# Ego-J/I2VSGG

Hardware: AMD Instinct MI355X
Metric: frames/sec (600x1000, 32 ROI/frame) (higher is better)
Workload: dtype f32; 1 GPU; BASELINE.json configs[1]: cfgs/res101.yml, SGG_emb fwd+bwd+SGD, 2 frames/GPU 600x1000, 32 boxes + 32 pairs/frame, ResNet-101 C4; frames_per_gpu=2, global_frames=2, hip_graph=True, parallelism=dp1 (frames sharded, RCCL all-reduce of vrd grads)

## Files before the change

i2vsgg_amd/_lib.py:

```python
import ctypes as C
import os

import torch

_HERE = os.path.dirname(os.path.abspath(__file__))
LIB_PATH = os.path.join(_HERE, "libi2vsgg_hip.so")

LAYOUT_NHWC, LAYOUT_NCHW = 0, 1
EPI_RELU, EPI_RESIDUAL, EPI_SCALE, EPI_BIAS, EPI_ZEROED = 1, 2, 4, 8, 16

_p, _i, _f, _z, _l = C.c_void_p, C.c_int32, C.c_float, C.c_size_t, C.c_int64

SIGNATURES = {
    "i2v_version": (_i, []),
    "i2v_last_error": (C.c_char_p, []),
    "i2v_build_flags": (_i, []),
    "i2v_stream_create": (_i, [_i, _i, C.POINTER(C.c_void_p)]),
    "i2v_stream_destroy": (_i, [_p]),
    "i2v_roi_align_fwd": (_i, [_p, _i, _i, _i, _i, _i, _p, _i, _i, _i, _f, _i, _p, _i, _p]),
    "i2v_roi_align_bwd": (_i, [_p, _i, _p, _i, _i, _i, _f, _i, _p, _i, _i, _i, _i, _i, _p]),
    "i2v_roi_align_bwd_gather_workspace_bytes": (_z, [_i, _i, _i, _i, _i]),
    "i2v_roi_align_bwd_gather": (_i, [_p, _p, _i, _i, _i, _f, _i, _p, _i, _i, _i, _i, _p, _z, _p]),
    "i2v_roi_align_sampled_fwd": (_i, [_p, _i, _i, _i, _i, _i, _p, _i, _i, _i, _f, _i, _p, _i, _p]),
    "i2v_roi_align_sampled_bwd": (_i, [_p, _i, _p, _i, _i, _i, _f, _i, _p, _i, _i, _i, _i, _i, _p]),
    "i2v_roi_pool_fwd": (_i, [_p, _i, _i, _i, _i, _i, _p, _i, _i, _i, _f, _p, _p, _i, _p]),
    "i2v_roi_pool_fwd_geom": (_i, [_p, _i, _i, _p, _l, _p, _i, _i, _i, _f, _p, _p, _i, _p]),
    "i2v_roi_pool_bwd": (_i, [_p, _p, _i, _p, _i, _i, _i, _p, _i, _i, _i, _i, _i, _p]),
    "i2v_nms_workspace_bytes": (_z, [_i, _i]),
    "i2v_nms_sorted": (_i, [_p, _i, _i, _f, _i, _p, _p, _p, _z, _p]),
    "i2v_rpn_proposal_workspace_bytes": (_z, [_i, _i, _i, _i, _i]),
    "i2v_rpn_proposal": (_i, [_p, _i, _p, _p, _p, _i, _i, _i, _i, _i, _i, _i, _f, _p, _p, _p, _p, _z, _p]),
    "i2v_rpn_decode": (_i, [_p, _i, _p, _p, _p, _i, _i, _i, _i, _i, _p, _p, _p]),
    "i2v_sort_desc_workspace_bytes": (_z, [_i, _i]),
    "i2v_sort_desc": (_i, [_p, _i, _i, _p, _p, _z, _p]),
    "i2v_bbox_overlaps": (_i, [_p, _i, _i, _i, _p, _i, _i, _i, _p, _p, _p, _p]),
    "i2v_conv_fwd": (_i, [_p, _p, _p, _p, _p, _p, _i, _i, _i, _i, _i, _i, _i, _i, _i, _i, _p, _z, _p]),
    "i2v_conv_fwd_splits": (_i, [_i, _i, _i, _i, _i, _i, _i, _i, _i, _z]),
    "i2v_conv_split_workspace_bytes": (_z, [_i, _i, _i, _i, _i, _i, _i, _i, _i]),
    "i2v_conv_fwd_plan": (_i, [_i, _i, _i, _i, _i, _i, _i, _i, _i, _i, _i, _z, _p, _i]),
    "i2v_conv_wgrad_plan": (_i, [_i, _i, _i, _i, _i, _i, _i, _i, _i, _i, _i, _i, _i, _i, _z, _p, _i]),
    "i2v_set_tuning": (_i, [_i, _i]),
    "i2v_get_tuning": (_i, [_i]),
    "i2v_gemm_nt_batched": (_i, [_p, _p, _p, _i, _i, _i, _i, _l, _l, _l, _p, _z, _p]),
    "i2v_winograd_filter": (_i, [_p, _p, _i, _i, _p]),
    "i2v_conv3x3_winograd_workspace_bytes": (_z, [_i, _i, _i, _i, _i]),
    "i2v_conv3x3_winograd_fwd": (_i, [_p, _p, _p, _p, _p, _i, _i, _i, _i, _i, _i, _p, _z, _p]),
    "i2v_winograd4_filter": (_i, [_p, _p, _i, _i, _p]),
    "i2v_winograd4_filter_dgrad": (_i, [_p, _p, _i, _i, _p]),
    "i2v_conv3x3_winograd4_workspace_bytes": (_z, [_i, _i, _i, _i, _i]),
    "i2v_conv3x3_winograd4_fwd": (_i, [_p, _p, _p, _p, _p, _i, _i, _i, _i, _i, _i, _p, _z, _p]),
    "i2v_conv_set_tile": (_i, [_i]),
    "i2v_conv_debug_clock": (_i, [_p]),
    "i2v_debug_clock_stamp": (_i, [_p, _p]),
    "i2v_conv_dgrad_workspace_bytes": (_z, [_i, _i, _i, _i]),
    "i2v_conv_dgrad": (_i, [_p, _p, _p, _i, _i, _i, _i, _i, _i, _i, _i, _i, _p, _z, _p, _z, _p]),
    "i2v_conv_wgrad_workspace_bytes": (_z, [_i, _i, _i, _i, _i, _i, _i, _i, _i]),
    "i2v_conv_wgrad": (_i, [_p, _p, _p, _i, _i, _i, _i, _i, _i, _i, _i, _i, _f, _p, _z, _p]),
    "i2v_conv_dgrad_fused": (_i, [_p, _p, _p, _p, _p, _p, _p, _i, _i, _i, _i, _i, _i, _i, _i, _i, _p, _z, _p, _z, _p]),
    "i2v_conv_wgrad_scaled": (_i, [_p, _p, _p, _p, _i, _i, _i, _i, _i, _i, _i, _i, _i, _f, _p, _z, _p]),
    "i2v_ordered_fallbacks": (_i, [_i]),
    "i2v_conv3x3_winograd4_dgrad": (_i, [_p, _p, _p, _p, _p, _i, _i, _i, _i, _i, _p, _z, _p]),
    "i2v_conv3x3_winograd4_wgrad_workspace_bytes": (_z, [_i, _i, _i, _i, _i]),
    "i2v_conv3x3_winograd4_wgrad": (_i, [_p, _p, _p, _p, _i, _i, _i, _i, _i, _f, _p, _z, _p]),
    "i2v_gemm_tn_batched": (_i, [_p, _p, _p, _i, _i, _i, _i, _l, _l, _l, _p]),
    "i2v_gemm_tn_batched_acc": (_i, [_p, _p, _p, _i, _i, _i, _i, _l, _l, _l, _p]),
    "i2v_conv3x3_winograd4_v_bytes": (_z, [_i, _i, _i, _i]),
    "i2v_conv3x3_winograd4_fwd_keep": (_i, [_p, _p, _p, _p, _p, _p, _i, _i, _i, _i, _i, _i, _p, _z, _p]),
    "i2v_conv3x3_winograd4_wgrad_v": (_i, [_p, _p, _p, _p, _i, _i, _i, _i, _i, _f, _p, _z, _p]),
    "i2v_conv_wgrad_sgd": (_i, [_p, _p, _p, _p, _i, _i, _i, _i, _i, _i, _i, _i, _i, _f, _f, _f, _p]),
    "i2v_epilogue_bwd": (_i, [_p, _p, _p, _p, _p, _p, _l, _i, _i, _p, _p, _z, _p]),
    "i2v_maxpool3x3s2_fwd": (_i, [_p, _p, _p, _i, _i, _i, _i, _p]),
    "i2v_sgd_momentum": (_i, [_p, _p, _p, _l, _f, _f, _f, _p]),
    "i2v_sgd_momentum_multi": (_i, [_p, _p, _p, _p, _p, _p, _i, _f, _p]),
    "i2v_adam_step": (_i, [_p, _p]),
    "i2v_adam_multi": (_i, [_p, _p, _p, _p, _p, _p, _p, _i, C.c_double, C.c_double, C.c_double, _p, _p]),
    "i2v_dstyle_pool_fwd": (_i, [_p, _p, _p, _l, _i, _i, _i, _p]),
    "i2v_dstyle_pool_bwd": (_i, [_p, _p, _p, _p, _p, _l, _i, _i, _i, _p]),
    "i2v_dstyle_fused_workspace_bytes": (_z, [_l, _i, _i, _i]),
    "i2v_dstyle_fused_fwd": (_i, [_p, _p, _p, _p, _p, _p, _p, _p, _l, _i, _i, _i, _i, _p, _z, _p]),
    "i2v_relation_topk_workspace_bytes": (_z, [_i, _i]),
    "i2v_relation_topk": (_i, [_p, _p, _p, _p, _i, _i, _i, _p, _p, _p, _p, _z, _p]),
    "i2v_video_associate_workspace_bytes": (_z, [_i, _i, _i]),
    "i2v_video_associate": (_i, [_p, _p, _p, _p, _p, _p, _i, _i, _i, _i, _p, _p, _p, _p, _p, _p, _z, _p]),
    "i2v_video_viou_match_workspace_bytes": (_z, [_i, _i]),
    "i2v_video_viou_match": (_i, [_p, _p, _p, _p, _p, _p, _i, _i, _i, _l, _i, _i, C.c_double, _p, _p, _p, _p, _z, _p]),
    "i2v_seqnms_workspace_bytes": (_z, [_i, _i, _i]),
    "i2v_seqnms": (_i, [_p, _p, _p, _p, _p, _i, _i, _i, C.c_double, C.c_double, _i, _p, _p, _p, _p, _z, _p]),
    "i2v_relation_targets_workspace_bytes": (_z, [_i]),
    "i2v_relation_targets": (_i, [_p] * 11 + [_i] * 5 + [_p] * 10 + [_z, _p]),
    "i2v_recognition_rows_workspace_bytes": (_z, [_i]),
    "i2v_recognition_rows": (_i, [_p, _p, _p, _p, _p, _i, _i, _i, _i, _p, _p, _p, _p, _p, _z, _p]),
    "i2v_recognition_align_workspace_bytes": (_z, [_i, _i]),
    "i2v_recognition_align": (_i, [_p, _p, _p, _p, _i, _i, _i, _i, _i, _i, _p, _p, _p, _p, _p, _p, _p, _z, _p]),
    "i2v_image_relation_match_workspace_bytes": (_z, [_i]),
    "i2v_image_relation_match": (_i, [_p, _p, _p, _p, _p, _p, _i, _i, _i, _i, C.c_double, _p, _p, _p, _p, _z, _p]),
    "i2v_image_relation_count": (_i, [_p, _p, _p, _p, _i, _i, _i, _p, _p, _p, _p, _z, _p]),
    "i2v_det_eval_match_workspace_bytes": (_z, [_i]),
    "i2v_det_eval_match": (_i, [_p, _p, _p, _p, _p, _p, _p, _i, _i, _i, _i, _i, C.c_double, _p, _p, _p, _p, _z, _p]),
    "i2v_det_eval_curve_workspace_bytes": (_z, [_i]),
    "i2v_det_eval_curve": (_i, [_p, _p, _p, _p, _i, _i, _p, _p, _p, _p, _p, _p, _p, _p, _z, _p]),
    "i2v_image_prep_size": (_i, [_i, _i, _i, _p, _p, _p]),
    "i2v_image_prep": (_i, [_p, _i, _i, _i, _i, _p, _i, _p, _i, _i, _p]),
    "i2v_det_postprocess_workspace_bytes": (_z, [_i, _i]),
    "i2v_det_postprocess": (_i, [_p, _p, _p, _i, _p, _p, _f, _f, _f, _i, _i, _f, _f, _i, _p, _p, _p, _z, _p]),
    "i2v_det_postprocess_info": (_i, [_p, _p, _p, _i, _p, _p, _p, _i, _i, _f, _f, _i, _p, _p, _p, _z, _p]),
    "i2v_l2norm_rows_fwd": (_i, [_p, _p, _p, _i, _i, _f, _p]),
    "i2v_l2norm_rows_bwd": (_i, [_p, _p, _p, _p, _i, _i, _f, _p]),
    "i2v_bce_rows_fwd": (_i, [_p, _p, _p, _p, _i, _i, _p]),
    "i2v_bce_rows_bwd": (_i, [_p, _p, _p, _p, _p, _i, _i, _p]),
    "i2v_half_mse_fwd": (_i, [_p, _l, _f, _p, _p]),
    "i2v_half_mse_bwd": (_i, [_p, _l, _f, _p, _p, _p]),
    "i2v_smooth_l1_fwd": (_i, [_p, _p, _p, _p, _l, _i, _i, _f, _p, _p]),
    "i2v_smooth_l1_bwd": (_i, [_p, _p, _p, _p, _l, _i, _i, _f, _p, _p, _p]),
    "i2v_bbox_transform": (_i, [_p, _i, _p, _i, _p, _i, _i, _p, _p, _p]),
    "i2v_signed_sqrt_fwd": (_i, [_p, _p, _l, _p]),
    "i2v_signed_sqrt_bwd": (_i, [_p, _p, _p, _l, _p]),
    "i2v_pair_gather_fwd": (_i, [_p, _p, _p, _p, _i, _i, _i, _p]),
    "i2v_pair_gather_bwd": (_i, [_p, _p, _p, _p, _i, _i, _i, _p]),
    "i2v_dpixel_fwd": (_i, [_p, _p, _p, _p, _p, _p, _p, _p, _i, _i, _p]),
    "i2v_dpixel_bwd_workspace_bytes": (_z, []),
    "i2v_dpixel_bwd": (_i, [_p, _p, _p, _p, _p, _p, _p, _p, _p, _p, _p, _p, _i, _i, _f, _p, _z, _p]),
}


class I2VError(RuntimeError):
    pass


def _load():
    if not os.path.exists(LIB_PATH):
        raise ImportError(
            "i2vsgg_amd: %s not found. Build it with `python -c 'import __graft_entry__ as g; g.build()'` "
            "(hipcc --offload-arch=gfx950). There is no CPU fallback." % LIB_PATH)
    lib = C.CDLL(LIB_PATH)
    for name, (res, args) in SIGNATURES.items():
        try:
            fn = getattr(lib, name)
        except AttributeError:
            raise ImportError("i2vsgg_amd: %s does not export %s (stale build?)" % (LIB_PATH, name))
        fn.restype, fn.argtypes = res, args
    return lib


lib = _load()

TUNE = {"I2V_CONV_SPEC": 0, "I2V_SPLIT_TARGET": 1, "I2V_SPLIT_TARGET_SKINNY": 2, "I2V_SPLIT_BELOW": 3, "I2V_SPLIT_ATOMICS": 4,
        "I2V_BIG_FC_TILE": 5, "I2V_WGRAD_V2": 6, "I2V_WGRAD_FUSED_TILE": 7, "I2V_WINO_ROWS": 8, "I2V_ROIPOOL_C128": 9, "I2V_CONV_GEMM": 10, "I2V_STAGGER": 11, "I2V_ROIALIGN_COLS": 12, "I2V_WGRAD_PER_CU": 13, "I2V_WGRAD_XCD": 14, "I2V_FC_FOLD": 15, "I2V_GEMM_X3": 16,
        "I2V_GEMM_PERSIST": 17, "I2V_WGRAD_PRIO": 18, "I2V_STREAM_TILE": 19, "I2V_KGROUPS": 20, "I2V_WGRAD_ORDERED_GFLOP": 21, "I2V_GEMM_DMA": 22,
        "I2V_WGRAD_DMA": 23, "I2V_ROIALIGN_BWD": 24, "I2V_NMS_SCAN": 25, "I2V_FC_UPDATE": 26}
ENV_TUNE = ("I2V_SPLIT_ATOMICS", "I2V_SPLIT_TARGET", "I2V_SPLIT_TARGET_SKINNY", "I2V_SPLIT_BELOW", "I2V_BIG_FC_TILE",
            "I2V_WGRAD_FUSED_TILE", "I2V_WGRAD_PER_CU", "I2V_KGROUPS", "I2V_WGRAD_ORDERED_GFLOP", "I2V_WINO_ROWS", "I2V_GEMM_DMA", "I2V_WGRAD_DMA", "I2V_ROIALIGN_BWD", "I2V_NMS_SCAN")
RETIRED_ENV = ("I2V_WINOGRAD_TRAIN", "I2V_BLOCK_FUSED", "I2V_WINOGRAD_WGRAD", "I2V_KEEP_V", "I2V_WGRAD_BRANCH", "I2V_ISD_BATCHED",
               "I2V_DEFER_FC", "I2V_EXPERIMENTS")
for _name, _key in TUNE.items():
    if os.environ.get(_name) in (None, ""):
        continue
    if _name not in ENV_TUNE:
        raise ImportError("i2vsgg_amd: %s is set but is not an environment knob (README.md lists them); it would be ignored. "
                          "Use i2vsgg_amd._lib.lib.i2v_set_tuning(TUNE[%r], value) from a tool or test" % (_name, _name))
    if lib.i2v_set_tuning(_key, int(os.environ[_name])) != 0:
        raise ImportError("i2vsgg_amd: %s=%s refused: %s" % (_name, os.environ[_name], lib.i2v_last_error().decode()))
for _name in RETIRED_ENV:
    if os.environ.get(_name) not in (None, ""):
        import warnings
        warnings.warn("i2vsgg_amd: %s is set but no longer read (a settled switch of rounds 1-5): the default runs" % _name)


def check(rc, what):
    if rc != 0:
        raise I2VError("%s failed (%d): %s" % (what, rc, lib.i2v_last_error().decode()))


def ptr(t):
    return None if t is None else t.data_ptr()


def stream():
    import torch
    return torch.cuda.current_stream().cuda_stream
```

i2vsgg_amd/csrc/api.cpp:

```cpp
#include <hip/hip_runtime.h>
#include <stdarg.h>
#include <stdio.h>
#include "../../include/i2vsgg_hip.h"

static thread_local char g_err[512] = "";

void i2v_set_error(const char* fmt, ...) {
    va_list ap;
    va_start(ap, fmt);
    vsnprintf(g_err, sizeof(g_err), fmt, ap);
    va_end(ap);
}

extern "C" int32_t i2v_version(void) { return 107; }
extern "C" const char* i2v_last_error(void) { return g_err; }

int g_i2v_tuning[I2V_TUNE_COUNT] = {
     -1,  2,  -1,  256,  2,
     1,  1,  128,  0,  1,
     1,  0,  2,  4,  1,
     0,  0,  0,  0,  1,
     0,  1000000,  1,  1,  1,  2,
     1,
};

extern "C" int32_t i2v_build_flags(void) {
    return 0;
}

extern "C" int32_t i2v_set_tuning(int32_t key, int32_t value) {
    if (key < 0 || key >= I2V_TUNE_COUNT) {
        i2v_set_error("set_tuning: unknown key %d", key);
        return I2V_ERR_ARG;
    }
    const bool retired = key == I2V_TUNE_CONV_SPEC ? value > 0
                       : (key == I2V_TUNE_FC_FOLD || key == I2V_TUNE_GEMM_X3 || key == I2V_TUNE_GEMM_PERSIST ||
                          key == I2V_TUNE_WGRAD_PRIO || key == I2V_TUNE_STAGGER) ? value != 0 : false;
    if (retired) {
        i2v_set_error("set_tuning: key %d belonged to an experiment kernel that is no longer in the library", key);
        return I2V_ERR_UNSUPPORTED;
    }
    g_i2v_tuning[key] = value;
    return I2V_OK;
}


extern "C" int32_t i2v_get_tuning(int32_t key) {
    return (key < 0 || key >= I2V_TUNE_COUNT) ? I2V_ERR_ARG : g_i2v_tuning[key];
}

extern "C" int32_t i2v_stream_create(int32_t device, int32_t priority, void** stream) {
    if (!stream) {
        i2v_set_error("stream_create: null output");
        return I2V_ERR_ARG;
    }
    int prev = -1, n = 0;
    if (hipGetDeviceCount(&n) != hipSuccess || device < 0 || device >= n) {
        i2v_set_error("stream_create: no device %d (%d visible)", device, n);
        return I2V_ERR_ARG;
    }
    hipStream_t s = nullptr;
    hipError_t e = hipGetDevice(&prev);
    if (e == hipSuccess && prev != device) e = hipSetDevice(device);
    if (e == hipSuccess) {
        int lo = 0, hi = 0;
        e = hipDeviceGetStreamPriorityRange(&lo, &hi);
        if (e == hipSuccess) {
            int pr = priority < hi ? hi : (priority > lo ? lo : priority);
            e = hipStreamCreateWithPriority(&s, hipStreamNonBlocking, pr);
        }
    }
    if (prev >= 0 && prev != device) (void)hipSetDevice(prev);
    if (e != hipSuccess) {
        i2v_set_error("stream_create: %s", hipGetErrorString(e));
        return I2V_ERR_LAUNCH;
    }
    *stream = (void*)s;
    return I2V_OK;
}

extern "C" int32_t i2v_stream_destroy(void* stream) {
    if (!stream) return I2V_OK;
    hipError_t e = hipStreamDestroy((hipStream_t)stream);
    if (e != hipSuccess) {
        i2v_set_error("stream_destroy: %s", hipGetErrorString(e));
        return I2V_ERR_LAUNCH;
    }
    return I2V_OK;
}
```

i2vsgg_amd/csrc/conv.hip:

```cpp
#include "conv_common.h"

using namespace convplan;

int g_ablate = 0;
unsigned long long* g_clk = nullptr;
int g_ordered_fallbacks = 0;

namespace {

struct ConvP {
    const float* x; const float* w; const float* scale; const float* shift; const float* res; float* y;
    const float* mask;
    int B, H, W, Cin, Cout, KH, KW, stride, pad, Ho, Wo;
    int pad_x;
    int M, N, K;
    int flags;
    int splitk, k_per_split;
    int ostride;
    int Hy, Wy;
    int lgCin;
    int reserved0;
    unsigned x_bytes, w_bytes;
    int ablate;
    int ktab_entries;
// ... 855 lines not shown
        if ((flags & I2V_EPI_MASK) && !(mask[i] > 0.f)) v = 0.f;
        y[i] = v;
    }
}

int g_force_tile = -1;

template <auto Kernel>
void launch_conv(dim3 grid, int threads, size_t lds, const ConvP& p, hipStream_t st) {
    static const bool once = [] {
        (void)hipFuncSetAttribute((const void*)Kernel, hipFuncAttributeMaxDynamicSharedMemorySize, 96 * 1024);
        return true;
    }();
    (void)once;
    Kernel<<<grid, threads, lds, st>>>(p);
}

template <int WAVES_M, int WAVES_N, int TM, int TN>
void launch_tile(int form, const ConvP& p, hipStream_t st) {
    constexpr int BM = WAVES_M * TM * 16, BN = WAVES_N * TN * 16;
    const dim3 grid(i2v_cdiv(p.M, BM) * i2v_cdiv(p.N, BN), p.splitk, p.nbatch > 1 ? p.nbatch : 1);
    const size_t lds_g = (size_t)(2 * (BM + BN) * BKS) * sizeof(float);
    const bool mask = (p.flags & I2V_EPI_MASK) != 0;
    switch (form) {
    case FORM_GEMM:
        if (mask) launch_conv<conv_gemm_f32<WAVES_M, WAVES_N, TM, TN, false, true>>(grid, THREADS, lds_g, p, st);
        else if (p.clk) launch_conv<conv_gemm_f32<WAVES_M, WAVES_N, TM, TN, true>>(grid, THREADS, lds_g, p, st);
        else launch_conv<conv_gemm_f32<WAVES_M, WAVES_N, TM, TN>>(grid, THREADS, lds_g, p, st);
        break;
    case FORM_GEMM_DMA32:
        if (mask) launch_conv<conv_gemm_f32<WAVES_M, WAVES_N, TM, TN, false, true, 1, 1>>(grid, THREADS, lds_g, p, st);
        else launch_conv<conv_gemm_f32<WAVES_M, WAVES_N, TM, TN, false, false, 1, 1>>(grid, THREADS, lds_g, p, st);
        break;
    case FORM_GEMM_DMA16:
        if (mask) launch_conv<conv_gemm_f32<WAVES_M, WAVES_N, TM, TN, false, true, 1, 2>>(grid, THREADS, lds_g / 2, p, st);
        else launch_conv<conv_gemm_f32<WAVES_M, WAVES_N, TM, TN, false, false, 1, 2>>(grid, THREADS, lds_g / 2, p, st);
        break;
    default: {
        const size_t stage = lds_g + p.ktab_entries * sizeof(float), epi = (size_t)BM * (BN + 4) * sizeof(float);
        launch_conv<conv_igemm_f32<WAVES_M, WAVES_N, TM, TN>>(grid, THREADS, stage > epi ? stage : epi, p, st);
    }
    }
}

template <int WAVES_M, int WAVES_N, int TM, int TN, int KG>
int launch_kgroups(const ConvP& p, hipStream_t st) {
    constexpr int BM = WAVES_M * TM * 16, BN = WAVES_N * TN * 16;
    constexpr int need = KG * 2 * (BM + BN) * BKS * 4;
    static_assert(need <= 159 * 1024, "the stage-buffer sets fit the CU's LDS");
    static const hipError_t once_k = [] {
        hipError_t e = hipFuncSetAttribute((const void*)conv_gemm_f32<WAVES_M, WAVES_N, TM, TN, false, false, KG>,
                                           hipFuncAttributeMaxDynamicSharedMemorySize, need);
        hipError_t e2 = hipFuncSetAttribute((const void*)conv_gemm_f32<WAVES_M, WAVES_N, TM, TN, false, true, KG>,
                                            hipFuncAttributeMaxDynamicSharedMemorySize, need);
        return e != hipSuccess ? e : e2;
    }();
    if (once_k != hipSuccess) {
        (void)hipGetLastError();
        i2v_set_error("conv: %d bytes of LDS refused for the K-group kernel: %s", need, hipGetErrorString(once_k));
        return I2V_ERR_LAUNCH;
    }
    const int tiles = i2v_cdiv(p.M, BM) * i2v_cdiv(p.N, BN);
    if (p.flags & I2V_EPI_MASK)
        conv_gemm_f32<WAVES_M, WAVES_N, TM, TN, false, true, KG><<<dim3(tiles, 1, 1), THREADS * KG, need, st>>>(p);
    else
        conv_gemm_f32<WAVES_M, WAVES_N, TM, TN, false, false, KG><<<dim3(tiles, 1, 1), THREADS * KG, need, st>>>(p);
    return I2V_OK;
}

ConvShape shape_of(const ConvP& p) {
    return {p.B, p.H, p.W, p.Cin, p.Cout, p.KH, p.KW, p.stride, p.pad, p.pad_x, p.ostride, p.Ho, p.Wo, p.nbatch, p.flags};
}

int run_conv(ConvP p, hipStream_t st, void* split_ws = nullptr, size_t split_ws_bytes = 0) {
    const ConvShape shape = shape_of(p);
    const FwdPlan pl = plan_conv_fwd(shape, g_i2v_tuning, g_force_tile, g_clk != nullptr, split_ws ? split_ws_bytes : 0);
    if (pl.status != PLAN_OK) return plan_error(pl.status, shape);
    p.M = p.B * p.Ho * p.Wo;
    p.N = p.Cout;
    p.K = p.KH * p.KW * p.Cin;
    p.lgCin = ilog2_exact(p.Cin);
    p.ktab_entries = pl.ktab_entries;
    p.x_bytes = pl.x_bytes;
    p.w_bytes = pl.w_bytes;
    p.clk = g_clk;
    p.ablate = g_ablate;
    p.splitk = pl.splitk;
    p.k_per_split = pl.k_per_split;
    p.ws = nullptr;
    p.cnt = nullptr;
    if (pl.finish == FIN_IN_KERNEL) {
        p.cnt = reinterpret_cast<int*>(split_ws);
        p.ws = reinterpret_cast<float*>(static_cast<char*>(split_ws) + kSplitCounterBytes);
    }
    if (pl.ordered_fallback) ++g_ordered_fallbacks;
    const long long ytotal = (long long)p.M * p.N;
    if (pl.clear_y) hipMemsetAsync(p.y, 0, (size_t)ytotal * sizeof(float), st);
    switch (pl.form == FORM_GEMM_KGROUPS2 ? 10 + pl.kg_tile : pl.form == FORM_GEMM_KGROUPS4 ? 20 + pl.kg_tile : pl.tile) {
        case 0: launch_tile<2, 2, 4, 4>(pl.form, p, st); break;
        case 1: launch_tile<2, 2, 4, 2>(pl.form, p, st); break;
        case 2: launch_tile<2, 2, 3, 2>(pl.form, p, st); break;
        case 3: launch_tile<1, 4, 5, 1>(pl.form, p, st); break;
        case 4: launch_tile<2, 2, 2, 2>(pl.form, p, st); break;
        case 5: launch_tile<2, 2, 1, 2>(pl.form, p, st); break;
        case 10: return launch_kgroups<1, 4, 5, 1, 2>(p, st);
        case 11: return launch_kgroups<2, 2, 2, 2, 2>(p, st);
        case 12: return launch_kgroups<1, 4, 3, 1, 2>(p, st);
        case 13: return launch_kgroups<2, 2, 1, 2, 2>(p, st);
        case 20: return launch_kgroups<1, 4, 5, 1, kKGroups>(p, st);
        case 21: return launch_kgroups<2, 2, 2, 2, kKGroups>(p, st);
        case 22: return launch_kgroups<1, 4, 3, 1, kKGroups>(p, st);
        case 23: return launch_kgroups<2, 2, 1, 2, kKGroups>(p, st);
    }
    if (pl.epilogue_pass == PASS_VEC4)
        conv_epilogue_kernel<<<(int)fmin((double)i2v_cdiv(ytotal / 4, 256), 4096.0), 256, 0, st>>>(
            p.y, p.scale, p.shift, p.res, p.mask, ytotal / 4, p.N, p.flags);
    else if (pl.epilogue_pass == PASS_SCALAR)
        conv_epilogue_scalar_kernel<<<(int)fmin((double)i2v_cdiv(ytotal, 256), 4096.0), 256, 0, st>>>(
            p.y, p.scale, p.shift, p.res, p.mask, ytotal, p.N, p.flags);
    return I2V_OK;
}

__global__ void weight_dgrad_layout(const float* __restrict__ w, float* __restrict__ wt, int Cout, int KH, int KW,
                                    int Cin, const float* __restrict__ nscale = nullptr) {
    const long long total = (long long)Cout * KH * KW * Cin;
    for (long long i = blockIdx.x * (long long)blockDim.x + threadIdx.x; i < total;
         i += (long long)gridDim.x * blockDim.x) {
        int n = i % Cout;
        long long t = i / Cout;
        int kx = t % KW; t /= KW;
        int ky = t % KH;
        int c = t / KH;
        const float v = w[(((long long)n * KH + (KH - 1 - ky)) * KW + (KW - 1 - kx)) * Cin + c];
        wt[i] = nscale ? v * nscale[n] : v;
    }
}

__global__ void weight_dgrad_sub_layout(const float* __restrict__ w, float* __restrict__ wt, int Cout, int KH, int KW,
                                        int Cin, int s, int ky0, int kx0, int Ty, int Tx) {
    const long long total = (long long)Cin * Ty * Tx * Cout;
    for (long long i = blockIdx.x * (long long)blockDim.x + threadIdx.x; i < total;
         i += (long long)gridDim.x * blockDim.x) {
        int n = i % Cout;
        long long t = i / Cout;
        int ux = t % Tx; t /= Tx;
        int uy = t % Ty;
        int c = t / Ty;
        const int ky = ky0 + s * (Ty - 1 - uy), kx = kx0 + s * (Tx - 1 - ux);
        wt[i] = w[(((long long)n * KH + ky) * KW + kx) * Cin + c];
    }
}

}

extern "C" int32_t i2v_ordered_fallbacks(int32_t reset) {
    const int n = g_ordered_fallbacks;
    if (reset) g_ordered_fallbacks = 0;
    return n;
}

extern "C" int32_t i2v_conv_debug_clock(void* buf) {
    g_clk = (unsigned long long*)buf;
    return I2V_OK;
}

namespace {
__global__ void clock_stamp_kernel(unsigned long long* out) {
    if (threadIdx.x == 0) { out[0] = __builtin_amdgcn_s_memtime(); out[1] = __builtin_amdgcn_s_memrealtime(); }
}
}

extern "C" int32_t i2v_debug_clock_stamp(void* out2, void* stream) {
    clock_stamp_kernel<<<1, 64, 0, (hipStream_t)stream>>>((unsigned long long*)out2);
    I2V_CHECK_LAUNCH("i2v_debug_clock_stamp");
    return I2V_OK;
}

extern "C" int32_t i2v_conv_set_tile(int32_t cfg) {
    if (cfg < 0) { g_force_tile = -1; g_ablate = 0; return I2V_OK; }
    if (cfg >> 8) {
        i2v_set_error("conv_set_tile: bits above the tile index selected experiment kernels that left the library in round 6");
        return I2V_ERR_UNSUPPORTED;
    }
    g_force_tile = (cfg & 0xFF) == 0xFF ? -1 : (cfg & 0xFF);
    return I2V_OK;
}

static int plan_conv(const char* who, FwdPlan& pl, size_t ws_bytes, int32_t B, int32_t H, int32_t W, int32_t Cin, int32_t Cout,
                     int32_t KH, int32_t KW, int32_t stride, int32_t pad, int32_t nbatch = 0, int32_t flags = 0) {
    int dummy = 0;
    int rc = check_conv(who, &dummy, &dummy, &dummy, B, H, W, Cin, Cout, KH, KW, stride, pad);
    if (rc) return rc;
    const ConvShape s = {B, H, W, Cin, Cout, KH, KW, stride, pad, pad, 1, (H + 2 * pad - KH) / stride + 1, (W + 2 * pad - KW) / stride + 1,
                         nbatch, flags};
    pl = plan_conv_fwd(s, g_i2v_tuning, g_force_tile, g_clk != nullptr, ws_bytes);
    return plan_error(pl.status, s);
}

extern "C" int32_t i2v_conv_fwd_splits(int32_t B, int32_t H, int32_t W, int32_t Cin, int32_t Cout, int32_t KH,
                                       int32_t KW, int32_t stride, int32_t pad, size_t ws_bytes) {
    FwdPlan pl = {};
    const int rc = plan_conv("conv_fwd_splits", pl, ws_bytes, B, H, W, Cin, Cout, KH, KW, stride, pad);
    return rc < 0 ? rc : pl.finish == FIN_ATOMICS;
}

extern "C" size_t i2v_conv_split_workspace_bytes(int32_t B, int32_t H, int32_t W, int32_t Cin, int32_t Cout, int32_t KH,
                                                 int32_t KW, int32_t stride, int32_t pad) {
    FwdPlan pl = {};
    return plan_conv("conv_fwd_splits", pl, 0, B, H, W, Cin, Cout, KH, KW, stride, pad) ? 0 : pl.ws_wanted;
}

extern "C" int32_t i2v_conv_fwd_plan(int32_t B, int32_t H, int32_t W, int32_t Cin, int32_t Cout, int32_t KH, int32_t KW,
                                     int32_t stride, int32_t pad, int32_t nbatch, int32_t flags, size_t ws_bytes, int32_t* out,
                                     int32_t n_out) {
    I2V_CHECK_ARG(out && n_out >= I2V_FWD_PLAN_FIELDS, "conv_fwd_plan: out needs room for I2V_FWD_PLAN_FIELDS values");
    FwdPlan pl = {};
    const int rc = plan_conv("conv_fwd_plan", pl, ws_bytes, B, H, W, Cin, Cout, KH, KW, stride, pad, nbatch, flags);
    if (rc && pl.status == PLAN_OK) return rc;
    const int32_t v[I2V_FWD_PLAN_FIELDS] = {pl.status, pl.tile, pl.splitk, pl.k_per_split, pl.ktab_entries, pl.form, pl.kg_tile,
                                            pl.finish, clamp32(pl.ws_wanted), clamp32(pl.ws_used), pl.clear_y, pl.epilogue_pass,
                                            pl.ordered_fallback};
    std::copy(v, v + I2V_FWD_PLAN_FIELDS, out);
    return I2V_OK;
}

extern "C" int32_t i2v_conv_fwd(const float* x, const float* w, const float* scale, const float* shift,
                                const float* res, float* y, int32_t B, int32_t H, int32_t W, int32_t Cin,
                                int32_t Cout, int32_t KH, int32_t KW, int32_t stride, int32_t pad, int32_t flags,
                                void* split_ws, size_t split_ws_bytes, void* stream) {
    int rc = check_conv("conv_fwd", x, w, y, B, H, W, Cin, Cout, KH, KW, stride, pad);
    if (rc) return rc;
    I2V_CHECK_ARG(!(flags & I2V_EPI_SCALE) || (scale && shift), "conv_fwd: EPI_SCALE needs scale and shift");
    I2V_CHECK_ARG(!(flags & I2V_EPI_BIAS) || shift, "conv_fwd: EPI_BIAS needs shift");
    I2V_CHECK_ARG(!(flags & I2V_EPI_RESIDUAL) || res, "conv_fwd: EPI_RESIDUAL needs res");
    ConvP p = {};
    p.x = x; p.w = w; p.scale = scale; p.shift = shift; p.res = res; p.y = y;
    p.B = B; p.H = H; p.W = W; p.Cin = Cin; p.Cout = Cout; p.KH = KH; p.KW = KW; p.stride = stride; p.pad = pad; p.pad_x = pad;
    p.Ho = (H + 2 * pad - KH) / stride + 1;
    p.Wo = (W + 2 * pad - KW) / stride + 1;
    p.flags = flags; p.ostride = 1; p.Hy = p.Ho; p.Wy = p.Wo;
    rc = run_conv(p, (hipStream_t)stream, split_ws, split_ws_bytes);
    if (rc) return rc;
    I2V_CHECK_LAUNCH("conv_fwd");
    return I2V_OK;
}

extern "C" int32_t i2v_gemm_nt_batched(const float* a, const float* b, float* c, int32_t M, int32_t N, int32_t K,
                                       int32_t nbatch, int64_t stride_a, int64_t stride_b, int64_t stride_c,
                                       void* split_ws, size_t split_ws_bytes, void* stream) {
    I2V_CHECK_ARG(a && b && c && M > 0 && N > 0 && K > 0 && nbatch > 0 && nbatch <= 65535, "gemm_nt_batched: bad argument");
    I2V_CHECK_ARG(K % 4 == 0, "gemm_nt_batched: K must be a multiple of 4");
    ConvP p = {};
    p.x = a; p.w = b; p.y = c;
    p.B = 1; p.H = M; p.W = 1; p.Cin = K; p.Cout = N; p.KH = 1; p.KW = 1; p.stride = 1; p.pad = 0; p.pad_x = 0;
    p.Ho = M; p.Wo = 1; p.flags = 0; p.ostride = 1; p.Hy = M; p.Wy = 1;
    p.nbatch = nbatch; p.bsx = stride_a; p.bsw = stride_b; p.bsy = stride_c;
    int rc = run_conv(p, (hipStream_t)stream, split_ws, split_ws_bytes);
    if (rc) return rc;
    I2V_CHECK_LAUNCH("gemm_nt_batched");
    return I2V_OK;
}

extern "C" size_t i2v_conv_dgrad_workspace_bytes(int32_t Cin, int32_t Cout, int32_t KH, int32_t KW) {
    return i2v_align((size_t)Cout * KH * KW * Cin * sizeof(float));
}

static int conv_dgrad_impl(const float* gy, const float* w, const float* gy_scale, const float* out_scale,
                           const float* res, const float* mask, float* gx, int32_t B, int32_t H, int32_t W,
                           int32_t Cin, int32_t Cout, int32_t KH, int32_t KW, int32_t stride, int32_t pad,
                           void* ws, size_t ws_bytes, void* split_ws, size_t split_ws_bytes, void* stream) {
    int rc = check_conv("conv_dgrad", gy, w, gx, B, H, W, Cin, Cout, KH, KW, stride, pad);
    if (rc) return rc;
    const bool fused = gy_scale || out_scale || res || mask;
    if (fused && stride != 1 && !(KH == 1 && KW == 1 && pad == 0)) {
        i2v_set_error("conv_dgrad_fused: stride 1, or a strided 1x1 layer (other strided layers take i2v_conv_dgrad and separate passes)");
        return I2V_ERR_UNSUPPORTED;
    }
    I2V_CHECK_ARG(Cout % 4 == 0, "conv_dgrad: Cout must be a multiple of 4");
    if (!ws || ws_bytes < (size_t)Cout * KH * KW * Cin * sizeof(float)) {
        i2v_set_error("conv_dgrad: workspace too small");
        return I2V_ERR_WORKSPACE;
    }
    hipStream_t st = (hipStream_t)stream;
    const int Ho = (H + 2 * pad - KH) / stride + 1, Wo = (W + 2 * pad - KW) / stride + 1;
    ConvP p = {};
    p.x = gy; p.y = gx;
    p.B = B; p.H = Ho; p.W = Wo; p.Cin = Cout; p.Cout = Cin; p.stride = 1;
    p.flags = 0;
    if (out_scale) { p.scale = out_scale; p.shift = nullptr; p.flags |= I2V_EPI_SCALE; }
    if (res) { p.res = res; p.flags |= I2V_EPI_RESIDUAL; }
    if (mask) { p.mask = mask; p.flags |= I2V_EPI_MASK; }
    p.Hy = H; p.Wy = W;
    const bool pointwise = KH == 1 && KW == 1 && pad == 0;
    if (stride == 1 || pointwise) {
        const long long wn = (long long)Cout * KH * KW * Cin;
        weight_dgrad_layout<<<(int)fmin((double)i2v_cdiv(wn, 256), 4096.0), 256, 0, st>>>(w, (float*)ws, Cout, KH, KW, Cin, gy_scale);
        p.w = (const float*)ws;
        p.KH = KH; p.KW = KW;
        if (stride == 1) {
            I2V_CHECK_ARG(KH - 1 - pad >= 0 && KW - 1 - pad >= 0, "conv_dgrad: padding larger than the filter");
            p.pad = KH - 1 - pad; p.pad_x = KW - 1 - pad;
            p.Ho = H; p.Wo = W; p.ostride = 1;
        } else {
            p.pad = 0; p.pad_x = 0; p.Ho = Ho; p.Wo = Wo; p.ostride = stride;
            hipMemsetAsync(gx, 0, (size_t)B * H * W * Cin * sizeof(float), st);
        }
// ... 54 lines not shown
```

i2vsgg_amd/csrc/conv_common.h:

```cpp
#pragma once
#include "common.h"
#include "conv_plan.h"
#include <algorithm>

typedef float f32x16 __attribute__((ext_vector_type(16)));
typedef float f32x4 __attribute__((ext_vector_type(4)));
typedef unsigned int u32x4 __attribute__((ext_vector_type(4)));

constexpr int THREADS = 256;

__device__ inline void lds_dma16(unsigned dst, unsigned voff, __amdgpu_buffer_rsrc_t r, unsigned soff) {
    asm volatile("s_mov_b32 m0, %0\n\ts_nop 0\n\tbuffer_load_dwordx4 %1, %2, %3 offen lds" ::"s"(dst), "v"(voff), "s"(r), "s"(soff) : "memory");
}

inline int ilog2_exact(int v) {
    if (v <= 0 || (v & (v - 1))) return -1;
    int l = 0;
    while ((1 << l) < v) ++l;
    return l;
}

inline int32_t clamp32(size_t v) { return (int32_t)std::min<size_t>(v, 0x7FFFFFFF); }

inline int check_conv(const char* who, const void* a, const void* b, const void* c, int B, int H, int W, int Cin,
                      int Cout, int KH, int KW, int stride, int pad) {
    if (!a || !b || !c) { i2v_set_error("%s: null pointer", who); return I2V_ERR_ARG; }
    if (B <= 0 || H <= 0 || W <= 0 || Cin <= 0 || Cout <= 0 || KH <= 0 || KW <= 0 || stride <= 0 || pad < 0) {
        i2v_set_error("%s: bad shape", who); return I2V_ERR_ARG;
    }
    if (Cin % 4) { i2v_set_error("%s: Cin must be a multiple of 4 (pad the stem input to 4 channels)", who); return I2V_ERR_ARG; }
    if ((H + 2 * pad - KH) < 0 || (W + 2 * pad - KW) < 0) { i2v_set_error("%s: kernel larger than input", who); return I2V_ERR_ARG; }
    return I2V_OK;
}

inline int plan_error(int status, const convplan::ConvShape& s) {
    using namespace convplan;
    if (status == PLAN_TAP_TABLE) i2v_set_error("conv: filter %dx%dx%d too large for the tap table", s.KH, s.KW, s.Cin);
    else if (status == PLAN_OPERAND_2GIB) i2v_set_error("conv: operand larger than 2 GiB (32-bit buffer offsets)");
    else if (status == PLAN_ROW_SCALE_NEEDS_V2) i2v_set_error("conv_wgrad_scaled: shape outside the v2 kernel (Cout % 4, 2 GiB operands)");
    else if (status == PLAN_FUSED_NEEDS_SPLIT) i2v_set_error("conv_wgrad_sgd: shape needs a split over pixels; use i2v_conv_wgrad + i2v_sgd_momentum");
    return status == PLAN_OK ? I2V_OK : I2V_ERR_UNSUPPORTED;
}

extern unsigned long long* g_clk;
extern int g_ablate;
extern int g_ordered_fallbacks;

int32_t i2v_internal_gemm_tn_batched_parts(const float* x, const float* gy, float* parts, int32_t M, int32_t N, int32_t K,
                                           int32_t nbatch, long long stride_x, long long stride_gy, int cap, int* splits, void* stream);
int32_t i2v_internal_reduce_parts(float* parts, int nparts, int planes, long long nk, void* stream);
void i2v_internal_reduce_scalar(const float* part, float* out, int nparts, long long n, int acc, unsigned blocks, void* stream);
```

i2vsgg_amd/csrc/conv_plan.h:

```cpp
#pragma once
#include <stddef.h>
#include <stdint.h>
#include "../../include/i2vsgg_hip.h"

namespace convplan {

constexpr int NUM_CU = 256;
constexpr int KTAB_MAX = 2560;
constexpr int BKS = 32;
constexpr int kSplitInKernelMax = 4;
constexpr int kKGroups = 4;
constexpr int kWgradOrderedMax = 16;
constexpr int kSplitCounters = 1024;
constexpr size_t kSplitCounterBytes = sizeof(int) * kSplitCounters;

struct TileCfg { int bm, bn; float eff; };
constexpr TileCfg kTiles[] = {{128, 128, 1.00f}, {128, 64, 0.97f}, {96, 64, 0.95f}, {80, 64, 0.95f}, {64, 64, 0.93f},
                              {32, 64, 0.80f}};
constexpr int kNumTiles = sizeof(kTiles) / sizeof(kTiles[0]);
constexpr int kKgroupBm[4] = {80, 64, 48, 32};

inline int cdiv(long long a, long long b) { return (int)((a + b - 1) / b); }

struct ConvShape {
    int B, H, W, Cin, Cout, KH, KW, stride, pad, pad_x, ostride, Ho, Wo, nbatch, flags;
    int M() const { return B * Ho * Wo; }
    int N() const { return Cout; }
    int K() const { return KH * KW * Cin; }
    int planes() const { return nbatch > 1 ? nbatch : 1; }
};

inline bool is_untapped(const ConvShape& s) { return s.KH == 1 && s.KW == 1 && s.pad == 0 && s.pad_x == 0; }
inline bool is_pointwise(const ConvShape& s) {
    return is_untapped(s) && s.stride == 1 && s.ostride == 1 && s.Ho == s.H && s.Wo == s.W && (s.N() & 3) == 0 && (s.K() & 3) == 0;
}
inline bool is_linear(const ConvShape& s) { return s.KH == 1 && s.KW == 1 && s.pad == 0 && s.stride == 1; }

enum PlanStatus { PLAN_OK = 0, PLAN_TAP_TABLE = 1, PLAN_OPERAND_2GIB = 2, PLAN_ROW_SCALE_NEEDS_V2 = 3, PLAN_FUSED_NEEDS_SPLIT = 4 };
enum FwdForm { FORM_IGEMM = 0, FORM_GEMM = 1, FORM_GEMM_DMA32 = 2, FORM_GEMM_DMA16 = 3, FORM_GEMM_KGROUPS2 = 4, FORM_GEMM_KGROUPS4 = 5 };
enum FwdFinish { FIN_NONE = 0, FIN_IN_KERNEL = 1, FIN_ATOMICS = 2 };
enum EpiloguePass { PASS_NONE = 0, PASS_VEC4 = 1, PASS_SCALAR = 2 };

struct FwdPlan {
    int status;
    int tile;
    int splitk, k_per_split;
    int ktab_entries;
    int form;
    int kg_tile;
    int finish;
    size_t ws_wanted;
    size_t ws_used;
    int clear_y;
    int epilogue_pass;
    int ordered_fallback;
    unsigned x_bytes, w_bytes;
};

inline FwdPlan plan_conv_fwd(const ConvShape& s, const int* tuning, int force_tile, bool clk, size_t ws_bytes) {
    FwdPlan q = {};
    const int M = s.M(), N = s.N(), K = s.K();
    if (!is_untapped(s) && (K > KTAB_MAX * 4 || s.KH * s.KW > 64 || ((long long)(s.KH * s.W + s.KW) * s.Cin) >= (1ll << 24))) {
        q.status = PLAN_TAP_TABLE;
        return q;
    }
    const long long xb = (long long)s.B * s.H * s.W * s.Cin * 4, wb = (long long)N * K * 4;
    const long long lead = (long long)(s.pad * s.W + s.pad_x) * s.Cin * 4;
    if (xb + (lead > 0 ? lead : 0) >= (1ll << 31) || wb >= (1ll << 31)) {
        q.status = PLAN_OPERAND_2GIB;
        return q;
    }
    q.ktab_entries = is_untapped(s) ? 4 : ((K + BKS - 1) / BKS) * (BKS / 4);
    q.x_bytes = (unsigned)xb;
    q.w_bytes = (unsigned)wb;
    const int split_atomics = tuning[I2V_TUNE_SPLIT_ATOMICS];
    const int ksteps = cdiv(K, BKS);
    auto cost_of = [&](int c, int& splitk) {
        const long long t = (long long)cdiv(M, kTiles[c].bm) * cdiv(N, kTiles[c].bn) * s.planes();
        splitk = 1;
        if (t < tuning[I2V_TUNE_SPLIT_BELOW] && ksteps >= 8 && s.ostride == 1 && s.nbatch <= 1) {
            const int skinny = tuning[I2V_TUNE_SPLIT_TARGET_SKINNY];
            const int target = (M <= 256 && skinny > 0) ? skinny : tuning[I2V_TUNE_SPLIT_TARGET];
            splitk = (int)((target * NUM_CU + t - 1) / t);
            splitk = splitk > ksteps / 4 ? ksteps / 4 : splitk;
            if (splitk < 1) splitk = 1;
            if (split_atomics == 2 && splitk > kSplitInKernelMax && (long long)M * N >= (1 << 18)) splitk = kSplitInKernelMax;
        }
        const long long blocks = t * splitk;
        const long long rounds = (blocks + NUM_CU - 1) / NUM_CU;
        const double r = rounds <= 4 ? (double)rounds : (double)blocks / NUM_CU + 0.5;
        double cost = r * kTiles[c].bm * kTiles[c].bn * (double)cdiv(ksteps, splitk) / kTiles[c].eff;
        if (splitk > 1) cost *= 1.05;
        return cost;
    };
    int cfg = 0, splitk = 1;
    double best = 1e300;
    for (int c = 0; c < kNumTiles; ++c) {
        int sk;
        const double cost = cost_of(c, sk);
        if (cost < best) { best = cost; cfg = c; splitk = sk; }
    }
    if (tuning[I2V_TUNE_STREAM_TILE] && s.KH == 1 && s.KW == 1 && s.stride == 1 && s.nbatch <= 1 && ksteps <= 4 && M >= 16384) {
        cfg = 3;
        cost_of(cfg, splitk);
    }
    if (s.nbatch > 1 && ksteps <= 4) { cfg = kNumTiles - 1; cost_of(cfg, splitk); }
    const int big_fc_tile = tuning[I2V_TUNE_BIG_FC_TILE];
    if (big_fc_tile >= 0 && big_fc_tile < kNumTiles && M <= 256 && K >= 16384) { cfg = big_fc_tile; cost_of(cfg, splitk); }
    if (force_tile >= 0 && force_tile < kNumTiles) { cfg = force_tile; cost_of(cfg, splitk); }
    q.tile = cfg;
    q.k_per_split = cdiv(ksteps, splitk) * BKS;
    q.splitk = cdiv(K, q.k_per_split);
    const bool gemm_kernel = is_pointwise(s) && tuning[I2V_TUNE_CONV_GEMM];
    const int kgroups = tuning[I2V_TUNE_KGROUPS];
    q.kg_tile = -1;
    const int kgn = kgroups == 2 ? 2 : kKGroups;
    if (kgroups && gemm_kernel && !clk && s.nbatch <= 1 && q.splitk >= 2 && force_tile < 0 && K % (kgn * BKS) == 0 &&
        K / kgn >= 2 * BKS && (long long)M * N >= (1 << 18)) {
        const int nt = cdiv(N, 64);
        for (int c = 3; c >= 0; --c) {
            const int t = cdiv(M, kKgroupBm[c]) * nt;
            if (t <= NUM_CU) { if (t >= (NUM_CU * 7) / 10) q.kg_tile = c; break; }
        }
        if (q.kg_tile >= 0) { q.splitk = 1; q.k_per_split = K; }
    }
    const long long ntiles = (long long)cdiv(M, kTiles[cfg].bm) * cdiv(N, kTiles[cfg].bn);
    const size_t ws_need = (size_t)q.splitk * ntiles * kTiles[cfg].bm * kTiles[cfg].bn * sizeof(float);
    const bool r4_ok = q.splitk <= kSplitInKernelMax && (long long)M * N >= (1 << 18);
    const bool wants_ws = q.splitk > 1 && split_atomics != 1 && (r4_ok || split_atomics == 0) && ntiles <= kSplitCounters &&
                          ws_need < (1ull << 31) - (64u << 20);
    const bool in_kernel = wants_ws && kSplitCounterBytes + ws_need <= ws_bytes;
    q.ws_wanted = wants_ws ? (kSplitCounterBytes + ws_need < 0x7FFFFFFF ? kSplitCounterBytes + ws_need : 0x7FFFFFFF) : 0;
    q.ws_used = in_kernel ? kSplitCounterBytes + ws_need : 0;
    q.finish = q.splitk <= 1 ? FIN_NONE : in_kernel ? FIN_IN_KERNEL : FIN_ATOMICS;
    q.ordered_fallback = q.finish == FIN_ATOMICS && split_atomics == 0;
    q.clear_y = q.finish == FIN_ATOMICS && !(s.flags & I2V_EPI_ZEROED);
    if (q.finish == FIN_ATOMICS && (s.flags & (I2V_EPI_SCALE | I2V_EPI_BIAS | I2V_EPI_RESIDUAL | I2V_EPI_RELU | I2V_EPI_MASK)))
        q.epilogue_pass = N % 4 == 0 ? PASS_VEC4 : PASS_SCALAR;
    const int dma = tuning[I2V_TUNE_GEMM_DMA];
    if (q.kg_tile >= 0) q.form = kgroups == 2 ? FORM_GEMM_KGROUPS2 : FORM_GEMM_KGROUPS4;
    else if (!gemm_kernel || q.finish == FIN_ATOMICS) q.form = FORM_IGEMM;
    else if (dma > 0 && !clk) q.form = dma == 2 ? FORM_GEMM_DMA16 : FORM_GEMM_DMA32;
    else q.form = FORM_GEMM;
    return q;
}

enum WgradKernel {
    WG_V1_64x64 = 0, WG_V2_DMA_128x128, WG_V2_DMA_128x64, WG_V2_DMA_64x64, WG_V2_FUSED_128x64, WG_V2_128x128, WG_V2_128x64,
    WG_V2_FUSED_64x64, WG_V2_CLK_64x64, WG_V2_64x64,
    WG_FC_UPDATE
};
enum WgradFinish { WFIN_DIRECT = 0, WFIN_ATOMICS = 1, WFIN_ORDERED_TILES = 2, WFIN_ORDERED_PARTS = 3, WFIN_EXTERNAL_PARTS = 4 };

struct WgradPlan {
    int status;
    int v2;
    int kernel;
    int tm, tk;
    int splits, m_per_split;
    int finish;
    int direct;
    int xcd_remap;
    int tiles;
    unsigned grid[3];
    int dma;
    size_t clear_bytes;
    int reduce_pass;
    int ordered_fallback;
    unsigned x_bytes, gy_bytes;
};

inline int wgrad_split_count(long long M, int N, int K, int planes, int tm, int tk, int rs, const int* tuning) {
    const long long tiles = (long long)cdiv(N, tm) * cdiv(K, tk), all_tiles = tiles * planes;
    const int msteps = cdiv(M, rs), per_cu = tuning[I2V_TUNE_WGRAD_PER_CU];
    int splits = (int)((long long)per_cu * NUM_CU / all_tiles);
    if (splits < 2) splits = (int)(((long long)per_cu * NUM_CU + all_tiles - 1) / all_tiles);
    if (splits > msteps / 4) splits = msteps / 4;
    if (splits < 1) splits = 1;
    return splits;
}

inline int wgrad_plane_splits(long long T, int Cout, int Cin, const int* tuning) {
    const int s = wgrad_split_count(T, Cout, Cin, 36, 64, 64, BKS, tuning);
    const int mps = cdiv(cdiv(T, BKS), s) * BKS;
    return cdiv(T, mps);
}

inline WgradPlan plan_wgrad(const ConvShape& s, bool beta_nonzero, bool fused, bool has_row_scale, int ext_part_cap, const int* tuning,
                            bool clk, size_t ws_bytes) {
    WgradPlan q = {};
    const int M = s.M(), N = s.N(), K = s.K(), planes = s.planes();
    const int wgrad_v2 = tuning[I2V_TUNE_WGRAD_V2];
    const long long xb = (long long)s.B * s.H * s.W * s.Cin * 4, gb = (long long)M * N * 4;
    const bool lin = is_linear(s);
    if (fused) {
        if ((long long)cdiv(N, 64) * cdiv(K, 64) < 2 * NUM_CU || M > 4096) { q.status = PLAN_FUSED_NEEDS_SPLIT; return q; }
        if (tuning[I2V_TUNE_FC_UPDATE] && wgrad_v2 && lin && M <= 256 && N % 4 == 0 && K % 4 == 0 && (long long)M * K * 4 < (1ll << 31) &&
            gb < (1ll << 31) && (long long)N * K * 4 < (1ll << 31)) {
            q.v2 = 1; q.kernel = WG_FC_UPDATE; q.splits = 1; q.direct = 1; q.finish = WFIN_DIRECT;
            return q;
        }
    }
    const bool v2 = (N % 4 == 0) && xb < (1ll << 31) && gb < (1ll << 31) && wgrad_v2;
    q.v2 = v2;
    if (has_row_scale && !v2) { q.status = PLAN_ROW_SCALE_NEEDS_V2; return q; }
    int tm = 64, tk = 64;
    if (v2 && fused && tuning[I2V_TUNE_WGRAD_FUSED_TILE] == 128 && N >= 128) tm = 128;
    if (v2 && wgrad_v2 >= 2) {
        if (N >= 128) tm = 128;
        if (K >= 128 && tm == 128 && wgrad_v2 == 2) tk = 128;
    }
    const long long tiles = (long long)cdiv(N, tm) * cdiv(K, tk);
    const int rs = v2 ? BKS : 16;
    const int msteps = cdiv(M, rs);
    int splits = fused ? 1 : wgrad_split_count(M, N, K, planes, tm, tk, rs, tuning);
    const bool ext_part = ext_part_cap >= 0;
    const bool has_ws = ws_bytes > 0;
    const double ord_flops = 1e9 * tuning[I2V_TUNE_WGRAD_ORDERED_GFLOP], flops = 2.0 * M * N * K * planes;
    const bool want_ord = !fused && !ext_part && splits > 1 && tuning[I2V_TUNE_SPLIT_ATOMICS] == 0 && flops < ord_flops;
    if (want_ord && has_ws && v2 && splits > kWgradOrderedMax && flops < 1e9) splits = kWgradOrderedMax;
    if (ext_part && splits > ext_part_cap) splits = ext_part_cap > 0 ? ext_part_cap : 1;
    q.m_per_split = cdiv(msteps, splits) * rs;
    splits = cdiv(M, q.m_per_split);
    q.direct = (splits == 1 && !beta_nonzero) || fused;
    q.finish = q.direct ? WFIN_DIRECT : WFIN_ATOMICS;
    if (ext_part) {
        if (splits > 1) q.finish = WFIN_EXTERNAL_PARTS;
    } else if (want_ord && splits > 1) {
        const size_t need_ord = kSplitCounterBytes + (size_t)splits * tiles * planes * (size_t)(tm * tk) * sizeof(float);
        const size_t need_part = kSplitCounterBytes + (size_t)splits * planes * (size_t)N * K * sizeof(float);
        if (has_ws && v2 && splits <= kWgradOrderedMax && tiles * planes <= kSplitCounters && need_ord <= ws_bytes && need_ord < (1ull << 31))
            q.finish = WFIN_ORDERED_TILES;
        else if (has_ws && need_part <= ws_bytes) {
            q.finish = WFIN_ORDERED_PARTS;
            q.reduce_pass = (((long long)N * K) & 3) == 0 ? PASS_VEC4 : PASS_SCALAR;
        } else q.ordered_fallback = 1;
    }
    if (!beta_nonzero && q.finish == WFIN_ATOMICS) q.clear_bytes = (size_t)planes * N * K * sizeof(float);
    q.x_bytes = (unsigned)xb;
    q.gy_bytes = (unsigned)gb;
    q.tm = tm; q.tk = tk; q.splits = splits; q.tiles = (int)tiles;
    q.grid[0] = (unsigned)tiles; q.grid[1] = (unsigned)splits; q.grid[2] = (unsigned)planes;
    const long long groups = (long long)splits * planes, total = tiles * groups;
    q.xcd_remap = (v2 && groups >= 2 && total < (1ll << 30) && tuning[I2V_TUNE_WGRAD_XCD]) ? 1 : 0;
    if (q.xcd_remap) { q.grid[0] = (unsigned)((total + 7) / 8 * 8); q.grid[1] = 1; q.grid[2] = 1; }
    const bool dma = v2 && !fused && !clk && lin && (K % 4 == 0) && tuning[I2V_TUNE_WGRAD_DMA];
    q.dma = dma;
    if (!v2) q.kernel = WG_V1_64x64;
    else if (dma && tm == 128 && tk == 128) q.kernel = WG_V2_DMA_128x128;
    else if (dma && tm == 128) q.kernel = WG_V2_DMA_128x64;
    else if (dma) q.kernel = WG_V2_DMA_64x64;
    else if (fused && tm == 128 && tk == 64) q.kernel = WG_V2_FUSED_128x64;
    else if (tm == 128 && tk == 128) q.kernel = WG_V2_128x128;
    else if (tm == 128) q.kernel = WG_V2_128x64;
    else if (fused) q.kernel = WG_V2_FUSED_64x64;
    else if (clk) q.kernel = WG_V2_CLK_64x64;
    else q.kernel = WG_V2_64x64;
    return q;
}

}
```

i2vsgg_amd/csrc/roi_ops.hip:

```cpp
#include "common.h"
#include <float.h>

namespace {

struct Strides { long long b, c, h, w; };

__host__ __device__ inline Strides feat_strides(int layout, int C, int H, int W) {
    Strides s;
    if (layout == I2V_LAYOUT_NHWC) { s.c = 1; s.w = C; s.h = (long long)W * C; s.b = (long long)H * W * C; }
    else { s.w = 1; s.h = W; s.c = (long long)H * W; s.b = (long long)C * H * W; }
    return s;
}

struct Sample { int ok, hs, ws; float hr, wr; };

__device__ inline Sample ra_sample(const float* roi, float scale, int H, int W, int AH, int AW, int ph, int pw) {
    Sample s;
    float x1 = roi[1] * scale, y1 = roi[2] * scale, x2 = roi[3] * scale, y2 = roi[4] * scale;
    float rw = fmaxf((float)((double)(x2 - x1) + 1.), 0.f);
    float rh = fmaxf((float)((double)(y2 - y1) + 1.), 0.f);
    float bh = (float)((double)rh / (AH - 1.));
    float bw = (float)((double)rw / (AW - 1.));
    float h = (float)ph * bh + y1;
    float w = (float)pw * bw + x1;
// ... 581 lines not shown
                v.x = l.x + v.x; v.y = l.y + v.y; v.z = l.z + v.z; v.w = l.w + v.w;
            }
            const int meta = __builtin_amdgcn_readfirstlane(rec.meta), nr = (meta >> 8) & 255, round = rec.meta & 255;
            float4* pl = (float4*)(mybuf + ((rec.off & 0xFFFFu) ^ lxor));
            float4* pr = (float4*)(mybuf + ((rec.off >> 16) ^ lxor));
            const float4 tl = make_float4(v.x * rec.wl, v.y * rec.wl, v.z * rec.wl, v.w * rec.wl);
            const float4 tr = make_float4(v.x * rec.wr, v.y * rec.wr, v.z * rec.wr, v.w * rec.wr);
#if defined(RAB_CLOCKS) && defined(RAB_ABL) && (RAB_ABL & 1)
            if (tl.x + tr.y == 12345.678f) *pl = tl;
            return;
#endif
            for (int s = 0; s < nr; ++s) {
                if (round == s) {
                    float4 a = *pl;
                    a.x += tl.x; a.y += tl.y; a.z += tl.z; a.w += tl.w;
                    *pl = a;
                    float4 c = *pr;
                    c.x += tr.x; c.y += tr.y; c.z += tr.z; c.w += tr.w;
                    *pr = c;
                }
            }
        };
        float4 q[RB2_DEPTH][NQ];
        if (n > 0) {
#pragma unroll
            for (int k = 0; k < RB2_DEPTH; ++k) issue(q[k], GROUPS * k + grp, list[min(GROUPS * k + grp, n - 1)]);
        }
        if (base == 0) {
            for (int i = threadIdx.x; i < (W + 2) * 32; i += 256) ((float4*)rowbuf)[i] = make_float4(0.f, 0.f, 0.f, 0.f);
        }
        for (int e0 = 0; e0 < n; e0 += RB2_CHUNK) {
            RAB_T(c_r0);
            {
                const int u = threadIdx.x >> 3, sx = threadIdx.x & 7, e = e0 + u;
                int cell = W;
                float wl = 0.f, wr = 0.f;
                if (e < n && sx < AW) {
                    const int code = 2 * base + (int)list[e], pair = code >> 1;
                    const int r = pair / AH, ah = pair - r * AH;
                    const float* roi = rois + 5 * (long long)r;
                    const AxisGeom qr = ra_axis(roi[2], roi[4], scale, H, AH, ah);
                    const AxisGeom qc = ra_axis(roi[1], roi[3], scale, W, AW, sx);
                    if (qc.ok) {
                        const float fh = (code & 1) ? qr.r : (1 - qr.r);
                        cell = qc.s; wl = fh * (1 - qc.r); wr = fh * qc.r;
                    }
                }
                int round = 0;
#pragma unroll
                for (int k = 1; k < 8; ++k) {
                    const int c = __shfl_up(cell, k, 8);
                    if (sx >= k && c == cell && cell < W) ++round;
                }
                int nr = round + 1;
#pragma unroll
                for (int m = 1; m < 8; m <<= 1) nr = max(nr, __shfl_xor(nr, m, 8));
                TapRec2 rec;
                rec.off = (unsigned)(cell * CHB + ((cell & 7) << 5)) | ((unsigned)((cell + 1) * CHB + (((cell + 1) & 7) << 5)) << 16);
                rec.wl = AVG ? wl * 0.25f : wl; rec.wr = AVG ? wr * 0.25f : wr;
                rec.meta = round | (nr << 8);
                s_rec[u][sx] = rec;
            }
            __syncthreads();
            RAB_T(c_r1);
            const int ne = min(RB2_CHUNK, n - e0);
            TapRec2 rec = s_rec[grp][sxl];
            int code = list[min(e0 + GROUPS * RB2_DEPTH + grp, n - 1)];
            for (int u0 = 0; u0 < ne; u0 += GROUPS * RB2_DEPTH) {
#pragma unroll
                for (int k = 0; k < RB2_DEPTH; ++k) {
                    const int u = u0 + GROUPS * k + grp;
                    const TapRec2 recn = s_rec[min(u + GROUPS, RB2_CHUNK - 1)][sxl];
                    const int coden = list[min(e0 + u + GROUPS * RB2_DEPTH + GROUPS, n - 1)];
                    if (u < ne) process(q[k], rec);
                    issue(q[k], e0 + u + GROUPS * RB2_DEPTH, code);
                    rec = recn;
                    code = coden;
                }
            }
            __syncthreads();
            RAB_T(c_r2);
            RAB_ADD(c_rec, c_r0, c_r1); RAB_ADD(c_add, c_r1, c_r2);
        }
    }
    __syncthreads();
    RAB_T(c_st0);
    constexpr int C4B = 32 / GROUPS;
    float* o = gfeat + (((long long)b * H + h) * W) * C + chunk * (128 / GROUPS);
    const float4* buf1 = (const float4*)rowbuf + (size_t)(W + 2) * C4B;
    for (int i = threadIdx.x; i < W * C4B; i += 256) {
        const int x = i / C4B, c4 = i % C4B, at = x * C4B + (c4 ^ ((x & 7) << 1));
        float4 a = ((const float4*)rowbuf)[at];
        if (GROUPS == 2) { const float4 c = buf1[at]; a.x += c.x; a.y += c.y; a.z += c.z; a.w += c.w; }
        *(float4*)(o + (long long)x * C + 4 * c4) = a;
    }
#ifdef RAB_CLOCKS
    if (threadIdx.x == 0 && blockIdx.x < 8192) {
        unsigned long long* o6 = g_rab_clk[blockIdx.x];
        const unsigned long long c_end = __builtin_amdgcn_s_memtime();
        o6[0] = c_end - c_begin; o6[1] = c_list; o6[2] = c_rec; o6[3] = c_end - c_st0; o6[4] = c_add; o6[5] = c_n;
    }
#endif
}

__global__ void __launch_bounds__(256)
roi_pool_fwd_kernel(const float* __restrict__ feat, const float* __restrict__ rois, float* __restrict__ out,
                    int* __restrict__ argmax, int C, int H, int W, int PH, int PW, float scale, Strides fs,
                    Strides os, int out_nchw, const int* __restrict__ geom, long long cap_cells) {
    extern __shared__ float lds[];
    const int P = PH * PW;
    float* sval = lds;
    int* sarg = (int*)(lds + 64 * P);
    if (geom) {
        H = geom[0]; W = geom[1];
        if (H <= 0 || W <= 0 || (long long)H * W > cap_cells) H = W = 0;
        fs = feat_strides(I2V_LAYOUT_NHWC, C, H, W);
    }
    const int chunks = (C + 63) / 64;
    const int r = blockIdx.x / chunks, c0 = (blockIdx.x % chunks) * 64;
    const int lane = threadIdx.x & 63, wave = threadIdx.x >> 6;
    const int c = c0 + lane;
    const float* roi = rois + 5 * (long long)r;
    const int b = (int)roi[0];
    const int x1 = (int)roundf(roi[1] * scale), y1 = (int)roundf(roi[2] * scale);
    const int x2 = (int)roundf(roi[3] * scale), y2 = (int)roundf(roi[4] * scale);
    const int rw = max(x2 - x1 + 1, 1), rh = max(y2 - y1 + 1, 1);
    const float bh = (float)rh / (float)PH, bw = (float)rw / (float)PW;
    const bool live = c < C;
    const float* fb = feat + (long long)b * fs.b + (live ? c : 0) * fs.c;
    for (int ph = wave; ph < PH; ph += 4) {
        int hs = (int)floorf((float)ph * bh), he = (int)ceilf((float)(ph + 1) * bh);
        hs = min(max(hs + y1, 0), H); he = min(max(he + y1, 0), H);
        for (int pw = 0; pw < PW; ++pw) {
            int ws = (int)floorf((float)pw * bw), we = (int)ceilf((float)(pw + 1) * bw);
            ws = min(max(ws + x1, 0), W); we = min(max(we + x1, 0), W);
            bool empty = (he <= hs) || (we <= ws);
            float m = empty ? 0.f : -FLT_MAX;
            int mi = -1;
            if (live)
                for (int h = hs; h < he; ++h)
                    for (int w = ws; w < we; ++w) {
                        float v = fb[h * fs.h + w * fs.w];
                        if (v > m) { m = v; mi = h * W + w; }
                    }
            sval[lane * P + ph * PW + pw] = m;
            sarg[lane * P + ph * PW + pw] = mi;
        }
    }
    __syncthreads();
    const int nch = min(64, C - c0);
    if (out_nchw) {
        float* o = out + (long long)r * C * P + (long long)c0 * P;
        int* a = argmax + (long long)r * C * P + (long long)c0 * P;
        for (int e = threadIdx.x; e < nch * P; e += 256) { o[e] = sval[e]; a[e] = sarg[e]; }
    } else {
        for (int p = wave; p < P; p += 4)
            if (live) {
                long long o = (long long)r * P * C + (long long)p * C + c;
                out[o] = sval[lane * P + p];
                argmax[o] = sarg[lane * P + p];
            }
    }
}

__global__ void __launch_bounds__(512)
roi_pool_fwd_c128_kernel(const float* __restrict__ feat, const float* __restrict__ rois, float* __restrict__ out,
                         int* __restrict__ argmax, int C, int H, int W, int PH, int PW, float scale, int out_nchw,
                         const int* __restrict__ geom, long long cap_cells) {
    extern __shared__ __attribute__((aligned(16))) float lds[];
    const int P = PH * PW;
    float* sval = lds;
    int* sarg = (int*)(lds + 128 * P);
    if (geom) {
        H = geom[0]; W = geom[1];
        if (H <= 0 || W <= 0 || (long long)H * W > cap_cells) H = W = 0;
    }
    const int chunks = C / 128;
    const int r = blockIdx.x / chunks, c0 = (blockIdx.x % chunks) * 128;
    const int l32 = threadIdx.x & 31, grp = threadIdx.x >> 5;
    const float* roi = rois + 5 * (long long)r;
    const int b = (int)roi[0];
    const int x1 = (int)roundf(roi[1] * scale), y1 = (int)roundf(roi[2] * scale);
    const int x2 = (int)roundf(roi[3] * scale), y2 = (int)roundf(roi[4] * scale);
    const int rw = max(x2 - x1 + 1, 1), rh = max(y2 - y1 + 1, 1);
    const float bh = (float)rh / (float)PH, bw = (float)rw / (float)PW;
    const __amdgpu_buffer_rsrc_t fr = __builtin_amdgcn_make_buffer_rsrc(const_cast<float*>(feat), 0, 0x7FFFFFFCu, 0x00020000);
    const unsigned lane_off = (unsigned)(c0 + 4 * l32) * 4u, row_bytes = (unsigned)C * 4u;
    const unsigned img = (unsigned)b * (unsigned)(H * W);
    const int ngrp = blockDim.x >> 5;
    for (int p = grp; p < P; p += ngrp) {
        const int ph = p / PW, pw = p - ph * PW;
        int hs = (int)floorf((float)ph * bh), he = (int)ceilf((float)(ph + 1) * bh);
        hs = min(max(hs + y1, 0), H); he = min(max(he + y1, 0), H);
        int ws = (int)floorf((float)pw * bw), we = (int)ceilf((float)(pw + 1) * bw);
        ws = min(max(ws + x1, 0), W); we = min(max(we + x1, 0), W);
        const bool empty = (he <= hs) || (we <= ws);
        float4 m = empty ? make_float4(0.f, 0.f, 0.f, 0.f) : make_float4(-FLT_MAX, -FLT_MAX, -FLT_MAX, -FLT_MAX);
        int4 mi = make_int4(-1, -1, -1, -1);
        const int nw = we - ws, cells = empty ? 0 : (he - hs) * nw;
        int h = hs, w = ws;
        for (int k0 = 0; k0 < cells; k0 += 8) {
            float4 v[8];
            int id[8];
#pragma unroll
            for (int u = 0; u < 8; ++u) {
                const bool live = k0 + u < cells;
                id[u] = live ? h * W + w : -1;
                v[u] = __builtin_bit_cast(float4, __builtin_amdgcn_raw_buffer_load_b128(
                    fr, ((img + (unsigned)(h * W + w)) * row_bytes + lane_off) | (live ? 0u : 0x80000000u), 0, 0));
                if (++w == we) { w = ws; ++h; }
            }
#pragma unroll
            for (int u = 0; u < 8; ++u) {
                if (id[u] < 0) continue;
                if (v[u].x > m.x) { m.x = v[u].x; mi.x = id[u]; }
                if (v[u].y > m.y) { m.y = v[u].y; mi.y = id[u]; }
                if (v[u].z > m.z) { m.z = v[u].z; mi.z = id[u]; }
                if (v[u].w > m.w) { m.w = v[u].w; mi.w = id[u]; }
            }
        }
        const int e = (4 * l32) * P + p;
        sval[e] = m.x; sval[e + P] = m.y; sval[e + 2 * P] = m.z; sval[e + 3 * P] = m.w;
        sarg[e] = mi.x; sarg[e + P] = mi.y; sarg[e + 2 * P] = mi.z; sarg[e + 3 * P] = mi.w;
    }
    __syncthreads();
    if (out_nchw) {
        float* o = out + (long long)r * C * P + (long long)c0 * P;
        int* a = argmax + (long long)r * C * P + (long long)c0 * P;
        if ((((long long)r * C + c0) * P) % 4 == 0 && (128 * P) % 4 == 0) {
            for (int e = threadIdx.x * 4; e < 128 * P; e += 4 * blockDim.x) {
                *(float4*)(o + e) = *(const float4*)(sval + e);
                *(int4*)(a + e) = *(const int4*)(sarg + e);
            }
        } else {
            for (int e = threadIdx.x; e < 128 * P; e += blockDim.x) { o[e] = sval[e]; a[e] = sarg[e]; }
        }
    } else {
        for (int e = threadIdx.x; e < 128 * P; e += blockDim.x) {
            const int p = e >> 7, ch = e & 127;
            const long long o = (long long)r * P * C + (long long)p * C + c0 + ch;
            out[o] = sval[ch * P + p];
            argmax[o] = sarg[ch * P + p];
        }
    }
}

__global__ void roi_pool_bwd_kernel(const float* __restrict__ gout, const int* __restrict__ argmax,
                                    const float* __restrict__ rois, float* __restrict__ gfeat, long long total,
                                    int C, int W, int P, Strides fs, int out_nchw) {
    for (long long idx = blockIdx.x * (long long)blockDim.x + threadIdx.x; idx < total;
         idx += (long long)gridDim.x * blockDim.x) {
        int c, r;
        if (out_nchw) { c = (idx / P) % C; r = idx / P / C; }
        else { c = idx % C; r = idx / C / P; }
        int a = argmax[idx];
        if (a < 0) continue;
        int b = (int)rois[5 * (long long)r];
        atomicAdd(gfeat + b * fs.b + c * fs.c + (a / W) * fs.h + (a % W) * fs.w, gout[idx]);
    }
}

struct RasGeom { float y0, x0, bh, bw; int gh, gw; };

__device__ inline RasGeom ras_geometry(const float* roi, float scale, int PH, int PW, int sampling) {
    RasGeom g;
    const float x1 = roi[1] * scale, y1 = roi[2] * scale, x2 = roi[3] * scale, y2 = roi[4] * scale;
    const float rw = fmaxf(x2 - x1, 1.f), rh = fmaxf(y2 - y1, 1.f);
    g.x0 = x1; g.y0 = y1;
    g.bh = rh / (float)PH; g.bw = rw / (float)PW;
    g.gh = sampling > 0 ? sampling : (int)ceilf(rh / (float)PH);
    g.gw = sampling > 0 ? sampling : (int)ceilf(rw / (float)PW);
    return g;
}

struct RasTaps { int ok, yl, xl, yh, xh; float w0, w1, w2, w3; };

__device__ inline RasTaps ras_taps(int H, int W, float y, float x) {
    RasTaps t;
    t.ok = !(y < -1.0f || y > (float)H || x < -1.0f || x > (float)W);
    if (y <= 0) y = 0;
    if (x <= 0) x = 0;
    t.yl = (int)y; t.xl = (int)x;
    if (t.yl >= H - 1) { t.yh = t.yl = H - 1; y = (float)t.yl; } else t.yh = t.yl + 1;
    if (t.xl >= W - 1) { t.xh = t.xl = W - 1; x = (float)t.xl; } else t.xh = t.xl + 1;
    const float ly = y - (float)t.yl, lx = x - (float)t.xl, hy = 1.f - ly, hx = 1.f - lx;
    t.w0 = hy * hx; t.w1 = hy * lx; t.w2 = ly * hx; t.w3 = ly * lx;
    if (!t.ok) t.yl = t.xl = t.yh = t.xh = 0;
    return t;
}

template <int VEC>
__global__ void __launch_bounds__(256)
roi_align_sampled_fwd_kernel(const float* __restrict__ feat, const float* __restrict__ rois, float* __restrict__ out,
                             int B, int C, int H, int W, int PH, int PW, float scale, int sampling, Strides fs,
                             Strides os) {
    const int pw = blockIdx.x % PW, ph = (blockIdx.x / PW) % PH, r = blockIdx.x / (PW * PH);
    const float* roi = rois + 5 * (long long)r;
    const int b = (int)roi[0];
    const bool live = b >= 0 && b < B;
    const RasGeom g = ras_geometry(roi, scale, PH, PW, sampling);
    const float count = (float)(g.gh * g.gw);
    const float* fb = feat + (long long)(live ? b : 0) * fs.b;
    for (int c = threadIdx.x * VEC; c < C; c += blockDim.x * VEC) {
        float acc[VEC];
#pragma unroll
        for (int k = 0; k < VEC; ++k) acc[k] = 0.f;
        for (int iy = 0; live && iy < g.gh; ++iy) {
            const float y = g.y0 + (float)ph * g.bh + ((float)iy + .5f) * g.bh / (float)g.gh;
            for (int ix = 0; ix < g.gw; ++ix) {
                const float x = g.x0 + (float)pw * g.bw + ((float)ix + .5f) * g.bw / (float)g.gw;
                const RasTaps t = ras_taps(H, W, y, x);
                if (!t.ok) continue;
                const float* p = fb + c * fs.c;
                float v0[VEC], v1[VEC], v2[VEC], v3[VEC];
                if (VEC == 4) {
                    *(float4*)v0 = *(const float4*)(p + t.yl * fs.h + t.xl * fs.w);
                    *(float4*)v1 = *(const float4*)(p + t.yl * fs.h + t.xh * fs.w);
                    *(float4*)v2 = *(const float4*)(p + t.yh * fs.h + t.xl * fs.w);
                    *(float4*)v3 = *(const float4*)(p + t.yh * fs.h + t.xh * fs.w);
                } else {
                    v0[0] = p[t.yl * fs.h + t.xl * fs.w]; v1[0] = p[t.yl * fs.h + t.xh * fs.w];
                    v2[0] = p[t.yh * fs.h + t.xl * fs.w]; v3[0] = p[t.yh * fs.h + t.xh * fs.w];
                }
#pragma unroll
                for (int k = 0; k < VEC; ++k) acc[k] += t.w0 * v0[k] + t.w1 * v1[k] + t.w2 * v2[k] + t.w3 * v3[k];
            }
        }
#pragma unroll
        for (int k = 0; k < VEC; ++k) out[r * os.b + (c + k) * os.c + ph * os.h + pw * os.w] = acc[k] / count;
    }
}

__global__ void __launch_bounds__(256)
roi_align_sampled_bwd_kernel(const float* __restrict__ gout, const float* __restrict__ rois, float* __restrict__ gfeat,
                             int B, int C, int H, int W, int PH, int PW, float scale, int sampling, Strides fs,
                             Strides os) {
    const int pw = blockIdx.x % PW, ph = (blockIdx.x / PW) % PH, r = blockIdx.x / (PW * PH);
    const float* roi = rois + 5 * (long long)r;
    const int b = (int)roi[0];
    if (b < 0 || b >= B) return;
    const RasGeom g = ras_geometry(roi, scale, PH, PW, sampling);
    const float count = (float)(g.gh * g.gw);
    float* fb = gfeat + (long long)b * fs.b;
    for (int c = threadIdx.x; c < C; c += blockDim.x) {
        const float top = gout[r * os.b + c * os.c + ph * os.h + pw * os.w];
        float* p = fb + c * fs.c;
        for (int iy = 0; iy < g.gh; ++iy) {
            const float y = g.y0 + (float)ph * g.bh + ((float)iy + .5f) * g.bh / (float)g.gh;
            for (int ix = 0; ix < g.gw; ++ix) {
                const float x = g.x0 + (float)pw * g.bw + ((float)ix + .5f) * g.bw / (float)g.gw;
                const RasTaps t = ras_taps(H, W, y, x);
                if (!t.ok) continue;
                atomicAdd(p + t.yl * fs.h + t.xl * fs.w, top * t.w0 / count);
                atomicAdd(p + t.yl * fs.h + t.xh * fs.w, top * t.w1 / count);
                atomicAdd(p + t.yh * fs.h + t.xl * fs.w, top * t.w2 / count);
                atomicAdd(p + t.yh * fs.h + t.xh * fs.w, top * t.w3 / count);
            }
        }
    }
}

inline Strides out_strides(int layout, int C, int PH, int PW) {
    Strides s;
    if (layout == I2V_LAYOUT_NHWC) { s.c = 1; s.w = C; s.h = (long long)PW * C; s.b = (long long)PH * PW * C; }
    else { s.w = 1; s.h = PW; s.c = (long long)PH * PW; s.b = (long long)C * PH * PW; }
    return s;
}

}

extern "C" int32_t i2v_roi_align_fwd(const float* feat, int32_t feat_layout, int32_t B, int32_t C, int32_t H,
                                     int32_t W, const float* rois, int32_t R, int32_t PH, int32_t PW,
                                     float scale, int32_t avg, float* out, int32_t out_layout, void* stream) {
    if (R == 0) return I2V_OK;
    I2V_CHECK_ARG(feat && rois && out, "roi_align_fwd: null pointer");
    I2V_CHECK_ARG(B > 0 && C > 0 && H >= 2 && W >= 2 && R >= 0 && PH > 0 && PW > 0, "roi_align_fwd: bad shape");
    I2V_CHECK_ARG(avg == 0 || avg == 1, "roi_align_fwd: avg must be 0/1");
    I2V_CHECK_ARG(avg || (PH > 1 && PW > 1), "roi_align_fwd: aligned grid needs >=2 points per side");
    hipStream_t st = (hipStream_t)stream;
    Strides os = out_strides(out_layout, C, PH, PW);
    if (feat_layout == I2V_LAYOUT_NHWC && (C % 4) == 0) {
        const int groups = (PW + 1) / 2;
        const bool per_roi = g_i2v_tuning[I2V_TUNE_ROIALIGN_COLS] == 2 && out_layout == I2V_LAYOUT_NHWC && (C % 128) == 0 &&
                             (PH + avg) * (PW + avg) <= 64 && (long long)B * H * W * C * 4 < (1ll << 31);
        if (per_roi) {
            if (R * (C / 128) < 512) {
                if (avg) roi_align_fwd_roi_kernel<1, 64><<<R * (C / 64), 256, 0, st>>>(feat, rois, out, R, C, H, W, PH, PW, scale);
                else roi_align_fwd_roi_kernel<0, 64><<<R * (C / 64), 256, 0, st>>>(feat, rois, out, R, C, H, W, PH, PW, scale);
            } else if (avg) roi_align_fwd_roi_kernel<1><<<R * (C / 128), 256, 0, st>>>(feat, rois, out, R, C, H, W, PH, PW, scale);
            else roi_align_fwd_roi_kernel<0><<<R * (C / 128), 256, 0, st>>>(feat, rois, out, R, C, H, W, PH, PW, scale);
        } else if (!g_i2v_tuning[I2V_TUNE_ROIALIGN_COLS]) {
            if (avg) roi_align_fwd_nhwc<1><<<R * PH, 256, 0, st>>>(feat, rois, out, C, H, W, PH, PW, scale, os);
            else roi_align_fwd_nhwc<0><<<R * PH, 256, 0, st>>>(feat, rois, out, C, H, W, PH, PW, scale, os);
        } else if (avg) {
            roi_align_fwd_nhwc_cols<1><<<(R + 7) / 8 * 8 * PH * groups, 256, 0, st>>>(feat, rois, out, R, C, H, W, PH, PW, scale, os);
        } else {
            roi_align_fwd_nhwc_cols<0><<<(R + 7) / 8 * 8 * PH * groups, 256, 0, st>>>(feat, rois, out, R, C, H, W, PH, PW, scale, os);
        }
    } else {
        Strides fs = feat_strides(feat_layout, C, H, W);
        long long total = (long long)R * C * PH * PW;
        int grid = (int)fmin((double)i2v_cdiv(total, 256), 65535.0 * 4);
        if (avg) roi_align_fwd_generic<1><<<grid, 256, 0, st>>>(feat, rois, out, total, C, H, W, PH, PW, scale, fs, os);
        else roi_align_fwd_generic<0><<<grid, 256, 0, st>>>(feat, rois, out, total, C, H, W, PH, PW, scale, fs, os);
    }
    I2V_CHECK_LAUNCH("roi_align_fwd");
    return I2V_OK;
}

extern "C" int32_t i2v_roi_align_bwd(const float* gout, int32_t out_layout, const float* rois, int32_t R,
                                     int32_t PH, int32_t PW, float scale, int32_t avg, float* gfeat,
                                     int32_t feat_layout, int32_t B, int32_t C, int32_t H, int32_t W,
                                     void* stream) {
    if (R == 0) return I2V_OK;
    I2V_CHECK_ARG(gout && rois && gfeat, "roi_align_bwd: null pointer");
    I2V_CHECK_ARG(B > 0 && C > 0 && H >= 2 && W >= 2 && R >= 0 && PH > 0 && PW > 0, "roi_align_bwd: bad shape");
    I2V_CHECK_ARG(avg == 0 || avg == 1, "roi_align_bwd: avg must be 0/1");
    hipStream_t st = (hipStream_t)stream;
    Strides os = out_strides(out_layout, C, PH, PW), fs = feat_strides(feat_layout, C, H, W);
    if (avg) roi_align_bwd_kernel<1><<<R * (PH + 1), 256, 0, st>>>(gout, rois, gfeat, C, H, W, PH, PW, scale, fs, os);
    else roi_align_bwd_kernel<0><<<R * PH, 256, 0, st>>>(gout, rois, gfeat, C, H, W, PH, PW, scale, fs, os);
    I2V_CHECK_LAUNCH("roi_align_bwd");
    return I2V_OK;
}

extern "C" size_t i2v_roi_align_bwd_gather_workspace_bytes(int32_t R, int32_t C, int32_t PH, int32_t PW, int32_t avg) {
    (void)R; (void)C; (void)PH; (void)PW; (void)avg;
    return 0;
}

extern "C" int32_t i2v_roi_align_bwd_gather(const float* gout, const float* rois, int32_t R, int32_t PH, int32_t PW, float scale,
                                            int32_t avg, float* gfeat, int32_t B, int32_t C, int32_t H, int32_t W, void* ws,
                                            size_t ws_bytes, void* stream) {
    (void)ws; (void)ws_bytes;
    I2V_CHECK_ARG(gout && rois && gfeat, "roi_align_bwd_gather: null pointer");
    I2V_CHECK_ARG(B > 0 && C > 0 && H >= 2 && W >= 2 && R > 0 && PH > 0 && PW > 0, "roi_align_bwd_gather: bad shape");
    I2V_CHECK_ARG(avg == 0 || avg == 1, "roi_align_bwd_gather: avg must be 0/1");
    I2V_CHECK_ARG(C % 128 == 0, "roi_align_bwd_gather: C must be a multiple of 128 (NHWC in and out)");
    const size_t AH = PH + avg, AW = PW + avg;
    I2V_CHECK_ARG(AW <= RAB_MAXA, "roi_align_bwd_gather: at most 8 sample columns (pooled_w + avg <= 8)");
    const bool form2 = g_i2v_tuning[I2V_TUNE_ROIALIGN_BWD] != 0;
    const size_t lds = (size_t)(W + 2) * 128 * sizeof(float) + (form2 ? 0 : (size_t)RAB_BATCH * RAB_MAXA * 128 * sizeof(float)) + RAB_SEG * sizeof(unsigned short);
    I2V_CHECK_ARG(lds <= 60 * 1024 && (long long)R * AH < (1ll << 29), "roi_align_bwd_gather: map too wide for the LDS row buffer");
    I2V_CHECK_ARG((long long)B * H * (C / 128) < (1ll << 31), "roi_align_bwd_gather: grid too large");
    I2V_CHECK_ARG((long long)R * PH * PW * C * 4 < (1ll << 31), "roi_align_bwd_gather: grad_out beyond the 2 GiB a 32-bit buffer offset reaches");
    hipStream_t st = (hipStream_t)stream;
    const bool two = form2 && (long long)B * H * (C / 64) <= 4ll * 256;
    static bool once = [] {
        (void)hipFuncSetAttribute((const void*)roi_align_bwd_row_kernel<0, 0>, hipFuncAttributeMaxDynamicSharedMemorySize, 60 * 1024);
        (void)hipFuncSetAttribute((const void*)roi_align_bwd_row_kernel<1, 0>, hipFuncAttributeMaxDynamicSharedMemorySize, 60 * 1024);
        (void)hipFuncSetAttribute((const void*)roi_align_bwd_row_kernel<1, 1>, hipFuncAttributeMaxDynamicSharedMemorySize, 60 * 1024);
        (void)hipFuncSetAttribute((const void*)roi_align_bwd_row2_kernel<0, 0, 1>, hipFuncAttributeMaxDynamicSharedMemorySize, 60 * 1024);
        (void)hipFuncSetAttribute((const void*)roi_align_bwd_row2_kernel<1, 0, 1>, hipFuncAttributeMaxDynamicSharedMemorySize, 60 * 1024);
        (void)hipFuncSetAttribute((const void*)roi_align_bwd_row2_kernel<1, 1, 1>, hipFuncAttributeMaxDynamicSharedMemorySize, 60 * 1024);
        (void)hipFuncSetAttribute((const void*)roi_align_bwd_row2_kernel<0, 0, 2>, hipFuncAttributeMaxDynamicSharedMemorySize, 60 * 1024);
        (void)hipFuncSetAttribute((const void*)roi_align_bwd_row2_kernel<1, 0, 2>, hipFuncAttributeMaxDynamicSharedMemorySize, 60 * 1024);
        (void)hipFuncSetAttribute((const void*)roi_align_bwd_row2_kernel<1, 1, 2>, hipFuncAttributeMaxDynamicSharedMemorySize, 60 * 1024);
        return true;
    }();
    (void)once;
    const dim3 grid(B * H * (C / 128)), grid2(B * H * (C / 64));
    const int p7 = avg && PH == 7 && PW == 7;
#define RAB2(A, P, G, GRID) roi_align_bwd_row2_kernel<A, P, G><<<GRID, 256, lds, st>>>(gout, rois, gfeat, R, PH, PW, scale, B, C, H, W)
    if (form2 && two) { if (p7) RAB2(1, 1, 2, grid2); else if (avg) RAB2(1, 0, 2, grid2); else RAB2(0, 0, 2, grid2); }
    else if (form2) { if (p7) RAB2(1, 1, 1, grid); else if (avg) RAB2(1, 0, 1, grid); else RAB2(0, 0, 1, grid); }
#undef RAB2
    else if (avg && PH == 7 && PW == 7) roi_align_bwd_row_kernel<1, 1><<<grid, 256, lds, st>>>(gout, rois, gfeat, R, PH, PW, scale, B, C, H, W);
    else if (avg) roi_align_bwd_row_kernel<1, 0><<<grid, 256, lds, st>>>(gout, rois, gfeat, R, PH, PW, scale, B, C, H, W);
    else roi_align_bwd_row_kernel<0, 0><<<grid, 256, lds, st>>>(gout, rois, gfeat, R, PH, PW, scale, B, C, H, W);
    I2V_CHECK_LAUNCH("roi_align_bwd_gather");
    return I2V_OK;
}

namespace {
int32_t roi_pool_fwd_launch(const float* feat, int32_t feat_layout, int32_t B, int32_t C, int32_t H, int32_t W,
                            const int32_t* geom, long long cap_cells, const float* rois, int32_t R, int32_t PH, int32_t PW,
                            float scale, float* out, int32_t* argmax, int32_t out_layout, void* stream) {
    I2V_CHECK_ARG(PH * PW <= 256, "roi_pool_fwd: pooled grid too large for the LDS stage");
    Strides fs = feat_strides(feat_layout, C, H, W), os = out_strides(out_layout, C, PH, PW);
    const int c128 = g_i2v_tuning[I2V_TUNE_ROIPOOL_C128];
    const long long feat_bytes = (long long)B * C * 4 * (geom ? cap_cells : (long long)H * W);
    if (c128 && feat_layout == I2V_LAYOUT_NHWC && C % 128 == 0 && (size_t)128 * PH * PW * 8 <= 64 * 1024 && feat_bytes < (1ll << 31)) {
        roi_pool_fwd_c128_kernel<<<R * (C / 128), 512, (size_t)128 * PH * PW * 8, (hipStream_t)stream>>>(
            feat, rois, out, argmax, C, H, W, PH, PW, scale, out_layout == I2V_LAYOUT_NCHW, geom, cap_cells);
        I2V_CHECK_LAUNCH("roi_pool_fwd");
        return I2V_OK;
    }
    size_t lds = (size_t)64 * PH * PW * 8;
    roi_pool_fwd_kernel<<<R * ((C + 63) / 64), 256, lds, (hipStream_t)stream>>>(
        feat, rois, out, argmax, C, H, W, PH, PW, scale, fs, os, out_layout == I2V_LAYOUT_NCHW, geom, cap_cells);
    I2V_CHECK_LAUNCH("roi_pool_fwd");
    return I2V_OK;
}
}

extern "C" int32_t i2v_roi_pool_fwd(const float* feat, int32_t feat_layout, int32_t B, int32_t C, int32_t H,
                                    int32_t W, const float* rois, int32_t R, int32_t PH, int32_t PW, float scale,
                                    float* out, int32_t* argmax, int32_t out_layout, void* stream) {
    if (R == 0) return I2V_OK;
    I2V_CHECK_ARG(feat && rois && out && argmax, "roi_pool_fwd: null pointer");
    I2V_CHECK_ARG(B > 0 && C > 0 && H > 0 && W > 0 && R >= 0 && PH > 0 && PW > 0, "roi_pool_fwd: bad shape");
    return roi_pool_fwd_launch(feat, feat_layout, B, C, H, W, nullptr, 0, rois, R, PH, PW, scale, out, argmax, out_layout,
                               stream);
}

extern "C" int32_t i2v_roi_pool_fwd_geom(const float* feat, int32_t B, int32_t C, const int32_t* geom, int64_t cap_cells,
                                         const float* rois, int32_t R, int32_t PH, int32_t PW, float scale, float* out,
                                         int32_t* argmax, int32_t out_layout, void* stream) {
    if (R == 0) return I2V_OK;
    I2V_CHECK_ARG(feat && geom && rois && out && argmax, "roi_pool_fwd_geom: null pointer");
    I2V_CHECK_ARG(B > 0 && C > 0 && cap_cells > 0 && R >= 0 && PH > 0 && PW > 0, "roi_pool_fwd_geom: bad shape");
    return roi_pool_fwd_launch(feat, I2V_LAYOUT_NHWC, B, C, 1, 1, geom, (long long)cap_cells, rois, R, PH, PW, scale, out,
                               argmax, out_layout, stream);
}

extern "C" int32_t i2v_roi_pool_bwd(const float* gout, const int32_t* argmax, int32_t out_layout,
                                    const float* rois, int32_t R, int32_t PH, int32_t PW, float* gfeat,
                                    int32_t feat_layout, int32_t B, int32_t C, int32_t H, int32_t W,
                                    void* stream) {
    if (R == 0) return I2V_OK;
    I2V_CHECK_ARG(gout && argmax && rois && gfeat, "roi_pool_bwd: null pointer");
    I2V_CHECK_ARG(B > 0 && C > 0 && H > 0 && W > 0 && R >= 0 && PH > 0 && PW > 0, "roi_pool_bwd: bad shape");
    Strides fs = feat_strides(feat_layout, C, H, W);
    long long total = (long long)R * C * PH * PW;
    int grid = (int)fmin((double)i2v_cdiv(total, 256), 65535.0 * 4);
    roi_pool_bwd_kernel<<<grid, 256, 0, (hipStream_t)stream>>>(gout, argmax, rois, gfeat, total, C, W, PH * PW, fs,
                                                                out_layout == I2V_LAYOUT_NCHW);
    I2V_CHECK_LAUNCH("roi_pool_bwd");
    return I2V_OK;
}

extern "C" int32_t i2v_roi_align_sampled_fwd(const float* feat, int32_t feat_layout, int32_t B, int32_t C, int32_t H,
                                             int32_t W, const float* rois, int32_t R, int32_t PH, int32_t PW,
                                             float scale, int32_t sampling_ratio, float* out, int32_t out_layout,
                                             void* stream) {
    if (R == 0) return I2V_OK;
    I2V_CHECK_ARG(feat && rois && out, "roi_align_sampled_fwd: null pointer");
    I2V_CHECK_ARG(B > 0 && C > 0 && H > 0 && W > 0 && R >= 0 && PH > 0 && PW > 0, "roi_align_sampled_fwd: bad shape");
    I2V_CHECK_ARG((long long)R * PH * PW < (1ll << 31), "roi_align_sampled_fwd: too many bins for one launch");
    Strides fs = feat_strides(feat_layout, C, H, W), os = out_strides(out_layout, C, PH, PW);
    const int grid = R * PH * PW;
    if (feat_layout == I2V_LAYOUT_NHWC && (C % 4) == 0)
        roi_align_sampled_fwd_kernel<4><<<grid, 256, 0, (hipStream_t)stream>>>(feat, rois, out, B, C, H, W, PH, PW, scale,
                                                                               sampling_ratio, fs, os);
    else
        roi_align_sampled_fwd_kernel<1><<<grid, 256, 0, (hipStream_t)stream>>>(feat, rois, out, B, C, H, W, PH, PW, scale,
                                                                               sampling_ratio, fs, os);
    I2V_CHECK_LAUNCH("roi_align_sampled_fwd");
    return I2V_OK;
}

extern "C" int32_t i2v_roi_align_sampled_bwd(const float* gout, int32_t out_layout, const float* rois, int32_t R,
                                             int32_t PH, int32_t PW, float scale, int32_t sampling_ratio, float* gfeat,
                                             int32_t feat_layout, int32_t B, int32_t C, int32_t H, int32_t W,
                                             void* stream) {
    if (R == 0) return I2V_OK;
    I2V_CHECK_ARG(gout && rois && gfeat, "roi_align_sampled_bwd: null pointer");
    I2V_CHECK_ARG(B > 0 && C > 0 && H > 0 && W > 0 && R >= 0 && PH > 0 && PW > 0, "roi_align_sampled_bwd: bad shape");
    I2V_CHECK_ARG((long long)R * PH * PW < (1ll << 31), "roi_align_sampled_bwd: too many bins for one launch");
    Strides fs = feat_strides(feat_layout, C, H, W), os = out_strides(out_layout, C, PH, PW);
    roi_align_sampled_bwd_kernel<<<R * PH * PW, 256, 0, (hipStream_t)stream>>>(gout, rois, gfeat, B, C, H, W, PH, PW, scale,
                                                                              sampling_ratio, fs, os);
    I2V_CHECK_LAUNCH("roi_align_sampled_bwd");
    return I2V_OK;
}
```

i2vsgg_amd/csrc/wgrad.hip:

```cpp
#include "conv_common.h"

using namespace convplan;

namespace {

constexpr int BK = 16;
constexpr int LDS_ROW = 20;

struct WgP {
    const float* x; const float* gy; float* gw; int direct;
    const float* row_scale;
    int xcd_remap;
    int r_tiles, r_splits, r_total;
    int nbatch;
    long long bsx, bsg, bsw;
    float* sgd_m; float lr, mom, wd;
    unsigned x_bytes, gy_bytes;
    int B, H, W, Cin, Cout, KH, KW, stride, pad, Ho, Wo, M, N, K, m_per_split, lgCin;
    unsigned long long* clk;
    int abl;
    float* ord_ws; int* ord_cnt; int ord_splits, ord_tiles, ord_acc;
    float* part_ws;
    int part_cap;
};
// ... 424 lines not shown
            for (int j = 0; j < TN; ++j)
                smem[row * CROW + (wn * TN + j) * 16 + fr] = p.row_scale ? acc[i][j][rr] * rsc : acc[i][j][rr];
        }
    __syncthreads();
    if (PREFETCH_W && p.sgd_m) {
#pragma unroll
        for (int it = 0; it < W_LD; ++it) {
            const int e = tid + it * THREADS;
            const int row = e / (BNW / 4), col = (e % (BNW / 4)) * 4;
            const int n = n0 + row, k = k0 + col;
            if (e >= BMW * (BNW / 4) || n >= p.N || k >= p.K) continue;
            const long long o = (long long)n * p.K + k;
            const float4 g = *(const float4*)&smem[row * CROW + col];
            float4 pv = pw[it], mv = pm[it];
            mv.x = p.mom * mv.x + (g.x + p.wd * pv.x); mv.y = p.mom * mv.y + (g.y + p.wd * pv.y);
            mv.z = p.mom * mv.z + (g.z + p.wd * pv.z); mv.w = p.mom * mv.w + (g.w + p.wd * pv.w);
            pv.x -= p.lr * mv.x; pv.y -= p.lr * mv.y; pv.z -= p.lr * mv.z; pv.w -= p.lr * mv.w;
            __builtin_nontemporal_store(__builtin_bit_cast(f32x4, mv), (f32x4*)(p.sgd_m + o));
            __builtin_nontemporal_store(__builtin_bit_cast(f32x4, pv), (f32x4*)(p.gw + o));
        }
    } else if (p.sgd_m || p.direct) {
        for (int e = tid; e < BMW * (BNW / 4); e += THREADS) {
            const int row = e / (BNW / 4), col = (e % (BNW / 4)) * 4;
            const int n = n0 + row, k = k0 + col;
            if (n >= p.N || k >= p.K) continue;
            const long long o = (long long)n * p.K + k;
            float4 g = *(const float4*)&smem[row * CROW + col];
            if (p.sgd_m) {
                float4 pv = *(const float4*)(p.gw + o), mv = *(const float4*)(p.sgd_m + o);
                mv.x = p.mom * mv.x + (g.x + p.wd * pv.x); mv.y = p.mom * mv.y + (g.y + p.wd * pv.y);
                mv.z = p.mom * mv.z + (g.z + p.wd * pv.z); mv.w = p.mom * mv.w + (g.w + p.wd * pv.w);
                pv.x -= p.lr * mv.x; pv.y -= p.lr * mv.y; pv.z -= p.lr * mv.z; pv.w -= p.lr * mv.w;
                *(float4*)(p.sgd_m + o) = mv;
                *(float4*)(p.gw + o) = pv;
            } else {
                *(float4*)(p.gw + o) = g;
            }
        }
    } else if (p.part_ws) {
        float* dst = p.part_ws + ((long long)by * (p.nbatch > 1 ? p.nbatch : 1) + bz) * ((long long)p.N * p.K);
        for (int e = tid; e < BMW * (BNW / 4); e += THREADS) {
            const int row = e / (BNW / 4), col = (e % (BNW / 4)) * 4;
            const int n = n0 + row, k = k0 + col;
            if (n >= p.N || k >= p.K) continue;
            *(float4*)(dst + (long long)n * p.K + k) = *(const float4*)&smem[row * CROW + col];
        }
    } else if (p.ord_ws) {
        constexpr int SC01 = 16;
        const int tile_lin = bz * p.ord_tiles + bx, nsplit = p.ord_splits, my = by;
        const size_t split_stride = (size_t)p.ord_tiles * (p.nbatch > 1 ? p.nbatch : 1) * (BMW * BNW);
        const __amdgpu_buffer_rsrc_t wsr = __builtin_amdgcn_make_buffer_rsrc(
            (void*)(p.ord_ws + (size_t)tile_lin * (BMW * BNW)), 0, 0x7FFFFFF0, 0x00020000);
        for (int e = tid; e < BMW * (BNW / 4); e += THREADS) {
            const int row = e / (BNW / 4), col = (e % (BNW / 4)) * 4;
            const float4 v = *(const float4*)&smem[row * CROW + col];
            __builtin_amdgcn_raw_buffer_store_b128(__builtin_bit_cast(u32x4, v), wsr,
                                                   (unsigned)(my * split_stride * sizeof(float)) + (unsigned)(row * BNW + col) * 4u, 0, SC01);
        }
        __builtin_amdgcn_s_waitcnt(0);
        __syncthreads();
        __shared__ int ord_last;
        if (tid == 0) {
            const int arrived = __hip_atomic_fetch_add(p.ord_cnt + tile_lin, 1, __ATOMIC_RELAXED, __HIP_MEMORY_SCOPE_AGENT);
            const int last = arrived == nsplit - 1;
            if (last) __hip_atomic_store(p.ord_cnt + tile_lin, 0, __ATOMIC_RELAXED, __HIP_MEMORY_SCOPE_AGENT);
            ord_last = last;
        }
        __syncthreads();
        if (ord_last) {
            for (int e = tid; e < BMW * (BNW / 4); e += THREADS) {
                const int row = e / (BNW / 4), col = (e % (BNW / 4)) * 4;
                const int n = n0 + row, k = k0 + col;
                if (n >= p.N || k >= p.K) continue;
                const long long o = (long long)n * p.K + k;
                const unsigned off = (unsigned)(row * BNW + col) * 4u;
                const float4 mine4 = *(const float4*)&smem[row * CROW + col];
                float4 v = make_float4(0.f, 0.f, 0.f, 0.f);
                if (p.ord_acc) v = *(const float4*)(p.gw + o);
                for (int s0 = 0; s0 < nsplit; s0 += 8) {
                    float4 u[8];
#pragma unroll
                    for (int sp = 0; sp < 8; ++sp)
                        u[sp] = __builtin_bit_cast(float4, __builtin_amdgcn_raw_buffer_load_b128(
                            wsr, (s0 + sp < nsplit && s0 + sp != my) ? off + (unsigned)((s0 + sp) * split_stride * sizeof(float)) : 0xFFFFFFF0u, 0, SC01));
#pragma unroll
                    for (int sp = 0; sp < 8; ++sp) {
                        const float4 t = s0 + sp == my ? mine4 : u[sp];
                        if (s0 == 0 && sp == 0 && !p.ord_acc) v = t;
                        else { v.x += t.x; v.y += t.y; v.z += t.z; v.w += t.w; }
                    }
                }
                *(float4*)(p.gw + o) = v;
            }
        }
    } else {
        for (int e = tid; e < BMW * BNW; e += THREADS) {
            const int row = e / BNW, col = e % BNW;
            const int n = n0 + row, k = k0 + col;
            if (n < p.N && k < p.K) atomicAdd(p.gw + (long long)n * p.K + k, smem[row * CROW + col]);
        }
    }
    if constexpr (CLK) {
        __builtin_amdgcn_s_waitcnt(0);
        if (tid == 0 && p.clk) {
            unsigned long long* o = p.clk + 8 * (blockIdx.y * gridDim.x + blockIdx.x);
            o[0] = c_rt0; o[1] = __builtin_amdgcn_s_memrealtime();
            o[2] = c_t1 - c_t0; o[3] = c_t2 - c_t1; o[4] = __builtin_amdgcn_s_memtime() - c_t2;
            o[5] = __builtin_amdgcn_s_getreg(63492); o[6] = __builtin_amdgcn_s_getreg(63508); o[7] = 1;
        }
    }
}

__global__ void __launch_bounds__(256)
wgrad_reduce_kernel(const float* __restrict__ part, float* __restrict__ gw, int splits, int planes, long long nk4, long long bsw, int acc) {
    const long long total = (long long)planes * nk4;
    for (long long e = blockIdx.x * 256ll + threadIdx.x; e < total; e += 256ll * gridDim.x) {
        const long long plane = e / nk4, i = e - plane * nk4;
        float4* o = (float4*)(gw + plane * bsw) + i;
        float4 v = acc ? *o : make_float4(0.f, 0.f, 0.f, 0.f);
        const float4* src = (const float4*)part + plane * nk4 + i;
        for (int s0 = 0; s0 < splits; s0 += 8) {
            float4 u[8];
#pragma unroll
            for (int k = 0; k < 8; ++k) u[k] = s0 + k < splits ? src[(long long)(s0 + k) * planes * nk4] : make_float4(0.f, 0.f, 0.f, 0.f);
#pragma unroll
            for (int k = 0; k < 8; ++k)
                if (s0 + k < splits) { v.x += u[k].x; v.y += u[k].y; v.z += u[k].z; v.w += u[k].w; }
        }
        *o = v;
    }
}
__global__ void __launch_bounds__(256)
wgrad_reduce_scalar_kernel(const float* __restrict__ part, float* __restrict__ gw, int splits, long long nk, int acc) {
    for (long long e = blockIdx.x * 256ll + threadIdx.x; e < nk; e += 256ll * gridDim.x) {
        float v = acc ? gw[e] : 0.f;
        for (int s0 = 0; s0 < splits; s0 += 16) {
            float u[16];
#pragma unroll
            for (int k = 0; k < 16; ++k) u[k] = s0 + k < splits ? part[(long long)(s0 + k) * nk + e] : 0.f;
#pragma unroll
            for (int k = 0; k < 16; ++k)
                if (s0 + k < splits) v += u[k];
        }
        gw[e] = v;
    }
}
constexpr int FCU_WAVES = 8, FCU_THREADS = 64 * FCU_WAVES, FCU_BN = 16 * FCU_WAVES, FCU_TK = 64;
struct FcuP {
    const float* x; const float* gy; float* w; float* m;
    float lr, mom, wd;
    int M, N, K;
    int strips, chunks, tiles, groups;
    unsigned x_bytes, gy_bytes, w_bytes;
};

template <int NS>
__global__ void __launch_bounds__(FCU_THREADS) fc_update_f32(const FcuP p) {
    const int L = (int)blockIdx.x, g = L & 7, r = L >> 3;
    const int start = (int)(((long long)g * p.groups) >> 3), count = (int)(((long long)(g + 1) * p.groups) >> 3) - start;
    if (r >= count) return;
    const int idx = start + r, chunk = idx / p.strips, strip = idx - chunk * p.strips;
    const int t0 = (int)((long long)chunk * p.tiles / p.chunks), t1 = (int)((long long)(chunk + 1) * p.tiles / p.chunks);

    constexpr unsigned MASK = 0x80000000u, NT = 2;
    constexpr int ROWS = 32 * NS;
    __shared__ __attribute__((aligned(16))) float xs[2][ROWS * FCU_TK];
    const int tid = threadIdx.x, lane = tid & 63, wave = tid >> 6, fr = lane & 15, fg = lane >> 4;
    const int n0 = strip * FCU_BN;
    const __amdgpu_buffer_rsrc_t gr = __builtin_amdgcn_make_buffer_rsrc((void*)p.gy, 0, p.gy_bytes, 0x00020000);
    const __amdgpu_buffer_rsrc_t xr = __builtin_amdgcn_make_buffer_rsrc((void*)p.x, 0, p.x_bytes, 0x00020000);
    const __amdgpu_buffer_rsrc_t wr = __builtin_amdgcn_make_buffer_rsrc((void*)p.w, 0, p.w_bytes, 0x00020000);
    const __amdgpu_buffer_rsrc_t mr = __builtin_amdgcn_make_buffer_rsrc((void*)p.m, 0, p.w_bytes, 0x00020000);

    float a[NS * 8];
    {
        const unsigned na = (unsigned)(n0 + 16 * wave + fr);
        const bool nin = (int)na < p.N;
#pragma unroll
        for (int st = 0; st < NS; ++st)
#pragma unroll
            for (int q = 0; q < 8; ++q) {
                const unsigned row = (unsigned)(32 * st + 16 * (q >> 2) + 4 * fg + (q & 3));
                const unsigned off = ((row * (unsigned)p.N + na) * 4u) | ((nin && (int)row < p.M) ? 0u : MASK);
                a[st * 8 + q] = __builtin_bit_cast(float, __builtin_amdgcn_raw_buffer_load_b32(gr, off, 0, 0));
            }
    }

    float4 xv[NS];
    auto xload = [&](int t) {
        const unsigned k = (unsigned)(t * FCU_TK + 4 * (tid & 15));
        const bool kin = t < t1 && (int)k < p.K;
#pragma unroll
        for (int q = 0; q < NS; ++q) {
            const unsigned row = (unsigned)((tid >> 4) + 32 * q);
            const unsigned off = ((row * (unsigned)p.K + k) * 4u) | ((kin && (int)row < p.M) ? 0u : MASK);
            xv[q] = __builtin_bit_cast(float4, __builtin_amdgcn_raw_buffer_load_b128(xr, off, 0, 0));
        }
    };
    auto xstore = [&](int buf) {
#pragma unroll
        for (int q = 0; q < NS; ++q) *(float4*)&xs[buf][((tid >> 4) + 32 * q) * FCU_TK + 4 * (tid & 15)] = xv[q];
    };
    auto wm_offsets = [&](int t, unsigned (&off)[4]) {
        const unsigned k = (unsigned)(t * FCU_TK + 4 * fr);
        const bool kin = t < t1 && (int)k < p.K;
#pragma unroll
        for (int q = 0; q < 4; ++q) {
            const unsigned n = (unsigned)(n0 + 16 * wave + 4 * fg + q);
            off[q] = ((n * (unsigned)p.K + k) * 4u) | ((kin && (int)n < p.N) ? 0u : MASK);
        }
    };
    auto wm_load = [&](int t, float4 (&wv)[4], float4 (&mv)[4]) {
        unsigned off[4];
        wm_offsets(t, off);
#pragma unroll
        for (int q = 0; q < 4; ++q) {
            wv[q] = __builtin_bit_cast(float4, __builtin_amdgcn_raw_buffer_load_b128(wr, off[q], 0, NT));
            mv[q] = __builtin_bit_cast(float4, __builtin_amdgcn_raw_buffer_load_b128(mr, off[q], 0, NT));
        }
    };

    int buf = 0;
    auto body = [&](int t, float4 (&wv)[4], float4 (&mv)[4]) {
        f32x4 acc[4];
#pragma unroll
        for (int j = 0; j < 4; ++j) acc[j] = (f32x4){0.f, 0.f, 0.f, 0.f};
#pragma unroll
        for (int st = 0; st < NS; ++st) {
            float4 b[8];
#pragma unroll
            for (int q = 0; q < 8; ++q) b[q] = *(const float4*)&xs[buf][(32 * st + 16 * (q >> 2) + 4 * fg + (q & 3)) * FCU_TK + 4 * fr];
#pragma unroll
            for (int q = 0; q < 8; ++q) {
                acc[0] = __builtin_amdgcn_mfma_f32_16x16x4f32(a[st * 8 + q], b[q].x, acc[0], 0, 0, 0);
                acc[1] = __builtin_amdgcn_mfma_f32_16x16x4f32(a[st * 8 + q], b[q].y, acc[1], 0, 0, 0);
                acc[2] = __builtin_amdgcn_mfma_f32_16x16x4f32(a[st * 8 + q], b[q].z, acc[2], 0, 0, 0);
                acc[3] = __builtin_amdgcn_mfma_f32_16x16x4f32(a[st * 8 + q], b[q].w, acc[3], 0, 0, 0);
            }
        }
        __builtin_amdgcn_sched_barrier(0);
        unsigned off[4];
        wm_offsets(t, off);
#pragma unroll
        for (int q = 0; q < 4; ++q) {
            float4 pv = wv[q], m4 = mv[q];
            m4.x = p.mom * m4.x + (acc[0][q] + p.wd * pv.x); m4.y = p.mom * m4.y + (acc[1][q] + p.wd * pv.y);
            m4.z = p.mom * m4.z + (acc[2][q] + p.wd * pv.z); m4.w = p.mom * m4.w + (acc[3][q] + p.wd * pv.w);
            pv.x -= p.lr * m4.x; pv.y -= p.lr * m4.y; pv.z -= p.lr * m4.z; pv.w -= p.lr * m4.w;
            __builtin_amdgcn_raw_buffer_store_b128(__builtin_bit_cast(u32x4, m4), mr, off[q], 0, NT);
            __builtin_amdgcn_raw_buffer_store_b128(__builtin_bit_cast(u32x4, pv), wr, off[q], 0, NT);
        }
        xstore(buf ^ 1);
        xload(t + 2);
        wm_load(t + 2, wv, mv);
        __syncthreads();
        buf ^= 1;
    };

    float4 wA[4], mA[4], wB[4], mB[4];
    xload(t0);
    __builtin_amdgcn_s_waitcnt(0);
    xstore(0);
    xload(t0 + 1);
    wm_load(t0, wA, mA);
    wm_load(t0 + 1, wB, mB);
    __syncthreads();
    for (int t = t0;; t += 2) {
        body(t, wA, mA);
        if (t + 1 >= t1) break;
        body(t + 1, wB, mB);
        if (t + 2 >= t1) break;
    }
}
}

static void launch_fc_update(const WgP& p, hipStream_t st) {
    const long long xb = (long long)p.M * p.K * 4, gb = (long long)p.M * p.N * 4, wb = (long long)p.N * p.K * 4;
    FcuP q = {};
    q.x = p.x; q.gy = p.gy; q.w = p.gw; q.m = p.sgd_m; q.lr = p.lr; q.mom = p.mom; q.wd = p.wd;
    q.M = p.M; q.N = p.N; q.K = p.K;
    q.strips = i2v_cdiv(p.N, FCU_BN);
    q.tiles = i2v_cdiv(p.K, FCU_TK);
    q.chunks = std::min(std::max(NUM_CU / q.strips, 1), q.tiles);
    q.groups = q.strips * q.chunks;
    q.x_bytes = (unsigned)xb; q.gy_bytes = (unsigned)gb; q.w_bytes = (unsigned)wb;
    const unsigned grid = (unsigned)((q.groups + 7) / 8 * 8);
    switch (i2v_cdiv(p.M, 32)) {
    case 1: fc_update_f32<1><<<grid, FCU_THREADS, 0, st>>>(q); break;
    case 2: fc_update_f32<2><<<grid, FCU_THREADS, 0, st>>>(q); break;
    case 3: fc_update_f32<3><<<grid, FCU_THREADS, 0, st>>>(q); break;
    case 4: fc_update_f32<4><<<grid, FCU_THREADS, 0, st>>>(q); break;
    case 5: fc_update_f32<5><<<grid, FCU_THREADS, 0, st>>>(q); break;
    case 6: fc_update_f32<6><<<grid, FCU_THREADS, 0, st>>>(q); break;
    case 7: fc_update_f32<7><<<grid, FCU_THREADS, 0, st>>>(q); break;
    default: fc_update_f32<8><<<grid, FCU_THREADS, 0, st>>>(q); break;
    }
}

static ConvShape shape_of(const WgP& p) {
    return {p.B, p.H, p.W, p.Cin, p.Cout, p.KH, p.KW, p.stride, p.pad, p.pad, 1, p.Ho, p.Wo, p.nbatch, 0};
}

static WgradPlan plan_of(const WgP& p, float beta, bool fused, void* split_ws, size_t split_ws_bytes) {
    return plan_wgrad(shape_of(p), beta != 0.f, fused, p.row_scale != nullptr, p.part_ws ? p.part_cap : -1, g_i2v_tuning,
                      g_clk != nullptr, split_ws ? split_ws_bytes : 0);
}

static void launch_wgrad(WgP& p, const WgradPlan& pl, float beta, hipStream_t st, void* split_ws = nullptr) {
    if (pl.kernel == WG_FC_UPDATE) return launch_fc_update(p, st);
    const int planes = p.nbatch > 1 ? p.nbatch : 1;
    p.m_per_split = pl.m_per_split;
    p.direct = pl.direct;
    p.x_bytes = pl.x_bytes;
    p.gy_bytes = pl.gy_bytes;
    if (pl.finish == WFIN_ORDERED_TILES) {
        p.ord_cnt = reinterpret_cast<int*>(split_ws);
        p.ord_ws = reinterpret_cast<float*>(static_cast<char*>(split_ws) + kSplitCounterBytes);
        p.ord_splits = pl.splits; p.ord_tiles = pl.tiles; p.ord_acc = beta != 0.f;
    } else if (pl.finish == WFIN_ORDERED_PARTS) {
        p.part_ws = reinterpret_cast<float*>(static_cast<char*>(split_ws) + kSplitCounterBytes);
    } else if (pl.finish != WFIN_EXTERNAL_PARTS) {
        p.part_ws = nullptr;
    }
    if (pl.ordered_fallback) ++g_ordered_fallbacks;
    if (pl.clear_bytes) hipMemsetAsync(p.gw, 0, pl.clear_bytes, st);
    p.xcd_remap = pl.xcd_remap;
    if (pl.xcd_remap) { p.r_tiles = pl.tiles; p.r_splits = pl.splits; p.r_total = pl.tiles * pl.splits * planes; }
    const dim3 grid(pl.grid[0], pl.grid[1], pl.grid[2]);
    switch (pl.kernel) {
    case WG_V1_64x64: conv_wgrad_f32<64, 64><<<grid, THREADS, 0, st>>>(p); break;
    case WG_V2_DMA_128x128: conv_wgrad2_f32<4, 4, false, false, true><<<grid, THREADS, 0, st>>>(p); break;
    case WG_V2_DMA_128x64: conv_wgrad2_f32<4, 2, false, false, true><<<grid, THREADS, 0, st>>>(p); break;
    case WG_V2_DMA_64x64: conv_wgrad2_f32<2, 2, false, false, true><<<grid, THREADS, 0, st>>>(p); break;
    case WG_V2_FUSED_128x64: conv_wgrad2_f32<4, 2, true><<<grid, THREADS, 0, st>>>(p); break;
    case WG_V2_128x128: conv_wgrad2_f32<4, 4><<<grid, THREADS, 0, st>>>(p); break;
    case WG_V2_128x64: conv_wgrad2_f32<4, 2><<<grid, THREADS, 0, st>>>(p); break;
    case WG_V2_FUSED_64x64: conv_wgrad2_f32<2, 2, true><<<grid, THREADS, 0, st>>>(p); break;
    case WG_V2_CLK_64x64: p.clk = g_clk; p.abl = g_ablate; conv_wgrad2_f32<2, 2, false, true><<<grid, THREADS, 0, st>>>(p); break;
    default: conv_wgrad2_f32<2, 2><<<grid, THREADS, 0, st>>>(p); break;
    }
    const long long nk = (long long)p.N * p.K;
    if (pl.reduce_pass == PASS_VEC4) {
        const long long total = (long long)planes * (nk / 4);
        wgrad_reduce_kernel<<<(unsigned)std::min<long long>(i2v_cdiv(total, 256), 2048), 256, 0, st>>>(
            p.part_ws, p.gw, pl.splits, planes, nk / 4, planes > 1 ? p.bsw : nk, beta != 0.f);
    } else if (pl.reduce_pass == PASS_SCALAR) {
        wgrad_reduce_scalar_kernel<<<(unsigned)std::min<long long>(i2v_cdiv(nk, 256), 2048), 256, 0, st>>>(p.part_ws, p.gw, pl.splits, nk, beta != 0.f);
    }
}

extern "C" int32_t i2v_conv_wgrad_plan(int32_t B, int32_t H, int32_t W, int32_t Cin, int32_t Cout, int32_t KH, int32_t KW,
                                       int32_t stride, int32_t pad, int32_t nbatch, int32_t beta_nonzero, int32_t fused,
                                       int32_t has_row_scale, int32_t ext_part_cap, size_t ws_bytes, int32_t* out, int32_t n_out) {
    I2V_CHECK_ARG(out && n_out >= I2V_WGRAD_PLAN_FIELDS, "conv_wgrad_plan: out needs room for I2V_WGRAD_PLAN_FIELDS values");
    int dummy = 0;
    const int rc = check_conv("conv_wgrad_plan", &dummy, &dummy, &dummy, B, H, W, Cin, Cout, KH, KW, stride, pad);
    if (rc) return rc;
    const ConvShape s = {B, H, W, Cin, Cout, KH, KW, stride, pad, pad, 1, (H + 2 * pad - KH) / stride + 1, (W + 2 * pad - KW) / stride + 1,
                         nbatch, 0};
    const WgradPlan pl = plan_wgrad(s, beta_nonzero != 0, fused != 0, has_row_scale != 0, ext_part_cap, g_i2v_tuning, g_clk != nullptr, ws_bytes);
    const int32_t v[I2V_WGRAD_PLAN_FIELDS] = {pl.status, pl.v2, pl.kernel, pl.tm, pl.tk, pl.splits, pl.m_per_split, pl.finish, pl.direct,
                                              pl.xcd_remap, (int32_t)pl.grid[0], (int32_t)pl.grid[1], (int32_t)pl.grid[2], pl.dma,
                                              clamp32(pl.clear_bytes), pl.reduce_pass, pl.ordered_fallback};
    std::copy(v, v + I2V_WGRAD_PLAN_FIELDS, out);
    return I2V_OK;
}

extern "C" size_t i2v_conv_wgrad_workspace_bytes(int32_t B, int32_t H, int32_t W, int32_t Cin, int32_t Cout,
                                                 int32_t KH, int32_t KW, int32_t stride, int32_t pad) {
    (void)B; (void)H; (void)W; (void)stride; (void)pad;
    (void)Cin; (void)Cout; (void)KH; (void)KW;
    return 256;
}

static int conv_wgrad_impl(const float* x, const float* gy, float* gw, const float* row_scale, int32_t B, int32_t H,
                           int32_t W, int32_t Cin, int32_t Cout, int32_t KH, int32_t KW, int32_t stride, int32_t pad,
                           float beta, void* stream, void* split_ws = nullptr, size_t split_ws_bytes = 0) {
    int rc = check_conv("conv_wgrad", x, gy, gw, B, H, W, Cin, Cout, KH, KW, stride, pad);
    if (rc) return rc;
    hipStream_t st = (hipStream_t)stream;
    WgP p = {};
    p.x = x; p.gy = gy; p.gw = gw; p.row_scale = row_scale;
    p.B = B; p.H = H; p.W = W; p.Cin = Cin; p.Cout = Cout; p.KH = KH; p.KW = KW; p.stride = stride; p.pad = pad;
    p.Ho = (H + 2 * pad - KH) / stride + 1;
    p.Wo = (W + 2 * pad - KW) / stride + 1;
    p.M = B * p.Ho * p.Wo; p.N = Cout; p.K = KH * KW * Cin;
    p.lgCin = ilog2_exact(Cin);
    I2V_CHECK_ARG(beta == 0.f || beta == 1.f, "conv_wgrad: beta must be 0 or 1");
    const WgradPlan pl = plan_of(p, beta, false, split_ws, split_ws_bytes);
    if (pl.status != PLAN_OK) return plan_error(pl.status, shape_of(p));
    launch_wgrad(p, pl, beta, st, split_ws);
    I2V_CHECK_LAUNCH("conv_wgrad");
    return I2V_OK;
}

static int32_t gemm_tn_batched_impl(const float* x, const float* gy, float* gw, int32_t M, int32_t N, int32_t K, int32_t nbatch,
                                    long long stride_x, long long stride_gy, long long stride_gw, float beta, void* stream,
                                    int part_cap = 0, int* part_splits = nullptr) {
    I2V_CHECK_ARG(x && gy && gw && M > 0 && N > 0 && K > 0 && nbatch > 0, "gemm_tn_batched: bad argument");
    I2V_CHECK_ARG(N % 4 == 0 && K % 4 == 0, "gemm_tn_batched: N and K must be multiples of 4");
    I2V_CHECK_ARG(nbatch == 1 || stride_gw == (long long)N * K, "gemm_tn_batched: gw batches must be contiguous");
    WgP p = {};
    p.x = x; p.gy = gy; p.gw = gw;
    p.B = 1; p.H = 1; p.W = M; p.Cin = K; p.Cout = N; p.KH = 1; p.KW = 1; p.stride = 1; p.pad = 0;
    p.Ho = 1; p.Wo = M;
    p.M = M; p.N = N; p.K = K;
    p.lgCin = ilog2_exact(K);
    p.nbatch = nbatch; p.bsx = stride_x; p.bsg = stride_gy; p.bsw = stride_gw;
    if (part_splits) {
        p.part_ws = gw; p.part_cap = part_cap;
    }
    const WgradPlan pl = plan_of(p, beta, false, nullptr, 0);
    if (!pl.v2) {
        i2v_set_error("gemm_tn_batched: operand larger than 2 GiB per batch");
        return I2V_ERR_UNSUPPORTED;
    }
    launch_wgrad(p, pl, beta, (hipStream_t)stream);
    if (part_splits) *part_splits = pl.splits;
    I2V_CHECK_LAUNCH("gemm_tn_batched");
    return I2V_OK;
}

int32_t i2v_internal_reduce_parts(float* parts, int nparts, int planes, long long nk, void* stream) {
    const long long total = (long long)planes * (nk / 4);
    wgrad_reduce_kernel<<<(unsigned)std::min<long long>(i2v_cdiv(total, 256), 4096), 256, 0, (hipStream_t)stream>>>(
        parts, parts, nparts, planes, nk / 4, nk, 0);
    return I2V_OK;
}

void i2v_internal_reduce_scalar(const float* part, float* out, int nparts, long long n, int acc, unsigned blocks, void* stream) {
    wgrad_reduce_scalar_kernel<<<blocks, 256, 0, (hipStream_t)stream>>>(part, out, nparts, n, acc);
}

int32_t i2v_internal_gemm_tn_batched_parts(const float* x, const float* gy, float* parts, int32_t M, int32_t N, int32_t K,
                                           int32_t nbatch, long long stride_x, long long stride_gy, int cap, int* splits, void* stream) {
    return gemm_tn_batched_impl(x, gy, parts, M, N, K, nbatch, stride_x, stride_gy, (long long)N * K, 0.f, stream, cap, splits);
}

extern "C" int32_t i2v_gemm_tn_batched(const float* x, const float* gy, float* gw, int32_t M, int32_t N, int32_t K,
                                       int32_t nbatch, long long stride_x, long long stride_gy, long long stride_gw,
                                       void* stream) {
    return gemm_tn_batched_impl(x, gy, gw, M, N, K, nbatch, stride_x, stride_gy, stride_gw, 0.f, stream);
}

extern "C" int32_t i2v_gemm_tn_batched_acc(const float* x, const float* gy, float* gw, int32_t M, int32_t N, int32_t K,
                                           int32_t nbatch, long long stride_x, long long stride_gy, long long stride_gw,
                                           void* stream) {
    return gemm_tn_batched_impl(x, gy, gw, M, N, K, nbatch, stride_x, stride_gy, stride_gw, 1.f, stream);
}

extern "C" int32_t i2v_conv_wgrad(const float* x, const float* gy, float* gw, int32_t B, int32_t H, int32_t W,
                                  int32_t Cin, int32_t Cout, int32_t KH, int32_t KW, int32_t stride, int32_t pad,
                                  float beta, void* ws, size_t ws_bytes, void* stream) {
    return conv_wgrad_impl(x, gy, gw, nullptr, B, H, W, Cin, Cout, KH, KW, stride, pad, beta, stream, ws, ws_bytes);
}

extern "C" int32_t i2v_conv_wgrad_scaled(const float* x, const float* gy, const float* row_scale, float* gw, int32_t B,
                                         int32_t H, int32_t W, int32_t Cin, int32_t Cout, int32_t KH, int32_t KW,
                                         int32_t stride, int32_t pad, float beta, void* ws, size_t ws_bytes, void* stream) {
    return conv_wgrad_impl(x, gy, gw, row_scale, B, H, W, Cin, Cout, KH, KW, stride, pad, beta, stream, ws, ws_bytes);
}

extern "C" int32_t i2v_conv_wgrad_sgd(const float* x, const float* gy, float* w, float* m, int32_t B, int32_t H,
                                      int32_t W, int32_t Cin, int32_t Cout, int32_t KH, int32_t KW, int32_t stride,
                                      int32_t pad, float lr, float momentum, float weight_decay, void* stream) {
    int rc = check_conv("conv_wgrad_sgd", x, gy, w, B, H, W, Cin, Cout, KH, KW, stride, pad);
    if (rc) return rc;
    I2V_CHECK_ARG(m, "conv_wgrad_sgd: null momentum buffer");
    WgP p = {};
    p.x = x; p.gy = gy; p.gw = w; p.sgd_m = m; p.lr = lr; p.mom = momentum; p.wd = weight_decay;
    p.B = B; p.H = H; p.W = W; p.Cin = Cin; p.Cout = Cout; p.KH = KH; p.KW = KW; p.stride = stride; p.pad = pad;
    p.Ho = (H + 2 * pad - KH) / stride + 1;
    p.Wo = (W + 2 * pad - KW) / stride + 1;
    p.M = B * p.Ho * p.Wo; p.N = Cout; p.K = KH * KW * Cin;
    p.lgCin = ilog2_exact(Cin);
    const WgradPlan pl = plan_of(p, 0.f, true, nullptr, 0);
    if (pl.status != PLAN_OK) return plan_error(pl.status, shape_of(p));
    launch_wgrad(p, pl, 0.f, (hipStream_t)stream);
    I2V_CHECK_LAUNCH("conv_wgrad_sgd");
    return I2V_OK;
}
```

i2vsgg_amd/ops.py:

```python

import ctypes

import numpy as np
import torch

from . import _lib, conv_route, launch
from ._lib import EPI_RELU, EPI_RESIDUAL, EPI_SCALE, EPI_ZEROED, LAYOUT_NCHW, LAYOUT_NHWC, check, lib, ptr, stream
from .conv_route import ARENA, AS_WGRAD, DIRECT, WINOGRAD, WINOGRAD_V

_CL = torch.channels_last


def _need_cuda(*ts):
    for t in ts:
        if t is not None and not t.is_cuda:
            raise _lib.I2VError("i2vsgg_amd ops run on the GPU only (got a %s tensor); there is no CPU fallback"
                                % t.device.type)


def as_nhwc(x):
    if x.dim() != 4:
        raise ValueError("expected a 4-D (B,C,H,W) tensor")
    if x.dtype != torch.float32:
        x = x.float()
# ... 14 lines not shown
ROIALIGN_BWD_KERNELS = {"roi_align_bwd_row2_kernel": 1}
NMS_KERNELS = {"nms_mask_kernel": 1, "nms_scan_super_kernel": 1}


class _RoIAlignFn(torch.autograd.Function):
    @staticmethod
    def forward(ctx, feat, rois, ph, pw, scale, avg, out_nchw):
        _need_cuda(feat, rois)
        rois = _rois_f32(rois)
        nhwc = _is_nhwc(feat)
        if not nhwc:
            feat = feat.contiguous()
        B, C, H, W = feat.shape
        R = rois.size(0)
        out = torch.empty((R, C, ph, pw), device=feat.device, dtype=torch.float32,
                          memory_format=torch.contiguous_format if out_nchw else _CL)
        check(lib.i2v_roi_align_fwd(ptr(feat), LAYOUT_NHWC if nhwc else LAYOUT_NCHW, B, C, H, W, ptr(rois), R, ph, pw,
                                    scale, int(avg), ptr(out), LAYOUT_NCHW if out_nchw else LAYOUT_NHWC, stream()),
              "roi_align_fwd")
        ctx.save_for_backward(rois)
        ctx.meta = (feat.shape, nhwc, ph, pw, scale, int(avg), out_nchw)
        return out

    @staticmethod
    def backward(ctx, gout):
        (rois,) = ctx.saved_tensors
        shape, nhwc, ph, pw, scale, avg, out_nchw = ctx.meta
        B, C, H, W = shape
        gout = gout.contiguous() if out_nchw else gout.contiguous(memory_format=_CL)
        if ROIALIGN_BWD_GATHER and nhwc and not out_nchw and C % 128 == 0 and W * 512 + 21504 <= 60 * 1024 and pw + avg <= 8 and rois.size(0) > 0:
            gfeat = torch.empty(shape, device=gout.device, dtype=torch.float32, memory_format=_CL)
            check(lib.i2v_roi_align_bwd_gather(ptr(gout), ptr(rois), rois.size(0), ph, pw, scale, avg, ptr(gfeat), B, C, H, W,
                                               None, 0, stream()), "roi_align_bwd_gather")
            return gfeat, None, None, None, None, None, None
        arena = launch.arena()
        gfeat = arena.take(B, C, H, W) if (arena is not None and nhwc) else None
        if gfeat is None:
            gfeat = torch.empty(shape, device=gout.device, dtype=torch.float32,
                                memory_format=_CL if nhwc else torch.contiguous_format).zero_()
        check(lib.i2v_roi_align_bwd(ptr(gout), LAYOUT_NCHW if out_nchw else LAYOUT_NHWC, ptr(rois), rois.size(0), ph, pw,
                                    scale, avg, ptr(gfeat), LAYOUT_NHWC if nhwc else LAYOUT_NCHW, B, C, H, W, stream()),
              "roi_align_bwd")
        return gfeat, None, None, None, None, None, None


def roi_align(feat, rois, pooled_h, pooled_w, spatial_scale, avg=True, out_nchw=False):
    return _RoIAlignFn.apply(feat, rois, int(pooled_h), int(pooled_w), float(spatial_scale), bool(avg), bool(out_nchw))


class _RoIAlignSampledFn(torch.autograd.Function):
    @staticmethod
    def forward(ctx, feat, rois, ph, pw, scale, sampling, out_nchw):
        _need_cuda(feat, rois)
        rois = _rois_f32(rois)
        nhwc = _is_nhwc(feat)
        if not nhwc:
            feat = feat.contiguous()
        B, C, H, W = feat.shape
        R = rois.size(0)
        out = torch.empty((R, C, ph, pw), device=feat.device, dtype=torch.float32,
                          memory_format=torch.contiguous_format if out_nchw else _CL)
        check(lib.i2v_roi_align_sampled_fwd(ptr(feat), LAYOUT_NHWC if nhwc else LAYOUT_NCHW, B, C, H, W, ptr(rois), R, ph, pw,
                                            scale, sampling, ptr(out), LAYOUT_NCHW if out_nchw else LAYOUT_NHWC, stream()),
              "roi_align_sampled_fwd")
        ctx.save_for_backward(rois)
        ctx.meta = (feat.shape, nhwc, ph, pw, scale, sampling, out_nchw)
        return out

    @staticmethod
    def backward(ctx, gout):
        (rois,) = ctx.saved_tensors
        shape, nhwc, ph, pw, scale, sampling, out_nchw = ctx.meta
        B, C, H, W = shape
        gout = gout.contiguous() if out_nchw else gout.contiguous(memory_format=_CL)
        gfeat = torch.empty(shape, device=gout.device, dtype=torch.float32,
                            memory_format=_CL if nhwc else torch.contiguous_format).zero_()
        check(lib.i2v_roi_align_sampled_bwd(ptr(gout), LAYOUT_NCHW if out_nchw else LAYOUT_NHWC, ptr(rois), rois.size(0), ph,
                                            pw, scale, sampling, ptr(gfeat), LAYOUT_NHWC if nhwc else LAYOUT_NCHW, B, C, H, W,
                                            stream()), "roi_align_sampled_bwd")
        return gfeat, None, None, None, None, None, None


def roi_align_sampled(feat, rois, pooled_h, pooled_w, spatial_scale, sampling_ratio=0, out_nchw=False):
    return _RoIAlignSampledFn.apply(feat, rois, int(pooled_h), int(pooled_w), float(spatial_scale), int(sampling_ratio),
                                    bool(out_nchw))


class _RoIPoolFn(torch.autograd.Function):
    @staticmethod
    def forward(ctx, feat, rois, ph, pw, scale, out_nchw):
        _need_cuda(feat, rois)
        rois = _rois_f32(rois)
        nhwc = _is_nhwc(feat)
        if not nhwc:
            feat = feat.contiguous()
        B, C, H, W = feat.shape
        R = rois.size(0)
        fmt = torch.contiguous_format if out_nchw else _CL
        out = torch.empty((R, C, ph, pw), device=feat.device, dtype=torch.float32, memory_format=fmt)
        arg = torch.empty((R, C, ph, pw), device=feat.device, dtype=torch.int32, memory_format=fmt)
        check(lib.i2v_roi_pool_fwd(ptr(feat), LAYOUT_NHWC if nhwc else LAYOUT_NCHW, B, C, H, W, ptr(rois), R, ph, pw,
                                   scale, ptr(out), ptr(arg), LAYOUT_NCHW if out_nchw else LAYOUT_NHWC, stream()),
              "roi_pool_fwd")
        ctx.save_for_backward(rois, arg)
        ctx.meta = (feat.shape, nhwc, ph, pw, out_nchw)
        ctx.mark_non_differentiable(arg)
        return out, arg

    @staticmethod
    def backward(ctx, gout, _garg):
        rois, arg = ctx.saved_tensors
        shape, nhwc, ph, pw, out_nchw = ctx.meta
        B, C, H, W = shape
        gout = gout.contiguous() if out_nchw else gout.contiguous(memory_format=_CL)
        gfeat = torch.empty(shape, device=gout.device, dtype=torch.float32,
                            memory_format=_CL if nhwc else torch.contiguous_format).zero_()
        check(lib.i2v_roi_pool_bwd(ptr(gout), ptr(arg), LAYOUT_NCHW if out_nchw else LAYOUT_NHWC, ptr(rois),
                                   rois.size(0), ph, pw, ptr(gfeat), LAYOUT_NHWC if nhwc else LAYOUT_NCHW, B, C, H, W,
                                   stream()), "roi_pool_bwd")
        return gfeat, None, None, None, None, None


def roi_pool(feat, rois, pooled_h, pooled_w, spatial_scale, out_nchw=True, return_argmax=False):
    out, arg = _RoIPoolFn.apply(feat, rois, int(pooled_h), int(pooled_w), float(spatial_scale), bool(out_nchw))
    return (out, arg) if return_argmax else out


class PackedMaps:

    def __init__(self, buf, n_maps, channels, geom):
        _need_cuda(buf, geom)
        if geom.dtype != torch.int32 or geom.numel() < 2 or not geom.is_contiguous():
            raise ValueError("geom must be a contiguous int32 tensor [H, W]")
        if buf.dtype != torch.float32 or not buf.is_contiguous():
            raise ValueError("PackedMaps needs a contiguous fp32 buffer")
        self.buf, self.n_maps, self.channels, self.geom = buf, int(n_maps), int(channels), geom
        self.cap_cells = buf.numel() // (self.n_maps * self.channels)

    @property
    def device(self):
        return self.buf.device

    def view(self, h, w):
        n = self.n_maps * h * w * self.channels
        return self.buf[:n].view(self.n_maps, h, w, self.channels).permute(0, 3, 1, 2)


def roi_pool_packed(maps, rois, pooled_h, pooled_w, spatial_scale, out_nchw=True):
    rois = _rois_f32(rois)
    _need_cuda(rois)
    R, C = rois.size(0), maps.channels
    fmt = torch.contiguous_format if out_nchw else _CL
    out = torch.empty((R, C, pooled_h, pooled_w), device=rois.device, dtype=torch.float32, memory_format=fmt)
    arg = torch.empty((R, C, pooled_h, pooled_w), device=rois.device, dtype=torch.int32, memory_format=fmt)
    check(lib.i2v_roi_pool_fwd_geom(ptr(maps.buf), maps.n_maps, C, ptr(maps.geom), maps.cap_cells, ptr(rois), R,
                                    int(pooled_h), int(pooled_w), float(spatial_scale), ptr(out), ptr(arg),
                                    LAYOUT_NCHW if out_nchw else LAYOUT_NHWC, stream()), "roi_pool_fwd_geom")
    return out


def nms_sorted(dets, thresh, max_keep=0):
    _need_cuda(dets)
    d = dets.contiguous().float()
    if d.dim() == 2:
        d = d.unsqueeze(0)
    n_img, n = d.shape[0], d.shape[1]
    keep = torch.empty((n_img, max(n, 1)), device=d.device, dtype=torch.int32)
    num = torch.empty((n_img,), device=d.device, dtype=torch.int32)
    nb = lib.i2v_nms_workspace_bytes(n_img, n)
    ws = launch.workspace(nb, d.device, "nms")
    check(lib.i2v_nms_sorted(ptr(d), n_img, n, float(thresh), int(max_keep), ptr(keep), ptr(num), ptr(ws), ws.numel(),
                             stream()), "nms_sorted")
    return keep, num


def sort_desc(keys):
    _need_cuda(keys)
    k = keys.contiguous().float()
    if k.dim() == 1:
        k = k.unsqueeze(0)
    n_seg, n = k.shape
    order = torch.empty((n_seg, n), device=k.device, dtype=torch.int32)
    ws = launch.workspace(lib.i2v_sort_desc_workspace_bytes(n_seg, n), k.device, "sort")
    check(lib.i2v_sort_desc(ptr(k), n_seg, n, ptr(order), ptr(ws), ws.numel(), stream()), "sort_desc")
    return order


def rpn_decode(cls_nhwc, bbox_nhwc, im_info, base_anchors, feat_stride, is_prob=False):
    _need_cuda(cls_nhwc, bbox_nhwc, im_info, base_anchors)
    cls_nhwc, bbox_nhwc = as_nhwc(cls_nhwc), as_nhwc(bbox_nhwc)
    B, C2, H, W = cls_nhwc.shape
    A = C2 // 2
    prop = torch.empty((B, H * W * A, 4), device=cls_nhwc.device, dtype=torch.float32)
    score = torch.empty((B, H * W * A), device=cls_nhwc.device, dtype=torch.float32)
    check(lib.i2v_rpn_decode(ptr(cls_nhwc), int(is_prob), ptr(bbox_nhwc), ptr(im_info.contiguous().float()),
                             ptr(base_anchors.contiguous().float()), B, H, W, A, int(feat_stride), ptr(prop), ptr(score),
                             stream()), "rpn_decode")
    return prop, score


def rpn_proposal(cls_nhwc, bbox_nhwc, im_info, base_anchors, feat_stride, pre_nms_top_n, post_nms_top_n, nms_thresh,
                 is_prob=False, want_index=False):
    _need_cuda(cls_nhwc, bbox_nhwc, im_info, base_anchors)
    cls_nhwc, bbox_nhwc = as_nhwc(cls_nhwc), as_nhwc(bbox_nhwc)
    B, C2, H, W = cls_nhwc.shape
    A = C2 // 2
    dev = cls_nhwc.device
    rois = torch.empty((B, post_nms_top_n, 5), device=dev, dtype=torch.float32)
    kept = torch.empty((B, post_nms_top_n), device=dev, dtype=torch.int32) if want_index else None
    num = torch.empty((B,), device=dev, dtype=torch.int32) if want_index else None
    nb = lib.i2v_rpn_proposal_workspace_bytes(B, H, W, A, int(pre_nms_top_n))
    ws = launch.workspace(nb, dev, "rpn")
    info = im_info.contiguous().float()
    base = base_anchors.contiguous().float()
    check(lib.i2v_rpn_proposal(ptr(cls_nhwc), int(is_prob), ptr(bbox_nhwc), ptr(info), ptr(base), B, H, W, A,
                               int(feat_stride), int(pre_nms_top_n), int(post_nms_top_n), float(nms_thresh), ptr(rois),
                               ptr(kept), ptr(num), ptr(ws), ws.numel(), stream()), "rpn_proposal")
    return (rois, kept, num) if want_index else rois


def bbox_overlaps(boxes, gt, want_matrix=False):
    _need_cuda(boxes, gt)
    gt = gt.contiguous().float()
    boxes = boxes.contiguous().float()
    B, K = gt.shape[0], gt.shape[1]
    batched = boxes.dim() == 3
    N = boxes.shape[-2]
    stride = boxes.shape[-1]
    off = 1 if stride == 5 else 0
    ov = torch.empty((B, N, K), device=gt.device, dtype=torch.float32) if want_matrix else None
    mx = torch.empty((B, N), device=gt.device, dtype=torch.float32)
    am = torch.empty((B, N), device=gt.device, dtype=torch.int32)
    check(lib.i2v_bbox_overlaps(ptr(boxes), stride, off, int(batched), ptr(gt), B, N, K, ptr(ov), ptr(mx), ptr(am),
                                stream()), "bbox_overlaps")
    return ov, mx, am


PROFILE = None


class _Timed:

    def __init__(self, flops, tag, desc="", nbytes=0):
        self.on = PROFILE is not None
        if self.on:
            self.rec = (torch.cuda.Event(enable_timing=True), torch.cuda.Event(enable_timing=True), flops, tag, desc,
                        float(nbytes))

    def __enter__(self):
        if self.on:
            self.rec[0].record()

    def __exit__(self, *a):
        if self.on:
            self.rec[1].record()
            PROFILE.append(self.rec)


PARAM_EPOCH = 0


def param_key(w):
    return (w.data_ptr(), w._version, w.device, PARAM_EPOCH if getattr(w, "_i2v_trained", False) else 0)


SMALL_GW_BYTES = 16 << 20
LINEAR_DGRAD_AS_WGRAD = 0
WINOGRAD_TRAIN = True
WINOGRAD_TRAIN_MIN_C = 64
WINOGRAD_WGRAD = True
WINOGRAD_KEEP_V = True
BLOCK_FUSED = True


def _switches():
    return conv_route.Switches(WINOGRAD_TRAIN, WINOGRAD_WGRAD, WINOGRAD_KEEP_V, WINOGRAD_TRAIN_MIN_C, LINEAR_DGRAD_AS_WGRAD,
                               SMALL_GW_BYTES)


def _plan(in_shape, w_shape, stride, pad, **layer):
    return conv_route.plan_conv(tuple(in_shape), tuple(w_shape), stride, pad, _switches(), **layer)


def _wgrad_route(w_shape, stride, pad):
    return _plan((1, w_shape[1], 1, 1), w_shape, stride, pad, needs_w=True).wgrad


def _conv_fwd_raw(x, w, scale, shift, res, stride, pad, flags, out=None):
    B, Cin, H, W = x.shape
    Cout, _, KH, KW = w.shape
    Ho = (H + 2 * pad - KH) // stride + 1
    Wo = (W + 2 * pad - KW) // stride + 1
    y = None
    sws = launch.split_buffer(x.device)
    atomics = lib.i2v_conv_fwd_splits(B, H, W, Cin, Cout, KH, KW, stride, pad, sws.numel()) == 1
    if out is not None and not atomics:
        if tuple(out.shape) != (B, Cout, Ho, Wo) or not out.is_contiguous(memory_format=_CL) or out.dtype != torch.float32:
            raise ValueError("conv2d(out=...): needs a (%d,%d,%d,%d) channels_last fp32 tensor" % (B, Cout, Ho, Wo))
        y = out
    arena = launch.arena()
    if y is None and arena is not None and atomics:
        y = arena.take(B, Cout, Ho, Wo)
        if y is not None:
            flags |= EPI_ZEROED
    if y is None:
        y = torch.empty((B, Cout, Ho, Wo), device=x.device, dtype=torch.float32, memory_format=_CL)
    kern = ""
    if PROFILE is not None:
        plan = (ctypes.c_int32 * 13)()
# ... 1053 lines not shown
```

include/i2vsgg_hip.h:

```cpp
#ifndef I2VSGG_HIP_H
#define I2VSGG_HIP_H

#include <stdint.h>
#include <stddef.h>

#ifdef __cplusplus
extern "C" {
#endif

#define I2V_OK               0
#define I2V_ERR_ARG         -1
#define I2V_ERR_LAUNCH      -2
#define I2V_ERR_WORKSPACE   -3
#define I2V_ERR_UNSUPPORTED -4

#define I2V_LAYOUT_NHWC 0
#define I2V_LAYOUT_NCHW 1

#define I2V_EPI_RELU      1
#define I2V_EPI_RESIDUAL  2
#define I2V_EPI_SCALE     4
#define I2V_EPI_BIAS      8
#define I2V_EPI_ZEROED   16
#define I2V_EPI_MASK     32
// ... 37 lines not shown
                         const float* rois, int32_t R, int32_t pooled_h, int32_t pooled_w,
                         float* grad_feat, int32_t feat_layout, int32_t B, int32_t C, int32_t H, int32_t W,
                         void* stream);

size_t  i2v_nms_workspace_bytes(int32_t n_img, int32_t n);
int32_t i2v_nms_sorted(const float* dets, int32_t n_img, int32_t n, float thresh, int32_t max_keep,
                       int32_t* keep_out, int32_t* num_out, void* workspace, size_t workspace_bytes,
                       void* stream);

size_t  i2v_rpn_proposal_workspace_bytes(int32_t B, int32_t H, int32_t W, int32_t A, int32_t pre_nms_top_n);
int32_t i2v_rpn_proposal(const float* cls, int32_t is_prob, const float* bbox, const float* im_info,
                         const float* base_anchors, int32_t B, int32_t H, int32_t W, int32_t A,
                         int32_t feat_stride, int32_t pre_nms_top_n, int32_t post_nms_top_n, float nms_thresh,
                         float* rois, int32_t* kept_idx, int32_t* num_kept,
                         void* workspace, size_t workspace_bytes, void* stream);

int32_t i2v_rpn_decode(const float* cls, int32_t is_prob, const float* bbox, const float* im_info,
                       const float* base_anchors, int32_t B, int32_t H, int32_t W, int32_t A, int32_t feat_stride,
                       float* proposals , float* scores , void* stream);
size_t  i2v_sort_desc_workspace_bytes(int32_t n_seg, int32_t n);
int32_t i2v_sort_desc(const float* keys, int32_t n_seg, int32_t n, int32_t* order_out ,
                      void* workspace, size_t workspace_bytes, void* stream);

int32_t i2v_image_prep_size(int32_t H, int32_t W, int32_t target_size, int32_t* Ho, int32_t* Wo, float* scale);
int32_t i2v_image_prep(const uint8_t* img, int32_t H, int32_t W, int32_t rgb_order, int32_t flipped,
                       const float* pixel_means_bgr, int32_t target_size, float* blob, int32_t blob_h,
                       int32_t blob_w, void* stream);

size_t  i2v_det_postprocess_workspace_bytes(int32_t R, int32_t C);
int32_t i2v_det_postprocess(const float* rois, const float* cls_prob, const float* bbox_pred, int32_t class_agnostic,
                            const float* stds, const float* means, float im_h, float im_w, float im_scale,
                            int32_t R, int32_t C, float score_thresh, float nms_thresh, int32_t max_per_image,
                            float* dets, int32_t* counts, void* workspace, size_t workspace_bytes, void* stream);
int32_t i2v_det_postprocess_info(const float* rois, const float* cls_prob, const float* bbox_pred, int32_t class_agnostic,
                                 const float* stds, const float* means, const float* im_info,
                                 int32_t R, int32_t C, float score_thresh, float nms_thresh, int32_t max_per_image,
                                 float* dets, int32_t* counts, void* workspace, size_t workspace_bytes, void* stream);

size_t  i2v_relation_topk_workspace_bytes(int32_t n_pairs, int32_t n_rel);
int32_t i2v_relation_topk(const float* rel_score, const float* conf, const int64_t* ixs, const int64_t* ixo,
                          int32_t n_pairs, int32_t n_rel, int32_t k, int32_t* pair_out, int32_t* pred_out,
                          float* conf_out, void* workspace, size_t workspace_bytes, void* stream);

size_t  i2v_video_associate_workspace_bytes(int32_t n_videos, int32_t n_frames, int32_t n_preds);
int32_t i2v_video_associate(const int32_t* frame_off, const int32_t* frame_no, const int32_t* pred_off,
                            const double* score, const int32_t* triplet, const double* boxes,
                            int32_t n_videos, int32_t n_frames, int32_t n_preds, int32_t max_per_frame,
                            int32_t* rel_id, int32_t* rel_start, int32_t* rel_len, double* rel_score,
                            int32_t* n_rel, void* workspace, size_t workspace_bytes, void* stream);
size_t  i2v_video_viou_match_workspace_bytes(int32_t n_pred, int32_t n_gt);
int32_t i2v_video_viou_match(const int32_t* pred_off, const int32_t* pred_rel, const double* pred_score,
                             const int32_t* gt_off, const int32_t* gt_rel, const double* boxes,
                             int32_t n_videos, int32_t n_pred, int32_t n_gt, int64_t n_boxes, int32_t max_pred,
                             int32_t max_gt, double viou_threshold, double* ov, int32_t* hit, double* hit_ov,
                             void* workspace, size_t workspace_bytes, void* stream);

size_t  i2v_seqnms_workspace_bytes(int32_t n_groups, int32_t n_frames, int32_t n_boxes);
int32_t i2v_seqnms(const int32_t* group_off, const int32_t* frame_no, const int32_t* box_off, const float* box,
                   const float* score, int32_t n_groups, int32_t n_frames, int32_t n_boxes, double link_iou,
                   double nms_iou, int32_t rescore, int32_t* tid, float* new_score, int32_t* n_tracks,
                   void* workspace, size_t workspace_bytes, void* stream);

size_t  i2v_relation_targets_workspace_bytes(int32_t n_frames);
int32_t i2v_relation_targets(const int32_t* det_off, const double* det_box, const int32_t* det_cls,
                             const int32_t* gt_off, const double* gt_box, const int32_t* gt_cls,
                             const int32_t* rel_off, const int32_t* rel, const uint32_t* u, const double* ih,
                             const double* iw, int32_t n_frames, int32_t n_det, int32_t n_gt, int32_t n_relations,
                             int32_t n_pred, float* rel5, int32_t* bounds, float* labels, int64_t* ixs, int64_t* ixo,
                             float* w, int32_t* n_pairs, int32_t* n_dropped, int32_t* samp,
                             void* workspace, size_t workspace_bytes, void* stream);

#define I2V_RECOGNITION_MAX_WIDTH 2048
size_t  i2v_recognition_rows_workspace_bytes(int32_t n_pairs);
int32_t i2v_recognition_rows(const float* cls_prob, const float* rel_prob, const int64_t* ixs, const int64_t* ixo,
                             const double* L, int32_t n_boxes, int32_t n_pairs, int32_t n_classes, int32_t n_rel,
                             float* sub, float* obj, float* pre, int32_t* cls, void* workspace, size_t workspace_bytes,
                             void* stream);
size_t  i2v_recognition_align_workspace_bytes(int32_t n_segments, int32_t n_instances);
int32_t i2v_recognition_align(const double* rows, const int32_t* seg_off, const int32_t* seg_row, const int32_t* inst,
                              int32_t n_rows, int32_t n_entries, int32_t n_segments, int32_t n_instances,
                              int32_t n_classes, int32_t n_rel, double* mean, int32_t* count, int32_t* top, int32_t* hit,
                              int64_t* totals, int64_t* per_class, void* workspace, size_t workspace_bytes, void* stream);

#define I2V_IMAGE_RELATION_MAX_GT 4096
#define I2V_IMAGE_RELATION_MAX_K 8
size_t  i2v_image_relation_match_workspace_bytes(int32_t n_images);
int32_t i2v_image_relation_match(const int32_t* pred_off, const int32_t* gt_off, const int32_t* pred_trip,
                                 const double* pred_box, const int32_t* gt_trip, const double* gt_box, int32_t n_images,
                                 int32_t n_pred, int32_t n_gt, int32_t max_gt, double iou_threshold, int32_t* hit,
                                 double* hit_ov, int32_t* gt_rank, void* workspace, size_t workspace_bytes, void* stream);
int32_t i2v_image_relation_count(const int32_t* gt_rank, const int32_t* gt_trip, const int32_t* gt_zs,
                                 const int32_t* nreturns, int32_t n_gt, int32_t n_rel, int32_t n_k, int64_t* totals,
                                 int64_t* zs_totals, int64_t* per_predicate, void* workspace, size_t workspace_bytes,
                                 void* stream);

size_t  i2v_det_eval_match_workspace_bytes(int32_t n_det);
int32_t i2v_det_eval_match(const int32_t* seg_det_off, const int32_t* seg_gt, const int32_t* gt_off,
                           const int32_t* det_key, const double* det_box, const double* gt_box, const int32_t* gt_hard,
                           int32_t n_seg, int32_t n_det, int32_t n_slots, int32_t n_gt, int32_t max_gt, double ovthresh,
                           int32_t* flag, double* ovmax, int32_t* jmax,
                           void* workspace, size_t workspace_bytes, void* stream);
size_t  i2v_det_eval_curve_workspace_bytes(int32_t n_det);
int32_t i2v_det_eval_curve(const int32_t* det_key, const int32_t* cls_off, const int32_t* flag, const int32_t* npos,
                           int32_t n_cls, int32_t n_det, int32_t* perm, int32_t* cum_tp, int32_t* cum_fp,
                           double* rec, double* prec, double* ap_area, double* ap_11pt,
                           void* workspace, size_t workspace_bytes, void* stream);

int32_t i2v_bbox_overlaps(const float* boxes, int32_t box_stride, int32_t box_off, int32_t boxes_batched,
                          const float* gt, int32_t B, int32_t N, int32_t K,
                          float* overlaps, float* max_ov, int32_t* argmax_ov, void* stream);

int32_t i2v_conv_fwd(const float* x, const float* w, const float* scale, const float* shift, const float* res,
                     float* y, int32_t B, int32_t H, int32_t W, int32_t Cin, int32_t Cout,
                     int32_t KH, int32_t KW, int32_t stride, int32_t pad, int32_t flags,
                     void* split_workspace, size_t split_workspace_bytes, void* stream);
int32_t i2v_conv_fwd_splits(int32_t B, int32_t H, int32_t W, int32_t Cin, int32_t Cout, int32_t KH, int32_t KW,
                            int32_t stride, int32_t pad, size_t ws_bytes);
size_t  i2v_conv_split_workspace_bytes(int32_t B, int32_t H, int32_t W, int32_t Cin, int32_t Cout, int32_t KH,
                                       int32_t KW, int32_t stride, int32_t pad);
#define I2V_FWD_PLAN_FIELDS   13
#define I2V_WGRAD_PLAN_FIELDS 17
int32_t i2v_conv_fwd_plan(int32_t B, int32_t H, int32_t W, int32_t Cin, int32_t Cout, int32_t KH, int32_t KW,
                          int32_t stride, int32_t pad, int32_t nbatch, int32_t flags, size_t ws_bytes, int32_t* out, int32_t n_out);
int32_t i2v_conv_wgrad_plan(int32_t B, int32_t H, int32_t W, int32_t Cin, int32_t Cout, int32_t KH, int32_t KW,
                            int32_t stride, int32_t pad, int32_t nbatch, int32_t beta_nonzero, int32_t fused,
                            int32_t has_row_scale, int32_t ext_part_cap, size_t ws_bytes, int32_t* out, int32_t n_out);
#define I2V_TUNE_CONV_SPEC            0
#define I2V_TUNE_SPLIT_TARGET         1
#define I2V_TUNE_SPLIT_TARGET_SKINNY  2
#define I2V_TUNE_SPLIT_BELOW          3
#define I2V_TUNE_SPLIT_ATOMICS        4
#define I2V_TUNE_BIG_FC_TILE          5
#define I2V_TUNE_WGRAD_V2             6
#define I2V_TUNE_WGRAD_FUSED_TILE     7
#define I2V_TUNE_WINO_ROWS            8
#define I2V_TUNE_ROIPOOL_C128         9
#define I2V_TUNE_CONV_GEMM           10
#define I2V_TUNE_STAGGER             11
#define I2V_TUNE_ROIALIGN_COLS       12
#define I2V_TUNE_WGRAD_PER_CU        13
#define I2V_TUNE_WGRAD_XCD           14
#define I2V_TUNE_FC_FOLD             15
#define I2V_TUNE_GEMM_X3             16
#define I2V_TUNE_GEMM_PERSIST        17
#define I2V_TUNE_WGRAD_PRIO          18
#define I2V_TUNE_STREAM_TILE         19
#define I2V_TUNE_KGROUPS             20
#define I2V_TUNE_WGRAD_ORDERED_GFLOP 21
#define I2V_TUNE_GEMM_DMA            22
#define I2V_TUNE_WGRAD_DMA           23
#define I2V_TUNE_ROIALIGN_BWD        24
#define I2V_TUNE_NMS_SCAN            25
#define I2V_TUNE_FC_UPDATE           26
#define I2V_TUNE_COUNT               27
int32_t i2v_set_tuning(int32_t key, int32_t value);
int32_t i2v_get_tuning(int32_t key);
int32_t i2v_conv_set_tile(int32_t cfg);
int32_t i2v_conv_debug_clock(void* buf);
int32_t i2v_debug_clock_stamp(void* out2, void* stream);
int32_t i2v_conv_dgrad_fused(const float* gy, const float* w, const float* gy_scale, const float* out_scale,
                             const float* res, const float* mask, float* gx, int32_t B, int32_t H, int32_t W,
                             int32_t Cin, int32_t Cout, int32_t KH, int32_t KW, int32_t stride, int32_t pad,
                             void* workspace, size_t workspace_bytes, void* split_workspace, size_t split_workspace_bytes,
                             void* stream);
int32_t i2v_conv_wgrad_scaled(const float* x, const float* gy, const float* row_scale, float* gw, int32_t B,
                              int32_t H, int32_t W, int32_t Cin, int32_t Cout, int32_t KH, int32_t KW,
                              int32_t stride, int32_t pad, float beta, void* split_workspace, size_t split_workspace_bytes,
                              void* stream);
int32_t i2v_ordered_fallbacks(int32_t reset);
int32_t i2v_conv3x3_winograd4_dgrad(const float* gy, const float* U, const float* out_scale, const float* mask,
                                    float* gx, int32_t B, int32_t H, int32_t W, int32_t Cout, int32_t Cin,
                                    void* workspace, size_t workspace_bytes, void* stream);
size_t  i2v_conv3x3_winograd4_wgrad_workspace_bytes(int32_t B, int32_t H, int32_t W, int32_t Cin, int32_t Cout);
int32_t i2v_conv3x3_winograd4_wgrad(const float* x, const float* gy, const float* row_scale, float* gw,
                                    int32_t B, int32_t H, int32_t W, int32_t Cin, int32_t Cout, float beta,
                                    void* workspace, size_t workspace_bytes, void* stream);
size_t  i2v_conv3x3_winograd4_v_bytes(int32_t B, int32_t H, int32_t W, int32_t Cin);
int32_t i2v_conv3x3_winograd4_fwd_keep(const float* x, const float* U, const float* scale, const float* shift,
                                       float* y, float* v_out, int32_t B, int32_t H, int32_t W, int32_t Cin,
                                       int32_t Cout, int32_t relu, void* workspace, size_t workspace_bytes, void* stream);
int32_t i2v_conv3x3_winograd4_wgrad_v(const float* v, const float* gy, const float* row_scale, float* gw,
                                      int32_t B, int32_t H, int32_t W, int32_t Cin, int32_t Cout, float beta,
                                      void* workspace, size_t workspace_bytes, void* stream);
int32_t i2v_gemm_tn_batched(const float* x, const float* gy, float* gw, int32_t M, int32_t N, int32_t K,
                            int32_t nbatch, long long stride_x, long long stride_gy, long long stride_gw, void* stream);
int32_t i2v_gemm_tn_batched_acc(const float* x, const float* gy, float* gw, int32_t M, int32_t N, int32_t K,
                            int32_t nbatch, long long stride_x, long long stride_gy, long long stride_gw, void* stream);
size_t  i2v_conv_dgrad_workspace_bytes(int32_t Cin, int32_t Cout, int32_t KH, int32_t KW);
int32_t i2v_conv_dgrad(const float* gy, const float* w, float* gx, int32_t B, int32_t H, int32_t W,
                       int32_t Cin, int32_t Cout, int32_t KH, int32_t KW, int32_t stride, int32_t pad,
                       void* workspace, size_t workspace_bytes, void* split_workspace, size_t split_workspace_bytes,
                       void* stream);
size_t  i2v_conv_wgrad_workspace_bytes(int32_t B, int32_t H, int32_t W, int32_t Cin, int32_t Cout,
                                       int32_t KH, int32_t KW, int32_t stride, int32_t pad);
int32_t i2v_conv_wgrad(const float* x, const float* gy, float* gw, int32_t B, int32_t H, int32_t W,
                       int32_t Cin, int32_t Cout, int32_t KH, int32_t KW, int32_t stride, int32_t pad,
                       float beta, void* workspace, size_t workspace_bytes, void* stream);

int32_t i2v_gemm_nt_batched(const float* a, const float* b, float* c, int32_t M, int32_t N, int32_t K, int32_t nbatch,
                            int64_t stride_a, int64_t stride_b, int64_t stride_c,
                            void* split_workspace, size_t split_workspace_bytes, void* stream);

int32_t i2v_winograd_filter(const float* w, float* U, int32_t Cout, int32_t Cin, void* stream);
size_t  i2v_conv3x3_winograd_workspace_bytes(int32_t B, int32_t H, int32_t W, int32_t Cin, int32_t Cout);
int32_t i2v_conv3x3_winograd_fwd(const float* x, const float* U, const float* scale, const float* shift, float* y,
                                 int32_t B, int32_t H, int32_t W, int32_t Cin, int32_t Cout, int32_t relu,
                                 void* workspace, size_t workspace_bytes, void* stream);

int32_t i2v_winograd4_filter(const float* w, float* U, int32_t Cout, int32_t Cin, void* stream);
int32_t i2v_winograd4_filter_dgrad(const float* w, float* U, int32_t Cout, int32_t Cin, void* stream);
size_t  i2v_conv3x3_winograd4_workspace_bytes(int32_t B, int32_t H, int32_t W, int32_t Cin, int32_t Cout);
int32_t i2v_conv3x3_winograd4_fwd(const float* x, const float* U, const float* scale, const float* shift, float* y,
                                  int32_t B, int32_t H, int32_t W, int32_t Cin, int32_t Cout, int32_t relu,
                                  void* workspace, size_t workspace_bytes, void* stream);

int32_t i2v_conv_wgrad_sgd(const float* x, const float* gy, float* w, float* m, int32_t B, int32_t H, int32_t W,
                           int32_t Cin, int32_t Cout, int32_t KH, int32_t KW, int32_t stride, int32_t pad,
                           float lr, float momentum, float weight_decay, void* stream);

int32_t i2v_epilogue_bwd(const float* gy, const float* y, const float* scale, float* g, float* gpre, float* gbias,
                         int64_t M, int32_t N, int32_t relu, float* g_t, void* split_ws, size_t split_ws_bytes, void* stream);

int32_t i2v_maxpool3x3s2_fwd(const float* x, float* y, int32_t* argmax, int32_t B, int32_t H, int32_t W, int32_t C,
                             void* stream);

int32_t i2v_dstyle_pool_fwd(const float* x1, const float* x2, float* z, int64_t rows, int32_t n_img,
                            int32_t dim, int32_t rank, void* stream);
int32_t i2v_dstyle_pool_bwd(const float* gz, const float* x1, const float* x2, float* g1, float* g2,
                            int64_t rows, int32_t n_img, int32_t dim, int32_t rank, void* stream);
size_t  i2v_dstyle_fused_workspace_bytes(int64_t rows, int32_t n_img, int32_t dim, int32_t rank);
int32_t i2v_dstyle_fused_fwd(const float* x, const float* w1, const float* b1, const float* w2, const float* b2,
                             float* z, float* x1, float* x2, int64_t rows, int32_t n_img, int32_t k, int32_t dim,
                             int32_t rank, void* workspace, size_t workspace_bytes, void* stream);

int32_t i2v_l2norm_rows_fwd(const float* x, float* y, float* inv_norm, int32_t rows, int32_t cols, float eps, void* stream);
int32_t i2v_l2norm_rows_bwd(const float* g, const float* y, const float* inv_norm, float* gx, int32_t rows, int32_t cols,
                            float eps, void* stream);
int32_t i2v_bce_rows_fwd(const float* z, const float* t, const float* w, float* loss, int32_t rows, int32_t cols,
                         void* stream);
int32_t i2v_bce_rows_bwd(const float* z, const float* t, const float* w, const float* gloss, float* gz, int32_t rows,
                         int32_t cols, void* stream);

int32_t i2v_pair_gather_fwd(const float* obj, const int64_t* ixs, const int64_t* ixo, float* out, int32_t n_pairs,
                            int32_t n_box, int32_t emb, void* stream);
int32_t i2v_pair_gather_bwd(const float* g, const int64_t* ixs, const int64_t* ixo, float* gobj, int32_t n_pairs,
                            int32_t n_box, int32_t emb, void* stream);

int32_t i2v_half_mse_fwd(const float* d, int64_t n, float target, float* out, void* stream);
int32_t i2v_half_mse_bwd(const float* d, int64_t n, float target, const float* gout, float* gd, void* stream);
int32_t i2v_smooth_l1_fwd(const float* pred, const float* tgt, const float* inw, const float* outw, int64_t n, int32_t per_weight,
                          int32_t rows, float sigma, float* out, void* stream);
int32_t i2v_smooth_l1_bwd(const float* pred, const float* tgt, const float* inw, const float* outw, int64_t n, int32_t per_weight,
                          int32_t rows, float sigma, const float* gout, float* gpred, void* stream);
int32_t i2v_bbox_transform(const float* ex, int32_t ex_batched, const float* gt, int32_t gt_stride, float* out, int32_t B, int32_t N,
                           const float* means4, const float* stds4, void* stream);
int32_t i2v_signed_sqrt_fwd(const float* z, float* y, int64_t n, void* stream);
int32_t i2v_signed_sqrt_bwd(const float* z, const float* g, float* gz, int64_t n, void* stream);

int32_t i2v_dpixel_fwd(const float* x, const float* w1, const float* w2, const float* w3, float* h1, float* h2,
                       float* d, float* feat, int32_t M, int32_t pix_per_roi, void* stream);
size_t  i2v_dpixel_bwd_workspace_bytes(void);
int32_t i2v_dpixel_bwd(const float* gd, const float* gfeat, const float* d, const float* h1, const float* h2,
                       const float* w1, const float* w2, const float* w3, float* g3, float* gh2, float* gh1,
                       float* gx, int32_t M, int32_t pix_per_roi, float lambda, void* workspace,
                       size_t workspace_bytes, void* stream);

int32_t i2v_sgd_momentum(float* p, const float* g, float* m, int64_t n, float lr, float momentum,
                         float weight_decay, void* stream);
int32_t i2v_sgd_momentum_multi(float* const* p, const float* const* g, float* const* m, const int64_t* n,
                               const float* lr, const float* weight_decay, int32_t count, float momentum,
                               void* stream);

int32_t i2v_adam_step(int32_t* step_counter, void* stream);
int32_t i2v_adam_multi(float* const* p, const float* const* g, float* const* m, float* const* v, const int64_t* n,
                       const double* lr, const float* weight_decay, int32_t count, double beta1, double beta2, double eps,
                       const int32_t* step_counter, void* stream);

#ifdef __cplusplus
}
#endif
#endif
```

Measured before the change: 505.8 frames/s.

## Add FC update kernel fused with next-step forward GEMM; drop roi_pool argmax

Adds a lookahead variant of the fused FC SGD update kernel. While applying the momentum update to each weight tile, it multiplies the updated weights with the next forward input, producing split-K partials that a small finish kernel reduces with bias and ReLU. This is meant to avoid re-reading the weights in the following forward GEMM, at the cost of extra LDS and registers, which may force single buffering. The path is off by default behind a new tuning knob. Separately, roi_pool forward no longer allocates or writes the argmax buffer, saving an allocation and int32 stores.

```diff
diff --git a/i2vsgg_amd/_lib.py b/i2vsgg_amd/_lib.py
--- a/i2vsgg_amd/_lib.py
+++ b/i2vsgg_amd/_lib.py
@@ -68,6 +68,9 @@
     "i2v_conv3x3_winograd4_fwd_keep": (_i, [_p, _p, _p, _p, _p, _p, _i, _i, _i, _i, _i, _i, _p, _z, _p]),
     "i2v_conv3x3_winograd4_wgrad_v": (_i, [_p, _p, _p, _p, _i, _i, _i, _i, _i, _f, _p, _z, _p]),
     "i2v_conv_wgrad_sgd": (_i, [_p, _p, _p, _p, _i, _i, _i, _i, _i, _i, _i, _i, _i, _f, _f, _f, _p]),
+    "i2v_conv_wgrad_sgd_lookahead": (_i, [_p, _p, _p, _p, _i, _i, _i, _i, _i, _i, _i, _i, _i, _f, _f, _f, _p, _i, _p, _z, _z, _p, _p]),
+    "i2v_fc_lookahead_finish": (_i, [_p, _i, _p, _p, _i, _i, _i, _p]),
+    "i2v_fc_lookahead_plan": (_i, [_i, _i, _i, _i, _z, _p, _i]),
     "i2v_epilogue_bwd": (_i, [_p, _p, _p, _p, _p, _p, _l, _i, _i, _p, _p, _z, _p]),
     "i2v_maxpool3x3s2_fwd": (_i, [_p, _p, _p, _i, _i, _i, _i, _p]),
     "i2v_sgd_momentum": (_i, [_p, _p, _p, _l, _f, _f, _f, _p]),
@@ -147,7 +150,7 @@
 TUNE = {"I2V_CONV_SPEC": 0, "I2V_SPLIT_TARGET": 1, "I2V_SPLIT_TARGET_SKINNY": 2, "I2V_SPLIT_BELOW": 3, "I2V_SPLIT_ATOMICS": 4,
         "I2V_BIG_FC_TILE": 5, "I2V_WGRAD_V2": 6, "I2V_WGRAD_FUSED_TILE": 7, "I2V_WINO_ROWS": 8, "I2V_ROIPOOL_C128": 9, "I2V_CONV_GEMM": 10, "I2V_STAGGER": 11, "I2V_ROIALIGN_COLS": 12, "I2V_WGRAD_PER_CU": 13, "I2V_WGRAD_XCD": 14, "I2V_FC_FOLD": 15, "I2V_GEMM_X3": 16,
         "I2V_GEMM_PERSIST": 17, "I2V_WGRAD_PRIO": 18, "I2V_STREAM_TILE": 19, "I2V_KGROUPS": 20, "I2V_WGRAD_ORDERED_GFLOP": 21, "I2V_GEMM_DMA": 22,
-        "I2V_WGRAD_DMA": 23, "I2V_ROIALIGN_BWD": 24, "I2V_NMS_SCAN": 25, "I2V_FC_UPDATE": 26}
+        "I2V_WGRAD_DMA": 23, "I2V_ROIALIGN_BWD": 24, "I2V_NMS_SCAN": 25, "I2V_FC_UPDATE": 26, "I2V_FC_LOOKAHEAD": 27}
 ENV_TUNE = ("I2V_SPLIT_ATOMICS", "I2V_SPLIT_TARGET", "I2V_SPLIT_TARGET_SKINNY", "I2V_SPLIT_BELOW", "I2V_BIG_FC_TILE",
             "I2V_WGRAD_FUSED_TILE", "I2V_WGRAD_PER_CU", "I2V_KGROUPS", "I2V_WGRAD_ORDERED_GFLOP", "I2V_WINO_ROWS", "I2V_GEMM_DMA", "I2V_WGRAD_DMA", "I2V_ROIALIGN_BWD", "I2V_NMS_SCAN")
 RETIRED_ENV = ("I2V_WINOGRAD_TRAIN", "I2V_BLOCK_FUSED", "I2V_WINOGRAD_WGRAD", "I2V_KEEP_V", "I2V_WGRAD_BRANCH", "I2V_ISD_BATCHED",
diff --git a/i2vsgg_amd/csrc/api.cpp b/i2vsgg_amd/csrc/api.cpp
--- a/i2vsgg_amd/csrc/api.cpp
+++ b/i2vsgg_amd/csrc/api.cpp
@@ -12,7 +12,7 @@
     va_end(ap);
 }
 
-extern "C" int32_t i2v_version(void) { return 107; }
+extern "C" int32_t i2v_version(void) { return 108; }
 extern "C" const char* i2v_last_error(void) { return g_err; }
 
 int g_i2v_tuning[I2V_TUNE_COUNT] = {
@@ -21,7 +21,7 @@
      1,  0,  2,  4,  1,
      0,  0,  0,  0,  1,
      0,  1000000,  1,  1,  1,  2,
-     1,
+     1,  0,
 };
 
 extern "C" int32_t i2v_build_flags(void) {
diff --git a/i2vsgg_amd/csrc/conv.hip b/i2vsgg_amd/csrc/conv.hip
--- a/i2vsgg_amd/csrc/conv.hip
+++ b/i2vsgg_amd/csrc/conv.hip
@@ -1031,6 +1031,8 @@
 }
 
 }
+
+int i2v_internal_force_tile() { return g_force_tile; }
 
 extern "C" int32_t i2v_ordered_fallbacks(int32_t reset) {
     const int n = g_ordered_fallbacks;
diff --git a/i2vsgg_amd/csrc/conv_common.h b/i2vsgg_amd/csrc/conv_common.h
--- a/i2vsgg_amd/csrc/conv_common.h
+++ b/i2vsgg_amd/csrc/conv_common.h
@@ -46,6 +46,8 @@
 extern int g_ablate;
 extern int g_ordered_fallbacks;
 
+int i2v_internal_force_tile();
+
 int32_t i2v_internal_gemm_tn_batched_parts(const float* x, const float* gy, float* parts, int32_t M, int32_t N, int32_t K,
                                            int32_t nbatch, long long stride_x, long long stride_gy, int cap, int* splits, void* stream);
 int32_t i2v_internal_reduce_parts(float* parts, int nparts, int planes, long long nk, void* stream);
diff --git a/i2vsgg_amd/csrc/conv_plan.h b/i2vsgg_amd/csrc/conv_plan.h
--- a/i2vsgg_amd/csrc/conv_plan.h
+++ b/i2vsgg_amd/csrc/conv_plan.h
@@ -148,7 +148,8 @@
 enum WgradKernel {
     WG_V1_64x64 = 0, WG_V2_DMA_128x128, WG_V2_DMA_128x64, WG_V2_DMA_64x64, WG_V2_FUSED_128x64, WG_V2_128x128, WG_V2_128x64,
     WG_V2_FUSED_64x64, WG_V2_CLK_64x64, WG_V2_64x64,
-    WG_FC_UPDATE
+    WG_FC_UPDATE,
+    WG_FC_UPDATE_LOOKAHEAD
 };
 enum WgradFinish { WFIN_DIRECT = 0, WFIN_ATOMICS = 1, WFIN_ORDERED_TILES = 2, WFIN_ORDERED_PARTS = 3, WFIN_EXTERNAL_PARTS = 4 };
 
@@ -259,4 +260,26 @@
     return q;
 }
 
-}
+struct FcLookaheadPlan {
+    int kernel;
+    int splits, k_per_split;
+};
+
+inline FcLookaheadPlan plan_fc_lookahead(const ConvShape& upd, int m_next, const int* tuning, int force_tile, bool clk, size_t fwd_ws_bytes) {
+    FcLookaheadPlan q = {};
+    const WgradPlan u = plan_wgrad(upd, false, true, false, -1, tuning, clk, 0);
+    q.kernel = u.status == PLAN_OK ? u.kernel : -1;
+    if (u.status != PLAN_OK || u.kernel != WG_FC_UPDATE || !tuning[I2V_TUNE_FC_LOOKAHEAD]) return q;
+    const int N = upd.N(), K = upd.K();
+    if (m_next < 1 || m_next > 256 || K % 64 != 0 || (long long)m_next * K * 4 >= (1ll << 31)) return q;
+    const ConvShape f = {m_next, 1, 1, K, N, 1, 1, 1, 0, 0, 1, 1, 1, 0, 0};
+    const FwdPlan fp = plan_conv_fwd(f, tuning, force_tile, clk, fwd_ws_bytes);
+    if (fp.status != PLAN_OK || fp.finish != FIN_IN_KERNEL || fp.splitk < 2 || fp.k_per_split % 64 != 0) return q;
+    if (fp.form != FORM_GEMM && fp.form != FORM_GEMM_DMA32 && fp.form != FORM_GEMM_DMA16) return q;
+    q.kernel = WG_FC_UPDATE_LOOKAHEAD;
+    q.splits = fp.splitk;
+    q.k_per_split = fp.k_per_split;
+    return q;
+}
+
+}
diff --git a/i2vsgg_amd/csrc/roi_ops.hip b/i2vsgg_amd/csrc/roi_ops.hip
--- a/i2vsgg_amd/csrc/roi_ops.hip
+++ b/i2vsgg_amd/csrc/roi_ops.hip
@@ -757,13 +757,13 @@
     if (out_nchw) {
         float* o = out + (long long)r * C * P + (long long)c0 * P;
         int* a = argmax + (long long)r * C * P + (long long)c0 * P;
-        for (int e = threadIdx.x; e < nch * P; e += 256) { o[e] = sval[e]; a[e] = sarg[e]; }
+        for (int e = threadIdx.x; e < nch * P; e += 256) { o[e] = sval[e]; if (argmax) a[e] = sarg[e]; }
     } else {
         for (int p = wave; p < P; p += 4)
             if (live) {
                 long long o = (long long)r * P * C + (long long)p * C + c;
                 out[o] = sval[lane * P + p];
-                argmax[o] = sarg[lane * P + p];
+                if (argmax) argmax[o] = sarg[lane * P + p];
             }
     }
 }
@@ -835,17 +835,17 @@
         if ((((long long)r * C + c0) * P) % 4 == 0 && (128 * P) % 4 == 0) {
             for (int e = threadIdx.x * 4; e < 128 * P; e += 4 * blockDim.x) {
                 *(float4*)(o + e) = *(const float4*)(sval + e);
-                *(int4*)(a + e) = *(const int4*)(sarg + e);
+                if (argmax) *(int4*)(a + e) = *(const int4*)(sarg + e);
             }
         } else {
-            for (int e = threadIdx.x; e < 128 * P; e += blockDim.x) { o[e] = sval[e]; a[e] = sarg[e]; }
+            for (int e = threadIdx.x; e < 128 * P; e += blockDim.x) { o[e] = sval[e]; if (argmax) a[e] = sarg[e]; }
         }
     } else {
         for (int e = threadIdx.x; e < 128 * P; e += blockDim.x) {
             const int p = e >> 7, ch = e & 127;
             const long long o = (long long)r * P * C + (long long)p * C + c0 + ch;
             out[o] = sval[ch * P + p];
-            argmax[o] = sarg[ch * P + p];
+            if (argmax) argmax[o] = sarg[ch * P + p];
         }
     }
 }
@@ -1113,7 +1113,7 @@
                                          const float* rois, int32_t R, int32_t PH, int32_t PW, float scale, float* out,
                                          int32_t* argmax, int32_t out_layout, void* stream) {
     if (R == 0) return I2V_OK;
-    I2V_CHECK_ARG(feat && geom && rois && out && argmax, "roi_pool_fwd_geom: null pointer");
+    I2V_CHECK_ARG(feat && geom && rois && out, "roi_pool_fwd_geom: null pointer");
     I2V_CHECK_ARG(B > 0 && C > 0 && cap_cells > 0 && R >= 0 && PH > 0 && PW > 0, "roi_pool_fwd_geom: bad shape");
     return roi_pool_fwd_launch(feat, I2V_LAYOUT_NHWC, B, C, 1, 1, geom, (long long)cap_cells, rois, R, PH, PW, scale, out,
                                argmax, out_layout, stream);
diff --git a/i2vsgg_amd/csrc/wgrad.hip b/i2vsgg_amd/csrc/wgrad.hip
--- a/i2vsgg_amd/csrc/wgrad.hip
+++ b/i2vsgg_amd/csrc/wgrad.hip
@@ -600,19 +600,27 @@
     int M, N, K;
     int strips, chunks, tiles, groups;
     unsigned x_bytes, gy_bytes, w_bytes;
+    const float* xn; float* part; int Mn, tps; unsigned xn_bytes;
 };
 
-template <int NS>
+template <int NS, int NL = 0>
 __global__ void __launch_bounds__(FCU_THREADS) fc_update_f32(const FcuP p) {
     const int L = (int)blockIdx.x, g = L & 7, r = L >> 3;
     const int start = (int)(((long long)g * p.groups) >> 3), count = (int)(((long long)(g + 1) * p.groups) >> 3) - start;
     if (r >= count) return;
     const int idx = start + r, chunk = idx / p.strips, strip = idx - chunk * p.strips;
-    const int t0 = (int)((long long)chunk * p.tiles / p.chunks), t1 = (int)((long long)(chunk + 1) * p.tiles / p.chunks);
+    const int t0 = NL > 0 ? chunk * p.tps : (int)((long long)chunk * p.tiles / p.chunks);
+    const int t1 = NL > 0 ? min(p.tiles, t0 + p.tps) : (int)((long long)(chunk + 1) * p.tiles / p.chunks);
 
     constexpr unsigned MASK = 0x80000000u, NT = 2;
-    constexpr int ROWS = 32 * NS;
-    __shared__ __attribute__((aligned(16))) float xs[2][ROWS * FCU_TK];
+    constexpr int ROWS = 32 * NS, NROWS = 16 * NL;
+    constexpr int WT_FLOATS = NL > 0 ? FCU_WAVES * 16 * FCU_TK : 0;
+    constexpr bool DB = (2 * (ROWS + NROWS) * FCU_TK + WT_FLOATS) * 4 <= 160 * 1024;
+    constexpr int NBUF = DB ? 2 : 1;
+    static_assert((NBUF * (ROWS + NROWS) * FCU_TK + WT_FLOATS) * 4 <= 160 * 1024, "the tiles fit the CU's LDS");
+    __shared__ __attribute__((aligned(16))) float xs[NBUF][ROWS * FCU_TK];
+    __shared__ __attribute__((aligned(16))) float xns[NBUF][NL > 0 ? NROWS * FCU_TK : 4];
+    __shared__ __attribute__((aligned(16))) float wts[NL > 0 ? WT_FLOATS : 4];
     const int tid = threadIdx.x, lane = tid & 63, wave = tid >> 6, fr = lane & 15, fg = lane >> 4;
     const int n0 = strip * FCU_BN;
     const __amdgpu_buffer_rsrc_t gr = __builtin_amdgcn_make_buffer_rsrc((void*)p.gy, 0, p.gy_bytes, 0x00020000);
@@ -649,6 +657,30 @@
 #pragma unroll
         for (int q = 0; q < NS; ++q) *(float4*)&xs[buf][((tid >> 4) + 32 * q) * FCU_TK + 4 * (tid & 15)] = xv[q];
     };
+    const __amdgpu_buffer_rsrc_t nr = __builtin_amdgcn_make_buffer_rsrc((void*)(NL > 0 ? p.xn : p.x), 0, NL > 0 ? p.xn_bytes : 0u, 0x00020000);
+    constexpr int NV = NL > 0 ? NL / 2 : 1;
+    float4 nv[NV];
+    auto nload = [&](int t) {
+        const unsigned k = (unsigned)(t * FCU_TK + 4 * (tid & 15));
+        const bool kin = t < t1 && (int)k < p.K;
+#pragma unroll
+        for (int q = 0; q < NV; ++q) {
+            const unsigned row = (unsigned)((tid >> 4) + 32 * q);
+            const unsigned off = ((row * (unsigned)p.K + k) * 4u) | ((kin && (int)row < p.Mn) ? 0u : MASK);
+            nv[q] = __builtin_bit_cast(float4, __builtin_amdgcn_raw_buffer_load_b128(nr, off, 0, 0));
+        }
+    };
+    auto nstore = [&](int buf) {
+#pragma unroll
+        for (int q = 0; q < NV; ++q) {
+            const int row = (tid >> 4) + 32 * q;
+            *(float4*)&xns[buf][row * FCU_TK + (((tid & 15) ^ (row & 15)) << 2)] = nv[q];
+        }
+    };
+    f32x4 accn[NL > 0 ? NL : 1];
+#pragma unroll
+    for (int i = 0; i < (NL > 0 ? NL : 1); ++i) accn[i] = (f32x4){0.f, 0.f, 0.f, 0.f};
+    float* const wtw = wts + (NL > 0 ? wave * (16 * FCU_TK) : 0);
     auto wm_offsets = [&](int t, unsigned (&off)[4]) {
         const unsigned k = (unsigned)(t * FCU_TK + 4 * fr);
         const bool kin = t < t1 && (int)k < p.K;
@@ -697,19 +729,66 @@
             pv.x -= p.lr * m4.x; pv.y -= p.lr * m4.y; pv.z -= p.lr * m4.z; pv.w -= p.lr * m4.w;
             __builtin_amdgcn_raw_buffer_store_b128(__builtin_bit_cast(u32x4, m4), mr, off[q], 0, NT);
             __builtin_amdgcn_raw_buffer_store_b128(__builtin_bit_cast(u32x4, pv), wr, off[q], 0, NT);
-        }
-        xstore(buf ^ 1);
-        xload(t + 2);
-        wm_load(t + 2, wv, mv);
-        __syncthreads();
-        buf ^= 1;
+            if constexpr (NL > 0) {
+                const int r = 4 * fg + q;
+                *(float4*)&wtw[r * FCU_TK + ((fr ^ r) << 2)] = pv;
+            }
+        }
+        if constexpr (NL > 0) {
+            __builtin_amdgcn_fence(__ATOMIC_RELEASE, "wavefront");
+            __builtin_amdgcn_wave_barrier();
+            __builtin_amdgcn_fence(__ATOMIC_ACQUIRE, "wavefront");
+#pragma unroll
+            for (int sh = 0; sh < 4; ++sh) {
+                const float4 wb = *(const float4*)&wtw[fr * FCU_TK + (((4 * sh + fg) ^ fr) << 2)];
+#pragma unroll
+                for (int i0 = 0; i0 < NL; i0 += 4) {
+                    float4 xa[4];
+#pragma unroll
+                    for (int i = 0; i < 4; ++i) xa[i] = *(const float4*)&xns[buf][(16 * (i0 + i) + fr) * FCU_TK + (((4 * sh + fg) ^ fr) << 2)];
+#pragma unroll
+                    for (int i = 0; i < 4; ++i) accn[i0 + i] = __builtin_amdgcn_mfma_f32_16x16x4f32(wb.x, xa[i].x, accn[i0 + i], 0, 0, 0);
+#pragma unroll
+                    for (int i = 0; i < 4; ++i) accn[i0 + i] = __builtin_amdgcn_mfma_f32_16x16x4f32(wb.y, xa[i].y, accn[i0 + i], 0, 0, 0);
+#pragma unroll
+                    for (int i = 0; i < 4; ++i) accn[i0 + i] = __builtin_amdgcn_mfma_f32_16x16x4f32(wb.z, xa[i].z, accn[i0 + i], 0, 0, 0);
+#pragma unroll
+                    for (int i = 0; i < 4; ++i) accn[i0 + i] = __builtin_amdgcn_mfma_f32_16x16x4f32(wb.w, xa[i].w, accn[i0 + i], 0, 0, 0);
+                }
+            }
+            __builtin_amdgcn_fence(__ATOMIC_RELEASE, "wavefront");
+            __builtin_amdgcn_wave_barrier();
+            __builtin_amdgcn_sched_barrier(0);
+        }
+        if constexpr (DB) {
+            xstore(buf ^ 1);
+            if constexpr (NL > 0) nstore(buf ^ 1);
+            xload(t + 2);
+            if constexpr (NL > 0) nload(t + 2);
+            wm_load(t + 2, wv, mv);
+            __syncthreads();
+            buf ^= 1;
+        } else {
+            __syncthreads();
+            xload(t + 1);
+            nload(t + 1);
+            wm_load(t + 2, wv, mv);
+            xstore(0);
+            nstore(0);
+            __syncthreads();
+        }
     };
 
     float4 wA[4], mA[4], wB[4], mB[4];
     xload(t0);
+    if constexpr (NL > 0) nload(t0);
     __builtin_amdgcn_s_waitcnt(0);
     xstore(0);
-    xload(t0 + 1);
+    if constexpr (NL > 0) nstore(0);
+    if constexpr (DB) {
+        xload(t0 + 1);
+        if constexpr (NL > 0) nload(t0 + 1);
+    }
     wm_load(t0, wA, mA);
     wm_load(t0 + 1, wB, mB);
     __syncthreads();
@@ -718,6 +797,40 @@
         if (t + 1 >= t1) break;
         body(t + 1, wB, mB);
         if (t + 2 >= t1) break;
+    }
+    if constexpr (NL > 0) {
+        const int n = n0 + 16 * wave + 4 * fg;
+        float* dst = p.part + (size_t)chunk * p.Mn * p.N;
+#pragma unroll
+        for (int i = 0; i < NL; ++i) {
+            const int row = 16 * i + fr;
+            if (row < p.Mn && n < p.N) *(f32x4*)(dst + (size_t)row * p.N + n) = accn[i];
+        }
+    }
+}
+
+__global__ void __launch_bounds__(256)
+fc_lookahead_finish_kernel(const float* __restrict__ part, const float* __restrict__ bias, float* __restrict__ y, int splits,
+                           long long mn4, int N, int relu) {
+    for (long long e = blockIdx.x * 256ll + threadIdx.x; e < mn4; e += 256ll * gridDim.x) {
+        const float4* src = (const float4*)part + e;
+        float4 v = make_float4(0.f, 0.f, 0.f, 0.f);
+        for (int s0 = 0; s0 < splits; s0 += kSplitInKernelMax) {
+            float4 u[kSplitInKernelMax];
+#pragma unroll
+            for (int sp = 0; sp < kSplitInKernelMax; ++sp) u[sp] = s0 + sp < splits ? src[(long long)(s0 + sp) * mn4] : make_float4(0.f, 0.f, 0.f, 0.f);
+#pragma unroll
+            for (int sp = 0; sp < kSplitInKernelMax; ++sp) {
+                if (s0 == 0 && sp == 0) v = u[sp];
+                else { v.x += u[sp].x; v.y += u[sp].y; v.z += u[sp].z; v.w += u[sp].w; }
+            }
+        }
+        if (bias) {
+            const float4 b = *(const float4*)(bias + (int)((e * 4) % N));
+            v.x += b.x; v.y += b.y; v.z += b.z; v.w += b.w;
+        }
+        if (relu) { v.x = fmaxf(v.x, 0.f); v.y = fmaxf(v.y, 0.f); v.z = fmaxf(v.z, 0.f); v.w = fmaxf(v.w, 0.f); }
+        ((float4*)y)[e] = v;
     }
 }
 }
@@ -745,6 +858,37 @@
     }
 }
 
+template <int NL>
+static void launch_fc_lookahead_nl(const FcuP& q, unsigned grid, hipStream_t st) {
+    switch (i2v_cdiv(q.M, 32)) {
+    case 1: fc_update_f32<1, NL><<<grid, FCU_THREADS, 0, st>>>(q); break;
+    case 2: fc_update_f32<2, NL><<<grid, FCU_THREADS, 0, st>>>(q); break;
+    case 3: fc_update_f32<3, NL><<<grid, FCU_THREADS, 0, st>>>(q); break;
+    case 4: fc_update_f32<4, NL><<<grid, FCU_THREADS, 0, st>>>(q); break;
+    case 5: fc_update_f32<5, NL><<<grid, FCU_THREADS, 0, st>>>(q); break;
+    case 6: fc_update_f32<6, NL><<<grid, FCU_THREADS, 0, st>>>(q); break;
+    case 7: fc_update_f32<7, NL><<<grid, FCU_THREADS, 0, st>>>(q); break;
+    default: fc_update_f32<8, NL><<<grid, FCU_THREADS, 0, st>>>(q); break;
+    }
+}
+
+static void launch_fc_lookahead(const WgP& p, const FcLookaheadPlan& la, const float* xn, int Mn, float* part, hipStream_t st) {
+    FcuP q = {};
+    q.x = p.x; q.gy = p.gy; q.w = p.gw; q.m = p.sgd_m; q.lr = p.lr; q.mom = p.mom; q.wd = p.wd;
+    q.M = p.M; q.N = p.N; q.K = p.K;
+    q.strips = i2v_cdiv(p.N, FCU_BN);
+    q.tiles = p.K / FCU_TK;
+    q.chunks = la.splits;
+    q.tps = la.k_per_split / FCU_TK;
+    q.groups = q.strips * q.chunks;
+    q.x_bytes = (unsigned)((long long)p.M * p.K * 4); q.gy_bytes = (unsigned)((long long)p.M * p.N * 4);
+    q.w_bytes = (unsigned)((long long)p.N * p.K * 4);
+    q.xn = xn; q.part = part; q.Mn = Mn; q.xn_bytes = (unsigned)((long long)Mn * p.K * 4);
+    const unsigned grid = (unsigned)((q.groups + 7) / 8 * 8);
+    if (Mn <= 128) launch_fc_lookahead_nl<8>(q, grid, st);
+    else launch_fc_lookahead_nl<16>(q, grid, st);
+}
+
 static ConvShape shape_of(const WgP& p) {
     return {p.B, p.H, p.W, p.Cin, p.Cout, p.KH, p.KW, p.stride, p.pad, p.pad, 1, p.Ho, p.Wo, p.nbatch, 0};
 }
@@ -928,3 +1072,60 @@
     I2V_CHECK_LAUNCH("conv_wgrad_sgd");
     return I2V_OK;
 }
+
+static WgP linear_update_problem(const float* x, const float* gy, float* w, float* m, int32_t B, int32_t H, int32_t W, int32_t Cin,
+                                 int32_t Cout, int32_t KH, int32_t KW, int32_t stride, int32_t pad, float lr, float momentum,
+                                 float weight_decay) {
+    WgP p = {};
+    p.x = x; p.gy = gy; p.gw = w; p.sgd_m = m; p.lr = lr; p.mom = momentum; p.wd = weight_decay;
+    p.B = B; p.H = H; p.W = W; p.Cin = Cin; p.Cout = Cout; p.KH = KH; p.KW = KW; p.stride = stride; p.pad = pad;
+    p.Ho = (H + 2 * pad - KH) / stride + 1;
+    p.Wo = (W + 2 * pad - KW) / stride + 1;
+    p.M = B * p.Ho * p.Wo; p.N = Cout; p.K = KH * KW * Cin;
+    p.lgCin = ilog2_exact(Cin);
+    return p;
+}
+
+extern "C" int32_t i2v_fc_lookahead_plan(int32_t M, int32_t K, int32_t N, int32_t M_next, size_t fwd_ws_bytes, int32_t* out, int32_t n_out) {
+    I2V_CHECK_ARG(out && n_out >= 3, "fc_lookahead_plan: out needs room for 3 values");
+    I2V_CHECK_ARG(M > 0 && K > 0 && N > 0 && K % 4 == 0, "fc_lookahead_plan: bad shape");
+    const ConvShape s = {M, 1, 1, K, N, 1, 1, 1, 0, 0, 1, 1, 1, 0, 0};
+    const FcLookaheadPlan la = plan_fc_lookahead(s, M_next, g_i2v_tuning, i2v_internal_force_tile(), g_clk != nullptr, fwd_ws_bytes);
+    out[0] = la.kernel; out[1] = la.splits; out[2] = la.k_per_split;
+    return I2V_OK;
+}
+
+extern "C" int32_t i2v_conv_wgrad_sgd_lookahead(const float* x, const float* gy, float* w, float* m, int32_t B, int32_t H, int32_t W,
+                                                int32_t Cin, int32_t Cout, int32_t KH, int32_t KW, int32_t stride, int32_t pad,
+                                                float lr, float momentum, float weight_decay, const float* x_next, int32_t M_next,
+                                                float* partials, size_t partials_bytes, size_t fwd_ws_bytes, int32_t* splits,
+                                                void* stream) {
+    int rc = check_conv("conv_wgrad_sgd_lookahead", x, gy, w, B, H, W, Cin, Cout, KH, KW, stride, pad);
+    if (rc) return rc;
+    I2V_CHECK_ARG(m && splits, "conv_wgrad_sgd_lookahead: null momentum buffer or split count");
+    WgP p = linear_update_problem(x, gy, w, m, B, H, W, Cin, Cout, KH, KW, stride, pad, lr, momentum, weight_decay);
+    *splits = 0;
+    const WgradPlan pl = plan_of(p, 0.f, true, nullptr, 0);
+    if (pl.status != PLAN_OK) return plan_error(pl.status, shape_of(p));
+    FcLookaheadPlan la = {};
+    if (x_next && partials && M_next > 0)
+        la = plan_fc_lookahead(shape_of(p), M_next, g_i2v_tuning, i2v_internal_force_tile(), g_clk != nullptr, fwd_ws_bytes);
+    if (la.kernel == WG_FC_UPDATE_LOOKAHEAD && (size_t)la.splits * M_next * p.N * sizeof(float) <= partials_bytes) {
+        launch_fc_lookahead(p, la, x_next, M_next, partials, (hipStream_t)stream);
+        *splits = la.splits;
+    } else {
+        launch_wgrad(p, pl, 0.f, (hipStream_t)stream);
+    }
+    I2V_CHECK_LAUNCH("conv_wgrad_sgd_lookahead");
+    return I2V_OK;
+}
+
+extern "C" int32_t i2v_fc_lookahead_finish(const float* partials, int32_t splits, const float* bias, float* y, int32_t M, int32_t N,
+                                           int32_t relu, void* stream) {
+    I2V_CHECK_ARG(partials && y && splits > 0 && M > 0 && N > 0 && N % 4 == 0, "fc_lookahead_finish: bad argument");
+    const long long mn4 = (long long)M * N / 4;
+    fc_lookahead_finish_kernel<<<(unsigned)std::min<long long>(i2v_cdiv(mn4, 256), 2048), 256, 0, (hipStream_t)stream>>>(
+        partials, bias, y, splits, mn4, N, relu);
+    I2V_CHECK_LAUNCH("fc_lookahead_finish");
+    return I2V_OK;
+}
diff --git a/i2vsgg_amd/ops.py b/i2vsgg_amd/ops.py
--- a/i2vsgg_amd/ops.py
+++ b/i2vsgg_amd/ops.py
@@ -190,9 +190,8 @@
     R, C = rois.size(0), maps.channels
     fmt = torch.contiguous_format if out_nchw else _CL
     out = torch.empty((R, C, pooled_h, pooled_w), device=rois.device, dtype=torch.float32, memory_format=fmt)
-    arg = torch.empty((R, C, pooled_h, pooled_w), device=rois.device, dtype=torch.int32, memory_format=fmt)
     check(lib.i2v_roi_pool_fwd_geom(ptr(maps.buf), maps.n_maps, C, ptr(maps.geom), maps.cap_cells, ptr(rois), R,
-                                    int(pooled_h), int(pooled_w), float(spatial_scale), ptr(out), ptr(arg),
+                                    int(pooled_h), int(pooled_w), float(spatial_scale), ptr(out), None,
                                     LAYOUT_NCHW if out_nchw else LAYOUT_NHWC, stream()), "roi_pool_fwd_geom")
     return out
 
diff --git a/include/i2vsgg_hip.h b/include/i2vsgg_hip.h
--- a/include/i2vsgg_hip.h
+++ b/include/i2vsgg_hip.h
@@ -213,7 +213,8 @@
 #define I2V_TUNE_ROIALIGN_BWD        24
 #define I2V_TUNE_NMS_SCAN            25
 #define I2V_TUNE_FC_UPDATE           26
-#define I2V_TUNE_COUNT               27
+#define I2V_TUNE_FC_LOOKAHEAD        27
+#define I2V_TUNE_COUNT               28
 int32_t i2v_set_tuning(int32_t key, int32_t value);
 int32_t i2v_get_tuning(int32_t key);
 int32_t i2v_conv_set_tile(int32_t cfg);
@@ -278,6 +279,13 @@
 int32_t i2v_conv_wgrad_sgd(const float* x, const float* gy, float* w, float* m, int32_t B, int32_t H, int32_t W,
                            int32_t Cin, int32_t Cout, int32_t KH, int32_t KW, int32_t stride, int32_t pad,
                            float lr, float momentum, float weight_decay, void* stream);
+int32_t i2v_conv_wgrad_sgd_lookahead(const float* x, const float* gy, float* w, float* m, int32_t B, int32_t H, int32_t W,
+                                     int32_t Cin, int32_t Cout, int32_t KH, int32_t KW, int32_t stride, int32_t pad,
+                                     float lr, float momentum, float weight_decay, const float* x_next, int32_t M_next,
+                                     float* partials, size_t partials_bytes, size_t fwd_ws_bytes, int32_t* splits, void* stream);
+int32_t i2v_fc_lookahead_finish(const float* partials, int32_t splits, const float* bias, float* y, int32_t M, int32_t N,
+                                int32_t relu, void* stream);
+int32_t i2v_fc_lookahead_plan(int32_t M, int32_t K, int32_t N, int32_t M_next, size_t fwd_ws_bytes, int32_t* out, int32_t n_out);
 
 int32_t i2v_epilogue_bwd(const float* gy, const float* y, const float* scale, float* g, float* gpre, float* gbias,
                          int64_t M, int32_t N, int32_t relu, float* g_t, void* split_ws, size_t split_ws_bytes, void* stream);
```

Result: no change. 506.9 frames/s (median of 6 runs) (+0.2%).
